# Boese0601/Dyadic-Interaction-Modeling

Measured on AMD Instinct MI355X. Metric: listener clips/sec (T=300, EMOCA-56), higher is better.
Workload: dtype bf16; 1 GPU; C3: B=256/GPU synthetic dyad clips, T=300, SLMFT.forward(mode='val'): listener VQ encode + encoder + 299-step AR decode (top-k 52 sampling) + VQ decode; global_batch=256, seq_len=300, gather=tokens+coeffs, gather_bytes_per_rank=17452032

## Files before the change

### dyadic-interaction-modeling_amd/csrc/chain.hip

```cpp
#include <algorithm>

#include "common.hpp"
#include "decode_attn_body.hpp"

namespace dimx {
namespace {

typedef __attribute__((address_space(3))) void lds_void_t;
typedef const __attribute__((address_space(1))) void glb_void_t;

constexpr int kWaves = 8;
constexpr int kThreads = kWaves * 64;
constexpr int kGroupCUs = 32;
constexpr int kGroupRows = 32;
constexpr int AUX_PLAIN = 0, AUX_SC1 = 16;
constexpr size_t kMaxDynLds = 160 * 1024 - 512;

__device__ __forceinline__ unsigned xcc_id() {
    unsigned v;
    asm volatile("s_getreg_b32 %0, hwreg(HW_REG_XCC_ID)" : "=s"(v));
    return v & 0xf;
}
__device__ __forceinline__ unsigned ld_sc1_u32(const unsigned* p) {
    return __hip_atomic_load(p, __ATOMIC_RELAXED, __HIP_MEMORY_SCOPE_AGENT);
// ... 758 lines not shown
    const int n1 = a.g1.W ? a.g1.ncb : 1, n2 = a.g2.W ? a.g2.ncb : 1;
    if (a.defer) {
        if (a.g2.W) {
            if (n1 == 1 && n2 == 1) CHD(true, 1, 1);
            else if (n1 == 2 && n2 == 1) CHD(true, 2, 1);
            else if (n1 == 1 && n2 == 2) CHD(true, 1, 2);
            else CHD(true, 2, 2);
        } else {
            if (n1 == 1) CHD(false, 1, 1);
            else CHD(false, 2, 1);
        }
    } else if (a.g1.W && a.g2.W) {
        if (n1 == 1 && n2 == 1) CH(true, true, 1, 1);
        else if (n1 == 2 && n2 == 1) CH(true, true, 2, 1);
        else if (n1 == 1 && n2 == 2) CH(true, true, 1, 2);
        else CH(true, true, 2, 2);
    } else if (a.g1.W) {
        if (n1 == 1) CH(true, false, 1, 1);
        else CH(true, false, 2, 1);
    } else if (a.g2.W) {
        if (n2 == 1) CH(false, true, 1, 1);
        else CH(false, true, 1, 2);
    } else {
        CH(false, false, 1, 1);
    }
#undef CH
#undef CHD
    DIMX_HIP(hipGetLastError());
    return DIMX_OK;
}


static size_t layer_plan(LayerChainArgs& a) {
    desc_fill(a.g_so);
    desc_fill(a.g_cq);
    desc_fill(a.g_co);
    const size_t sc_bytes = ((size_t)kAttnWaves * a.sc_stride * 4 + 1023) / 1024 * 1024;
    a.off_base = (int)sc_bytes;
    auto wbytes = [](const ChainGemmDesc& d) { return (size_t)d.nkt * d.rows_pad * 128 + 4096; };
    auto abytes = [](const ChainGemmDesc& d) { return (size_t)d.nkt * kGroupRows * 128; };
    auto rbytes = [](const ChainGemmDesc& d) { return (size_t)kWaves * d.ncb * 4096; };
    a.off_A1 = 0;
    a.off_W1 = (int)abytes(a.g_so);
    const size_t end1 = std::max(a.off_W1 + wbytes(a.g_so), rbytes(a.g_so));
    a.off_A2 = 0;
    a.off_W2 = (int)std::max(abytes(a.g_cq), rbytes(a.g_so));
    const size_t end2 = std::max(a.off_W2 + wbytes(a.g_cq), rbytes(a.g_cq));
    a.off_W3 = 0;
    a.off_A3 = (int)std::max(wbytes(a.g_co), rbytes(a.g_co));
    const size_t end3 = a.off_A3 + abytes(a.g_co);
    return sc_bytes + std::max(end1, std::max(end2, end3));
}

bool layer_chain_supported(const LayerChainArgs& a0, int cu_count) {
    LayerChainArgs a = a0;
    if (cu_count != 8 * kGroupCUs) return false;
    if (a.B < 1 || a.B > 8 * kGroupRows || a.C > 3 * kThreads || a.C % 64 != 0) return false;
    if (a.sa.H != kAttnWaves || a.ca.H != kAttnWaves || a.sa.dtype != DIMX_BF16 || a.ca.dtype != DIMX_BF16) return false;
    if (a.B * kAttnWaves * 2 <= 3072) return false;
    if (a.ca.rows_per_clip > 1) return false;
    for (ChainGemmDesc* d : {&a.g_so, &a.g_cq, &a.g_co}) {
        if (!d->W || d->N % kGroupCUs != 0 || d->K % 64 != 0 || d->ldw % 8 != 0) return false;
        desc_fill(*d);
        if (d->ncb < 1 || d->ncb > 2) return false;
    }
    if (a.g_so.N != a.C || a.g_co.N != a.C || a.g_cq.K != a.C || a.g_so.ncb != 2 || a.g_co.ncb != 2 || a.g_cq.ncb != 1) return false;
    if (a.ld_o % 8 != 0) return false;
    return layer_plan(a) <= kMaxDynLds;
}

int launch_layer_chain(const LayerChainArgs& a0, hipStream_t s) {
    LayerChainArgs a = a0;
    DIMX_REQUIRE(a.x && a.y && a.o && a.qc && a.stats && a.colsum_cq && a.counters && a.seen && a.err, DIMX_ERR_ARG,
                 "layer_chain: null operand");
    const size_t lds = layer_plan(a);
    DIMX_REQUIRE(lds <= kMaxDynLds, DIMX_ERR_ARG, "layer_chain: LDS plan %zu bytes", lds);
    if (a.sa.tab) {
        DIMX_REQUIRE(a.sa.hist && a.sa.hist_ld >= a.sa.Tmax && a.sa.Tmax >= 1 && a.sa.tab_rows >= 1 && a.sa.tab_ld % 8 == 0 &&
                         a.sa.tab_koff % 8 == 0 && a.sa.tab_voff % 8 == 0 && a.sa.tab_koff >= 0 && a.sa.tab_voff >= 0 &&
                         a.sa.tab_koff + kAttnWaves * 64 <= a.sa.tab_ld && a.sa.tab_voff + kAttnWaves * 64 <= a.sa.tab_ld &&
                         (uintptr_t)a.sa.tab % 16 == 0,
                     DIMX_ERR_ARG, "layer_chain: table form with rows of %d, K at %d, V at %d, history stride %d", a.sa.tab_ld, a.sa.tab_koff,
                     a.sa.tab_voff, a.sa.hist_ld);
        (void)hipFuncSetAttribute((const void*)xcd_layer_kernel<2, 1, 2, true>, hipFuncAttributeMaxDynamicSharedMemorySize, (int)kMaxDynLds);
        hipLaunchKernelGGL((xcd_layer_kernel<2, 1, 2, true>), dim3(8 * kGroupCUs), dim3(kLayerThreads), lds, s, a);
        DIMX_HIP(hipGetLastError());
        return DIMX_OK;
    }
    (void)hipFuncSetAttribute((const void*)xcd_layer_kernel<2, 1, 2>, hipFuncAttributeMaxDynamicSharedMemorySize, (int)kMaxDynLds);
    hipLaunchKernelGGL((xcd_layer_kernel<2, 1, 2>), dim3(8 * kGroupCUs), dim3(kLayerThreads), lds, s, a);
    DIMX_HIP(hipGetLastError());
    return DIMX_OK;
}

}
```

### dyadic-interaction-modeling_amd/csrc/common.hpp

```cpp
#pragma once
#include <hip/hip_runtime.h>
#include <stdint.h>
#include <stdio.h>
#include <string.h>
#include <string>

#include "../../include/dimx.h"

namespace dimx {

void set_error(const char* fmt, ...);
const char* get_error();

#define DIMX_HIP(expr)                                                                       \
    do {                                                                                     \
        hipError_t _e = (expr);                                                              \
        if (_e != hipSuccess) {                                                              \
            dimx::set_error("%s:%d: %s -> %s", __FILE__, __LINE__, #expr, hipGetErrorString(_e)); \
            return DIMX_ERR_HIP;                                                             \
        }                                                                                    \
    } while (0)

#define DIMX_REQUIRE(cond, code, ...)       \
    do {                                    \
// ... 222 lines not shown
    int w_tiled;
    const void* w3;
    long w3_plane;
    int x3_decode;
    int vt_pack4;
};

void gemm_args_init(GemmArgs& a);
void gemm_set_plain_out(GemmArgs& a, void* C, int ldc);
int launch_gemm(const GemmArgs& a, hipStream_t s);
bool gemm256_eligible(const GemmArgs& a);
int launch_gemm256(const GemmArgs& a, hipStream_t s);
int launch_gemm256_segs(const GemmArgs& a, const OutSeg* segs, int nseg, int seg_width, hipStream_t s);
bool gemm_use_x3(const GemmArgs& a);
bool gemm_x3_plan(const GemmArgs& a, int* bn_out, int* sp_out);
int launch_gemm_x3(const GemmArgs& a, hipStream_t s);
int launch_split_x3(const float* w, void* planes, size_t n, hipStream_t s);
int gemm_plan_splits(const GemmArgs& a);

int launch_layernorm(int out_dtype, const float* x, void* y, const float* gamma, const float* beta, int M,
                     int C, hipStream_t s);
int launch_add_slabs_layernorm(int out_dtype, float* x, const float* slabs, int nslab, long slab_stride, void* y,
                               const float* gamma, int M, int C, hipStream_t s);
int launch_instnorm(int out_dtype, const float* x, void* y, const int32_t* lens, int B, int T, int C,
                    hipStream_t s);

struct AttnArgs {
    int dtype;
    const void *q, *k, *vt;
    void* o;
    long q_sb, q_st, q_sh;
    long k_sb, k_st, k_sh;
    long v_sb, v_sh, v_sd;
    int v_rows;
    long v_st;
    long o_sb, o_st, o_sh;
    int B, H, Lq, Lk, D;
    float scale;
    int causal;
    const int32_t* lens;
    const uint8_t* kmask;
    int kmask_ld;
    unsigned long long* kwords;
    size_t kwords_cap;
    int kwords_ready;
};
int launch_pack_key_words(const uint8_t* kmask, int kmask_ld, const int32_t* lens, int B, int Lk, unsigned long long* words, size_t cap,
                          hipStream_t s);
int launch_attention(const AttnArgs& a, hipStream_t s);
int launch_attention_tr(const AttnArgs& a, hipStream_t s);
size_t mlp_fused_packed_bytes(int C, int F);
int mlp_fused_pack(const float* w1, const float* b1, const float* w2, int C, int F, uint16_t* out);
int launch_mlp_fused(float* x, const void* packed, const float* b2, const float* ln_g, const float* ln_b, int M, int C, int F, int act,
                     hipStream_t s);

struct DecodeAttnArgs {
    int dtype;
    const void* q;
    int q_ld;
    int q_f32;
    int nslab;
    long slab_stride;
    int force_nsplit;
    int rows_per_clip;
    const void* knew;
    const void* vnew;
    int kv_ld;
    void* kcache;
    void* vcache;
    int Tmax;
    void* out;
    int o_ld;
    int B, H;
    const int32_t* step;
    int n_keys;
    const uint8_t* kmask;
    int kmask_ld;
    float scale;
    const void* tab;
    int tab_ld, tab_koff, tab_voff, tab_rows;
    const int32_t* hist;
    int hist_ld;
    int win, lookahead;
};
int launch_decode_attn(const DecodeAttnArgs& a, hipStream_t s);

int launch_vq_argmin(const float* z, int N, const float* Et , const float* ee ,
                     int32_t* idx, float* best_d, float* margin, hipStream_t s);

struct ChainGemmDesc {
    const void* W;
    int N, K, ldw;
    int cols, rows_pad, ncb, nkt;
};
struct ChainArgs {
    int B;
    ChainGemmDesc g1;
    const void* A1;
    int lda1;
    float* xr;
    float* x;
    int C;
    const float* slabs;
    int nslab;
    long slab_stride;
    void* y;
    const float* gamma;
    ChainGemmDesc g2;
    float* out2;
    int ld_out2;
    unsigned* counters;
    unsigned* seen;
    const int32_t* step;
    unsigned* err;
    int defer;
    float* stats;
    const float* colsum2;
    int nbar;
    int fault;
    int offA1, offW1, offRed1, offA2, offW2, offRed2;
};
struct LayerChainArgs {
    int B, C;
    DecodeAttnArgs sa, ca;
    ChainGemmDesc g_so, g_cq, g_co;
    const void* o;
    int ld_o;
    float* x;
    void* y;
    float* stats;
    const float* colsum_cq;
    float* qc;
    int ld_qc;
    unsigned* counters;
    unsigned* seen;
    const int32_t* step;
    int epoch_add;
    unsigned* err;
    int fault;
    unsigned long long* prof;
    int sc_stride;
    int off_base, off_A1, off_W1, off_A2, off_W2, off_W3, off_A3;
};
bool layer_chain_supported(const LayerChainArgs& a, int cu_count);
int launch_layer_chain(const LayerChainArgs& a, hipStream_t s);
size_t chain_plan(ChainArgs& a);
bool chain_supported(const ChainArgs& a, int cu_count);
int launch_chain(const ChainArgs& a, hipStream_t s);

int launch_cast_pad(int out_dtype, const float* x, int ldx, const float* coladd, void* y, int ldy, int M, int K,
                    hipStream_t s, const uint8_t* zero_rows = nullptr);
int launch_gather_rows(int out_dtype, const float* table, int ld_table, int rows, const int32_t* idx, void* y,
                       int ldy, int M, int C, hipStream_t s);
constexpr int kLstmSave = 6;
size_t lstm_scratch_bytes(int B, int T, int In);
int lstm_layer_run(const float* x, int B, int T, int In, int H, const float* const* w_ih, const float* const* w_hh,
                   const float* const* b_ih, const float* const* b_hh, float* y, void* scratch, size_t scratch_bytes, int flags,
                   int cu_count, int* fault_count, hipStream_t st, float* save = nullptr);
size_t lstm_bwd_scratch_bytes(int B, int T);
int lstm_bwd_run(const float* dy, const float* save, const float* const* w_hh, int B, int T, float* dgates, void* scratch,
                 size_t scratch_bytes, int flags, int cu_count, int* fault_count, hipStream_t st);
int launch_context_concat(int out_dtype, const float* x_s, const float* patch, const float* audio, void* ctx,
                          int M, int dim, int dim_a, hipStream_t s);
int launch_finalize_idx(int32_t* idx, const int32_t* lens, int B, int T, int32_t pad_value, hipStream_t s,
                        int fqn = 1);
int launch_shift_tokens(const int32_t* z, int32_t* inp, int32_t* tgt, int B, int T, hipStream_t s);
int launch_ce_argmax(const float* logits, const int32_t* target, float* row_loss, int32_t* argmax_tok, int R,
                     int V, hipStream_t s);
// ... 12 lines not shown
    uint64_t step_host = 0;
    int32_t* tokens = nullptr;
    int tok_ld = 0, tok_col_from_step = 0, nslab = 0;
    long slab_stride = 0;
    float* logits_out = nullptr;
    int logits_out_ld = 0, row0 = 0, rows_total = 0;
    const float* emb_table = nullptr;
    int emb_C = 0;
    float* x_next = nullptr;
    int32_t* step_rw = nullptr;
    unsigned* done_ctr = nullptr;
    const float* pos_table = nullptr;
    float pos_scale = 0.f;
    int pos_rows = 0;
    const int32_t* dev_params = nullptr;
    void* y_next = nullptr;
    const float* y_gamma = nullptr;
    int y_dtype = DIMX_F32;
    const float* qkv0_table = nullptr;
    float* qkv0_out = nullptr;
    int qkv0_N = 0;
    const int32_t* prompt = nullptr;
    int prompt_ld = 0, prompt_max = 0;
    const int32_t* prompt_len = nullptr;
    int prompt_div = 1;
    int32_t* epoch_rw = nullptr;
    SampleFilter filt;
    int32_t* hist = nullptr;
    int hist_ld = 0;
};
int launch_sample(const SampleArgs& a, hipStream_t s);
struct BeamSelectArgs {
    const float* logits = nullptr;
    int nslab = 1;
    long slab_stride = 0;
    int nclip = 0, W = 0;
    const int32_t* step_dev = nullptr;
    int step_host = 0;
    int32_t* step_rw = nullptr;
    unsigned* done_ctr = nullptr;
    int32_t* epoch_rw = nullptr;
    const int32_t* dev_params = nullptr;
    const int32_t* prompt = nullptr;
    int prompt_ld = 0, prompt_max = 0;
    const int32_t* prompt_len = nullptr;
    const int32_t* lens = nullptr;
    int len_off = 0;
    const int32_t* mode = nullptr;
    const int32_t* forced_tok = nullptr;
    const double* cum_in = nullptr;
    double* cum_out = nullptr;
    int32_t* parent = nullptr;
    int32_t* tokens = nullptr;
    int32_t* backptr = nullptr;
    int tok_ld = 1;
    float* logits_out = nullptr;
    const float* emb_table = nullptr;
    int emb_C = 0;
    float* x_next = nullptr;
    const float* qkv0_table = nullptr;
    float* qkv0_out = nullptr;
    int qkv0_N = 0;
};
bool beam_width_supported(int W);
int launch_beam_select(const BeamSelectArgs& a, hipStream_t s);
struct BeamReorderArgs {
    void* buf[16] = {};
    int nbuf = 0, es = 4, nclip = 0, W = 0, H = 0, T = 0;
    const int32_t* parent = nullptr;
    const int32_t* step_dev = nullptr;
    int step_back = 0, c_host = 0;
    int32_t* tokens = nullptr;
    int32_t* backptr = nullptr;
    int tok_ld = 0;
};
int launch_beam_reorder(const BeamReorderArgs& a, hipStream_t s);
int launch_beam_init(double* cum, int32_t* parent, int R, int W, hipStream_t s);
int launch_iota_clamp(int32_t* ids, int n, int rows, hipStream_t s);
int launch_sum_slabs_rows(const float* slabs, int nslab, long slab_stride, float* table, int id0, int rows, int M, int N,
                          hipStream_t s);
int launch_gather_start_rows(const float* table, int N, int rows, const int32_t* start, int start_div, float* out, int B,
                             hipStream_t s, int start_ld = 1, int32_t* hist = nullptr, int hist_ld = 0);
int launch_kv0_image(const float* table, int ld, int rows, int col0, int W, void* image, hipStream_t s);
int launch_gen_params(int32_t* base, int groups, float temperature, uint64_t seed, int row_off, int rows_total,
                      hipStream_t s, int step0 = 0, float filter_a = 0.f, float filter_b = 0.f);
int launch_embed_step(const float* table, int C, int rows, const int32_t* start, const int32_t* tokens, int tok_ld,
                      const int32_t* step_dev, float* x, int B, int start_div, hipStream_t s,
                      const float* pos_table = nullptr, float pos_scale = 0.f, int start_ld = 1, int start_step = 0);
int launch_kv_rows_to_cache(int dtype, const void* src, void* cache, int B, int n, int H, int T, int S, hipStream_t st);
int launch_kv_vt_to_cache(const float* vt, int ld_t, float* cache, int B, int n, int H, int T, int S, hipStream_t st);
int launch_kv_rows_to_vt(const float* v_rows, int ld_rows, float* vt, int ld_t, int B, int n, int H, hipStream_t st);
int launch_prompt_rows(const int32_t* prompt, int ld, int B, int n0, int V, int S, int32_t* inp, int32_t* tokens, int tok_ld,
                       hipStream_t st);
int launch_add_pos_rows(float* x, const float* pos, int M, int n, int C, float scale, hipStream_t s);
int launch_mask_lens(const uint8_t* mask, int32_t* lens, int B, int T, hipStream_t s);
int launch_legacy_scramble(int out_dtype, const float* E, const int32_t* idx, const int32_t* lens, void* out, int B,
                           int T, int fqn, int zdim, int n_embed, hipStream_t s);
int launch_step_inc(int32_t* step_dev, hipStream_t s);
int launch_copy_rows_step(const float* src, float* dst, int B, int V, int n, const int32_t* step_dev, hipStream_t s);
int launch_mask_and(const uint8_t* a, const uint8_t* b, uint8_t* out, int n, hipStream_t s);

}
```

### dyadic-interaction-modeling_amd/csrc/decode_attn.hip

```cpp
#include "common.hpp"
#include "decode_attn_body.hpp"

namespace dimx {
namespace {

template <typename T, bool SELF, bool QF32, int NSPLIT, bool TAB = false, bool WIN = false>
__global__ __launch_bounds__(256) void decode_attn_kernel(const DecodeAttnArgs a) {
    constexpr int PPB = 4 / NSPLIT;
    __shared__ float sc[PPB][kMaxKeys];
    __shared__ float red_m[4], red_l[4];
    __shared__ float red_acc[4][64];
    decode_attn_body<T, SELF, QF32, NSPLIT, 4, false, TAB, WIN>(a, blockIdx.x, &sc[0][0], kMaxKeys, red_m, red_l, &red_acc[0][0]);
}

template <typename T, int SQ, bool QF32, bool WIN = false>
__global__ __launch_bounds__(256) void decode_attn_multi_kernel(const DecodeAttnArgs a) {
    constexpr int EPC = 16 / sizeof(T);
    constexpr int LPK = 64 / EPC;
    constexpr int KPI = 64 / LPK;
    constexpr int U = 4;
    constexpr int KB = U * KPI;
    extern __shared__ __attribute__((aligned(16))) float dyn_sc[];

    const int wave = threadIdx.x >> 6, lane = threadIdx.x & 63;
// ... 30 lines not shown
    }
    float mx[SQ];
#pragma unroll
    for (int q = 0; q < SQ; ++q) mx[q] = kNegD;
    for (int j0 = 0; j0 < n; j0 += KB) {
        if (j0 + KB < n) load_batch(kc, j0 + KB, nxt);
#pragma unroll
        for (int u = 0; u < U; ++u) {
            const int j = j0 + u * KPI + sub;
            float kv[EPC];
            cvt_chunk<T, EPC>(cur[u], kv);
            const bool dead = masked && j < n && a.kmask[(size_t)b * a.kmask_ld + j] == 0;
#pragma unroll
            for (int q = 0; q < SQ; ++q) {
                float d = 0.f;
#pragma unroll
                for (int e = 0; e < EPC; ++e) d = fmaf(qv[q][e], kv[e], d);
                d = LPK == 8 ? group8_sum(d) : row16_sum(d);
                if (j < n) {
                    const float sv = dead ? kNegD : d * scale2;
                    if (ch == 0) s[q * npad + j] = sv;
                    mx[q] = fmaxf(mx[q], sv);
                }
            }
        }
#pragma unroll
        for (int u = 0; u < U; ++u) cur[u] = nxt[u];
    }
    load_batch(vc, 0, cur);
#pragma unroll
    for (int q = 0; q < SQ; ++q) mx[q] = wave_max(mx[q]);
    __syncthreads();
    float lsum[SQ];
#pragma unroll
    for (int q = 0; q < SQ; ++q) {
        float l = 0.f;
        for (int j = lane; j < n; j += 64) {
            const float p = exp2f(s[q * npad + j] - mx[q]);
            s[q * npad + j] = p;
            l += p;
        }
        lsum[q] = wave_sum_sel<sizeof(T) == 2>(l);
    }
    __syncthreads();
    float acc[SQ][EPC];
#pragma unroll
    for (int q = 0; q < SQ; ++q)
#pragma unroll
        for (int e = 0; e < EPC; ++e) acc[q][e] = 0.f;
    for (int j0 = 0; j0 < n; j0 += KB) {
        if (j0 + KB < n) load_batch(vc, j0 + KB, nxt);
#pragma unroll
        for (int u = 0; u < U; ++u) {
            const int j = j0 + u * KPI + sub;
            float vv[EPC];
            cvt_chunk<T, EPC>(cur[u], vv);
#pragma unroll
            for (int q = 0; q < SQ; ++q) {
                const float p = j < n ? s[q * npad + j] : 0.f;
#pragma unroll
                for (int e = 0; e < EPC; ++e) acc[q][e] = fmaf(p, vv[e], acc[q][e]);
            }
        }
#pragma unroll
        for (int u = 0; u < U; ++u) cur[u] = nxt[u];
    }
#pragma unroll
    for (int q = 0; q < SQ; ++q) {
#pragma unroll
        for (int e = 0; e < EPC; ++e) {
            if (LPK <= 8) acc[q][e] += xor_lane_f32<8>(acc[q][e]);
            acc[q][e] += xor_lane_f32<16>(acc[q][e]);
            acc[q][e] += xor_lane_f32<32>(acc[q][e]);
        }
        if (active && sub == 0) {
            const float inv = lsum[q] > 0.f ? 1.0f / lsum[q] : 0.f;
#pragma unroll
            for (int e = 0; e < EPC; ++e) acc[q][e] *= inv;
            store_chunk<T, EPC>((T*)a.out + ((size_t)b * SQ + q) * a.o_ld + h * 64 + ch * EPC, acc[q]);
        }
    }
}

}

int launch_decode_attn(const DecodeAttnArgs& a, hipStream_t s) {
    DIMX_REQUIRE(a.q && a.kcache && a.vcache && a.out, DIMX_ERR_ARG, "decode_attn: null operand");
    DIMX_REQUIRE((a.knew == nullptr) == (a.vnew == nullptr), DIMX_ERR_ARG, "decode_attn: knew/vnew mismatch");
    DIMX_REQUIRE(a.knew == nullptr || a.step != nullptr, DIMX_ERR_ARG, "decode_attn: self attention needs a step counter");
    DIMX_REQUIRE(a.Tmax <= kMaxKeys && a.n_keys <= kMaxKeys, DIMX_ERR_ARG, "decode_attn: more than %d keys", kMaxKeys);
    DIMX_REQUIRE(a.knew != nullptr || a.n_keys >= 1, DIMX_ERR_ARG, "decode_attn: cross attention over %d keys", a.n_keys);
    if (a.tab) {
        const int epc = a.dtype == DIMX_BF16 ? 8 : 4;
        DIMX_REQUIRE(a.knew && a.q_f32 && a.hist && a.hist_ld >= a.Tmax && a.Tmax >= 1 && a.tab_rows >= 1, DIMX_ERR_ARG,
                     "decode_attn: the table form is self attention on f32 slabs with a token history of at least Tmax entries per row");
        DIMX_REQUIRE(a.tab_ld % epc == 0 && a.tab_koff % epc == 0 && a.tab_voff % epc == 0 && a.tab_koff >= 0 && a.tab_voff >= 0 &&
                         a.tab_koff + a.H * 64 <= a.tab_ld && a.tab_voff + a.H * 64 <= a.tab_ld && (uintptr_t)a.tab % 16 == 0,
                     DIMX_ERR_ARG, "decode_attn: table rows of %d with K at %d and V at %d", a.tab_ld, a.tab_koff, a.tab_voff);
    }
    DIMX_REQUIRE(!a.win || (a.knew == nullptr && a.step != nullptr && !a.tab), DIMX_ERR_ARG,
                 "decode_attn: the windowed form is cross attention with a step counter");
    if (a.rows_per_clip > 1) {
        DIMX_REQUIRE(a.knew == nullptr, DIMX_ERR_ARG, "decode_attn: rows_per_clip applies to cross attention only");
        const int S = a.rows_per_clip;
        const int npad = (a.n_keys + 3) & ~3;
        const size_t lds = (size_t)4 * S * npad * sizeof(float);
        DIMX_REQUIRE(lds <= 150 * 1024, DIMX_ERR_ARG, "decode_attn: %d samples x %d keys do not fit the LDS score buffer", S,
                     a.n_keys);
        dim3 grid(ceil_div(a.B * a.H, 4)), block(256);
#define DM_W(TT, SS, QQ, WW)                                                                                    \
    do {                                                                                                        \
        (void)hipFuncSetAttribute((const void*)decode_attn_multi_kernel<TT, SS, QQ, WW>,                        \
                                  hipFuncAttributeMaxDynamicSharedMemorySize, (int)lds);                        \
        hipLaunchKernelGGL((decode_attn_multi_kernel<TT, SS, QQ, WW>), grid, block, lds, s, a);                 \
    } while (0)
#define DM(TT, SS, QQ)                        \
    do {                                      \
        if (a.win) DM_W(TT, SS, QQ, true);    \
        else DM_W(TT, SS, QQ, false);         \
    } while (0)
#define DM_S(TT, QQ)                         \
    do {                                     \
        switch (S) {                         \
            case 2: DM(TT, 2, QQ); break;    \
            case 4: DM(TT, 4, QQ); break;    \
            case 5: DM(TT, 5, QQ); break;    \
            case 8: DM(TT, 8, QQ); break;    \
            case 10: DM(TT, 10, QQ); break;  \
            default:                         \
                set_error("decode_attn: rows_per_clip %d not in {2,4,5,8,10}", S); \
                return DIMX_ERR_ARG;         \
        }                                    \
    } while (0)
        if (a.dtype == DIMX_BF16) { if (a.q_f32) DM_S(bf16, true); else DM_S(bf16, false); }
        else { if (a.q_f32) DM_S(float, true); else DM_S(float, false); }
#undef DM_S
#undef DM
#undef DM_W
        DIMX_HIP(hipGetLastError());
        return DIMX_OK;
    }
    const int pairs = a.B * a.H;
    int nsplit = 1;
    if (pairs * 2 <= 3072) nsplit = 2;
    if (pairs * 4 <= 3072) nsplit = 4;
    if (a.dtype != DIMX_BF16) nsplit = a.Tmax >= 1024 ? 4 : (a.Tmax >= 512 ? 2 : 1);
    if (a.force_nsplit == 1 || a.force_nsplit == 2 || a.force_nsplit == 4) nsplit = a.force_nsplit;
    dim3 grid(ceil_div(pairs, 4 / nsplit)), block(256);
    const bool self = a.knew != nullptr;
#define DA_LAUNCH(TT, SS, QQ, NS) hipLaunchKernelGGL((decode_attn_kernel<TT, SS, QQ, NS>), grid, block, 0, s, a)
#define DA_NS(TT, SS, QQ)                          \
    do {                                           \
        if (nsplit == 4) DA_LAUNCH(TT, SS, QQ, 4); \
        else if (nsplit == 2) DA_LAUNCH(TT, SS, QQ, 2); \
        else DA_LAUNCH(TT, SS, QQ, 1);             \
    } while (0)
#define DA_TAB(TT)                                                                                  \
    do {                                                                                            \
        if (nsplit == 4) hipLaunchKernelGGL((decode_attn_kernel<TT, true, true, 4, true>), grid, block, 0, s, a);      \
        else if (nsplit == 2) hipLaunchKernelGGL((decode_attn_kernel<TT, true, true, 2, true>), grid, block, 0, s, a); \
        else hipLaunchKernelGGL((decode_attn_kernel<TT, true, true, 1, true>), grid, block, 0, s, a);                  \
    } while (0)
#define DA_WIN(TT, QQ)                                                                              \
    do {                                                                                            \
        if (nsplit == 4) hipLaunchKernelGGL((decode_attn_kernel<TT, false, QQ, 4, false, true>), grid, block, 0, s, a);      \
        else if (nsplit == 2) hipLaunchKernelGGL((decode_attn_kernel<TT, false, QQ, 2, false, true>), grid, block, 0, s, a); \
        else hipLaunchKernelGGL((decode_attn_kernel<TT, false, QQ, 1, false, true>), grid, block, 0, s, a);                  \
    } while (0)
    if (a.tab) {
        if (a.dtype == DIMX_BF16) DA_TAB(bf16); else DA_TAB(float);
    } else if (a.win) {
        if (a.dtype == DIMX_BF16) { if (a.q_f32) DA_WIN(bf16, true); else DA_WIN(bf16, false); }
        else { if (a.q_f32) DA_WIN(float, true); else DA_WIN(float, false); }
    } else if (a.dtype == DIMX_BF16) {
        if (a.q_f32) { if (self) DA_NS(bf16, true, true); else DA_NS(bf16, false, true); }
        else { if (self) DA_NS(bf16, true, false); else DA_NS(bf16, false, false); }
    } else {
        if (a.q_f32) { if (self) DA_NS(float, true, true); else DA_NS(float, false, true); }
        else { if (self) DA_NS(float, true, false); else DA_NS(float, false, false); }
    }
#undef DA_WIN
#undef DA_TAB
// ... 8 lines not shown
```

### dyadic-interaction-modeling_amd/csrc/decode_attn_body.hpp

```cpp
#pragma once
#include "common.hpp"

namespace dimx {
namespace {

typedef unsigned int u32x4_nt __attribute__((ext_vector_type(4)));
template <typename P> __device__ __forceinline__ uint4 ld_stream(const P* p) {
    const u32x4_nt v = __builtin_nontemporal_load((const u32x4_nt*)p);
    return make_uint4(v.x, v.y, v.z, v.w);
}

__device__ __forceinline__ int win_keys(int step, int lookahead, int n_keys) {
    const long long v = (long long)step + 2 + lookahead;
    return v < 1 ? 1 : (v > n_keys ? n_keys : (int)v);
}

constexpr int kMaxKeys = 2048;
constexpr float kNegD = -3.0e38f;

template <typename T, int EPC> __device__ __forceinline__ void load_chunk(const T* p, float (&v)[EPC]);
template <> __device__ __forceinline__ void load_chunk<float, 4>(const float* p, float (&v)[4]) {
    const float4 f = *(const float4*)p;
    v[0] = f.x; v[1] = f.y; v[2] = f.z; v[3] = f.w;
}
template <> __device__ __forceinline__ void load_chunk<bf16, 8>(const bf16* p, float (&v)[8]) {
    const uint4 u = *(const uint4*)p;
    const uint32_t w[4] = {u.x, u.y, u.z, u.w};
#pragma unroll
    for (int i = 0; i < 4; ++i) {
        v[2 * i] = __builtin_bit_cast(float, w[i] << 16);
        v[2 * i + 1] = __builtin_bit_cast(float, w[i] & 0xffff0000u);
    }
}
template <typename T, int EPC> __device__ __forceinline__ void store_chunk(T* p, const float (&v)[EPC]);
template <> __device__ __forceinline__ void store_chunk<float, 4>(float* p, const float (&v)[4]) {
    *(float4*)p = make_float4(v[0], v[1], v[2], v[3]);
}
template <> __device__ __forceinline__ void store_chunk<bf16, 8>(bf16* p, const float (&v)[8]) {
    *(uint4*)p = make_uint4(pack_bf16x2(v[0], v[1]), pack_bf16x2(v[2], v[3]), pack_bf16x2(v[4], v[5]),
                            pack_bf16x2(v[6], v[7]));
}

template <typename T, int EPC> __device__ __forceinline__ void cvt_chunk(const uint4& u, float (&v)[EPC]);
template <> __device__ __forceinline__ void cvt_chunk<float, 4>(const uint4& u, float (&v)[4]) {
    v[0] = __builtin_bit_cast(float, u.x); v[1] = __builtin_bit_cast(float, u.y);
    v[2] = __builtin_bit_cast(float, u.z); v[3] = __builtin_bit_cast(float, u.w);
}
template <> __device__ __forceinline__ void cvt_chunk<bf16, 8>(const uint4& u, float (&v)[8]) {
    const uint32_t w[4] = {u.x, u.y, u.z, u.w};
#pragma unroll
    for (int i = 0; i < 4; ++i) {
        v[2 * i] = __builtin_bit_cast(float, w[i] << 16);
        v[2 * i + 1] = __builtin_bit_cast(float, w[i] & 0xffff0000u);
    }
}

template <int EPC> __device__ __forceinline__ void load_f32_chunk(const float* p, float (&v)[EPC]) {
#pragma unroll
    for (int i = 0; i < EPC / 4; ++i) {
        const float4 f = *(const float4*)(p + 4 * i);
        v[4 * i] = f.x; v[4 * i + 1] = f.y; v[4 * i + 2] = f.z; v[4 * i + 3] = f.w;
    }
}
template <int EPC> __device__ __forceinline__ void load_f32_chunk_sc1(const float* p, float (&v)[EPC]) {
#pragma unroll
    for (int i = 0; i < EPC; ++i) v[i] = __hip_atomic_load(p + i, __ATOMIC_RELAXED, __HIP_MEMORY_SCOPE_AGENT);
}
template <int EPC> __device__ __forceinline__ void load_f32_slabs(const float* p, int nslab, long stride, float (&v)[EPC]) {
    load_f32_chunk<EPC>(p, v);
    for (int s = 1; s < nslab; ++s) {
        float t[EPC];
        load_f32_chunk<EPC>(p + (size_t)s * stride, t);
#pragma unroll
        for (int e = 0; e < EPC; ++e) v[e] += t[e];
    }
}

template <typename T, bool SELF, bool QF32, int NSPLIT, int NW, bool QSC1 = false, bool TAB = false, bool WIN = false>
__device__ __forceinline__ void decode_attn_body(const DecodeAttnArgs& a, int block_id, float* sc, int sc_stride, float* red_m,
                                                 float* red_l, float* red_acc) {
    constexpr int EPC = 16 / sizeof(T);
    constexpr int LPK = 64 / EPC;
    constexpr int KPI = 64 / LPK;
    constexpr int U = 4;
    constexpr int KB = U * KPI;
    constexpr int PPB = NW / NSPLIT;
    static_assert(!TAB || SELF, "the table form is a self-attention form");
    static_assert(!WIN || !SELF, "the windowed form is a cross-attention form");

    const int wave = threadIdx.x >> 6, lane = threadIdx.x & 63;
    const int pib = wave / NSPLIT, part = wave % NSPLIT;
    const int pair = block_id * PPB + pib;
    const bool active = pair < a.B * a.H;
    const int b = active ? pair / a.H : 0, h = active ? pair % a.H : 0;
    const int sub = lane / LPK, ch = lane % LPK;
    const int jfirst = part * KB, jstep = NSPLIT * KB;
    auto load_ids = [&](int j0, int (&id)[U]) {
        const int32_t* hrow = a.hist + (size_t)b * a.hist_ld;
#pragma unroll
        for (int u = 0; u < U; ++u) {
            const int j = j0 + u * KPI + sub;
            id[u] = hrow[j < a.Tmax ? j : a.Tmax - 1];
        }
    };
    int ida[U] = {}, idb[U] = {}, idc[U] = {};
    if constexpr (TAB) {
        load_ids(jfirst, ida);
        load_ids(jfirst + jstep, idb);
    }
    float qv[EPC], knv[EPC], vnv[EPC];
    if (QSC1)
        load_f32_chunk_sc1<EPC>((const float*)a.q + (size_t)b * a.q_ld + h * 64 + ch * EPC, qv);
    else if (QF32)
        load_f32_slabs<EPC>((const float*)a.q + (size_t)b * a.q_ld + h * 64 + ch * EPC, a.nslab, a.slab_stride, qv);
    else
        load_chunk<T, EPC>((const T*)a.q + (size_t)b * a.q_ld + h * 64 + ch * EPC, qv);
    if (SELF) {
        if (QF32) {
            load_f32_slabs<EPC>((const float*)a.knew + (size_t)b * a.kv_ld + h * 64 + ch * EPC, a.nslab, a.slab_stride, knv);
            load_f32_slabs<EPC>((const float*)a.vnew + (size_t)b * a.kv_ld + h * 64 + ch * EPC, a.nslab, a.slab_stride, vnv);
        } else {
            load_chunk<T, EPC>((const T*)a.knew + (size_t)b * a.kv_ld + h * 64 + ch * EPC, knv);
            load_chunk<T, EPC>((const T*)a.vnew + (size_t)b * a.kv_ld + h * 64 + ch * EPC, vnv);
        }
    }
    int n = a.n_keys;
    if (SELF) n = *a.step;
    if constexpr (WIN) n = win_keys(*a.step, a.lookahead, a.n_keys);
    const float scale2 = a.scale * 1.4426950408889634f;

    const T* kc = (const T*)a.kcache + ((size_t)(b * a.H + h) * a.Tmax) * 64 + ch * EPC;
    const T* vc = (const T*)a.vcache + ((size_t)(b * a.H + h) * a.Tmax) * 64 + ch * EPC;
    float* s = sc + (size_t)pib * sc_stride;
    const bool masked = !SELF && a.kmask != nullptr;

    auto load_batch = [&](const T* base, int j0, uint4 (&r)[U]) {
#pragma unroll
        for (int u = 0; u < U; ++u) {
            const int j = j0 + u * KPI + sub;
            r[u] = ld_stream(base + (size_t)(j < n ? j : (n > 0 ? n - 1 : 0)) * 64);
        }
    };
    const T* tk = (const T*)a.tab + a.tab_koff + h * 64 + ch * EPC;
    const T* tv = (const T*)a.tab + a.tab_voff + h * 64 + ch * EPC;
    auto load_tab = [&](const T* base, const int (&id)[U], uint4 (&r)[U]) {
#pragma unroll
        for (int u = 0; u < U; ++u) {
            const unsigned t = (unsigned)id[u] < (unsigned)a.tab_rows ? (unsigned)id[u] : (unsigned)a.tab_rows - 1u;
            r[u] = *(const uint4*)(base + (size_t)t * a.tab_ld);
        }
    };

    uint4 cur[U], nxt[U], vfirst[U];
    if (jfirst < n) {
        if constexpr (TAB) {
            load_tab(tk, ida, cur);
            load_tab(tv, ida, vfirst);
        } else {
            load_batch(kc, jfirst, cur);
            load_batch(vc, jfirst, vfirst);
        }
    }
    if (masked) {
        for (int j = part * 64 + lane; j < n; j += NSPLIT * 64) s[j] = a.kmask[(size_t)b * a.kmask_ld + j] ? 0.f : kNegD;
    }
    if (masked && NSPLIT > 1) __syncthreads();

    float mx = kNegD;
    for (int j0 = jfirst; j0 < n; j0 += jstep) {
        if constexpr (TAB) {
            if (j0 + 2 * jstep < n) load_ids(j0 + 2 * jstep, idc);
            if (j0 + jstep < n) load_tab(tk, idb, nxt);
        } else {
            if (j0 + jstep < n) load_batch(kc, j0 + jstep, nxt);
        }
#pragma unroll
        for (int u = 0; u < U; ++u) {
            const int j = j0 + u * KPI + sub;
            float kv[EPC];
            cvt_chunk<T, EPC>(cur[u], kv);
            float d = 0.f;
#pragma unroll
            for (int e = 0; e < EPC; ++e) d = fmaf(qv[e], kv[e], d);
            d = LPK == 8 ? group8_sum(d) : row16_sum(d);
            if (j < n) {
                float sv = d * scale2;
                if (masked && s[j] != 0.f) sv = kNegD;
                if (ch == 0) s[j] = sv;
                mx = fmaxf(mx, sv);
            }
        }
#pragma unroll
        for (int u = 0; u < U; ++u) cur[u] = nxt[u];
        if constexpr (TAB) {
#pragma unroll
            for (int u = 0; u < U; ++u) idb[u] = idc[u];
        }
    }
#pragma unroll
    for (int u = 0; u < U; ++u) cur[u] = vfirst[u];
    if constexpr (TAB) {
        if (jfirst + jstep < n) load_ids(jfirst + jstep, idb);
    }
    int total = n;
    if (SELF) {
        float d = 0.f;
#pragma unroll
        for (int e = 0; e < EPC; ++e) d = fmaf(qv[e], knv[e], d);
        d = LPK == 8 ? group8_sum(d) : row16_sum(d);
        const float sv = d * scale2;
        total = n + 1;
        if (part == 0) {
            if (lane == 0) s[n] = sv;
            mx = fmaxf(mx, sv);
            if (!TAB && active && sub == 0) {
                store_chunk<T, EPC>((T*)a.kcache + ((size_t)(b * a.H + h) * a.Tmax + n) * 64 + ch * EPC, knv);
                store_chunk<T, EPC>((T*)a.vcache + ((size_t)(b * a.H + h) * a.Tmax + n) * 64 + ch * EPC, vnv);
            }
        }
    }
    mx = wave_max(mx);
    if (NSPLIT > 1) {
        if (lane == 0) red_m[wave] = mx;
        __syncthreads();
#pragma unroll
        for (int p = 0; p < NSPLIT; ++p) mx = fmaxf(mx, red_m[pib * NSPLIT + p]);
    }

    float lsum = 0.f;
    for (int j = part * 64 + lane; j < total; j += NSPLIT * 64) {
        const float p = exp2f(s[j] - mx);
        s[j] = p;
        lsum += p;
    }
    lsum = wave_sum_sel<sizeof(T) == 2>(lsum);
    if (NSPLIT > 1) {
        if (lane == 0) red_l[wave] = lsum;
        __syncthreads();
        lsum = 0.f;
#pragma unroll
        for (int p = 0; p < NSPLIT; ++p) lsum += red_l[pib * NSPLIT + p];
    }

    float acc[EPC];
#pragma unroll
    for (int e = 0; e < EPC; ++e) acc[e] = 0.f;
    for (int j0 = jfirst; j0 < n; j0 += jstep) {
        if constexpr (TAB) {
            if (j0 + 2 * jstep < n) load_ids(j0 + 2 * jstep, idc);
            if (j0 + jstep < n) load_tab(tv, idb, nxt);
        } else {
            if (j0 + jstep < n) load_batch(vc, j0 + jstep, nxt);
        }
#pragma unroll
        for (int u = 0; u < U; ++u) {
            const int j = j0 + u * KPI + sub;
            float vv[EPC];
            cvt_chunk<T, EPC>(cur[u], vv);
            const float p = j < n ? s[j] : 0.f;
#pragma unroll
            for (int e = 0; e < EPC; ++e) acc[e] = fmaf(p, vv[e], acc[e]);
        }
#pragma unroll
        for (int u = 0; u < U; ++u) cur[u] = nxt[u];
        if constexpr (TAB) {
#pragma unroll
            for (int u = 0; u < U; ++u) idb[u] = idc[u];
        }
    }
    if (SELF && part == 0 && sub == 0) {
        const float p = s[n];
#pragma unroll
        for (int e = 0; e < EPC; ++e) acc[e] = fmaf(p, vnv[e], acc[e]);
    }
#pragma unroll
    for (int e = 0; e < EPC; ++e) {
        if (LPK <= 8) acc[e] += xor_lane_f32<8>(acc[e]);
        acc[e] += xor_lane_f32<16>(acc[e]);
        acc[e] += xor_lane_f32<32>(acc[e]);
    }
    if (NSPLIT > 1) {
        if (sub == 0) {
#pragma unroll
            for (int e = 0; e < EPC; ++e) red_acc[wave * 64 + ch * EPC + e] = acc[e];
        }
        __syncthreads();
        if (part == 0 && sub == 0) {
#pragma unroll
            for (int p = 1; p < NSPLIT; ++p)
#pragma unroll
                for (int e = 0; e < EPC; ++e) acc[e] += red_acc[(pib * NSPLIT + p) * 64 + ch * EPC + e];
        }
    }
// ... 11 lines not shown
```

### dyadic-interaction-modeling_amd/csrc/elementwise.hip

```cpp
#include "common.hpp"

namespace dimx {
namespace {

template <typename OutT>
__global__ void cast_pad_kernel(const float* __restrict__ x, int ldx, const float* __restrict__ coladd,
                                OutT* __restrict__ y, int ldy, int M, int K, const uint8_t* __restrict__ zero_rows) {
    const long total = (long)M * ldy;
    for (long i = (long)blockIdx.x * blockDim.x + threadIdx.x; i < total; i += (long)gridDim.x * blockDim.x) {
        const int m = (int)(i / ldy), k = (int)(i - (long)m * ldy);
        float v = 0.f;
        if (k < K && !(zero_rows && zero_rows[m])) {
            v = x[(size_t)m * ldx + k];
            if (coladd) v += coladd[k];
        }
        store_from_f32<OutT>(y + i, v);
    }
}

template <typename OutT>
__global__ void gather_rows_kernel(const float* __restrict__ table, int ld_table, int rows,
                                   const int32_t* __restrict__ idx, OutT* __restrict__ y, int ldy, int M, int C) {
    const long total = (long)M * C;
    for (long i = (long)blockIdx.x * blockDim.x + threadIdx.x; i < total; i += (long)gridDim.x * blockDim.x) {
// ... 371 lines not shown
                            *(float2*)((float*)y_next + (size_t)row * emb_C + 2 * i) = make_float2(o0, o1);
                    }
                }
            }
        } else {
            for (int i = lane; i < nv; i += 64) {
                float2 e = src[i];
                if (with_pos) {
                    const float2 q = pr[i];
                    e = make_float2(__fadd_rn(e.x, __fmul_rn(q.x, pos_scale)), __fadd_rn(e.y, __fmul_rn(q.y, pos_scale)));
                }
                dst[i] = e;
            }
        }
    }
    }
    if (step_rw) {
        __syncthreads();
        if (threadIdx.x == 0) {
            const unsigned prev = atomicAdd(done_ctr, 1u);
            if (prev == gridDim.x - 1) {
                *done_ctr = 0u;
                *step_rw = (int32_t)step + 1;
                if (epoch_rw) *epoch_rw += 1;
            }
        }
    }
}

__global__ __launch_bounds__(256) void embed_step_kernel(const float* __restrict__ table, int C,
                                                         const int32_t* __restrict__ start,
                                                         const int32_t* __restrict__ tokens, int tok_ld,
                                                         const int32_t* __restrict__ step_dev, float* __restrict__ x,
                                                         int rows, int start_div,
                                                         const float* __restrict__ pos_table, float pos_scale, int start_ld,
                                                         int start_step) {
    const int b = blockIdx.x;
    const int step = *step_dev;
    int tok = step == start_step ? start[(size_t)(b / start_div) * start_ld] : tokens[(size_t)b * tok_ld + step - 1];
    tok = tok < 0 ? 0 : (tok >= rows ? rows - 1 : tok);
    const float4* src = (const float4*)(table + (size_t)tok * C);
    float4* dst = (float4*)(x + (size_t)b * C);
    if (pos_table) {
        const float4* pr = (const float4*)(pos_table + (size_t)step * C);
        for (int i = threadIdx.x; i < C / 4; i += blockDim.x) {
            const float4 e = src[i], q = pr[i];
            dst[i] = make_float4(__fadd_rn(e.x, __fmul_rn(q.x, pos_scale)), __fadd_rn(e.y, __fmul_rn(q.y, pos_scale)),
                                 __fadd_rn(e.z, __fmul_rn(q.z, pos_scale)), __fadd_rn(e.w, __fmul_rn(q.w, pos_scale)));
        }
    } else {
        for (int i = threadIdx.x; i < C / 4; i += blockDim.x) dst[i] = src[i];
    }
}

__global__ void iota_clamp_kernel(int32_t* __restrict__ ids, int n, int rows) {
    const int i = blockIdx.x * blockDim.x + threadIdx.x;
    if (i < n) ids[i] = i < rows ? i : rows - 1;
}

__global__ __launch_bounds__(256) void sum_slabs_rows_kernel(const float* __restrict__ slabs, int nslab, long slab_stride,
                                                             float* __restrict__ table, int id0, int rows, int M, int N) {
    const int m = blockIdx.x;
    if (m >= M || id0 + m >= rows) return;
    const float4* src = (const float4*)(slabs + (size_t)m * N);
    float4* dst = (float4*)(table + (size_t)(id0 + m) * N);
    for (int i = threadIdx.x; i < N / 4; i += blockDim.x) {
        float4 v = src[i];
        for (int s = 1; s < nslab; ++s) {
            const float4 t = *(const float4*)(slabs + (size_t)s * slab_stride + (size_t)m * N + 4 * i);
            v.x = __fadd_rn(v.x, t.x); v.y = __fadd_rn(v.y, t.y); v.z = __fadd_rn(v.z, t.z); v.w = __fadd_rn(v.w, t.w);
        }
        dst[i] = v;
    }
}

__global__ __launch_bounds__(256) void gather_start_rows_kernel(const float* __restrict__ table, int N, int rows,
                                                                const int32_t* __restrict__ start, int start_div,
                                                                float* __restrict__ out, int start_ld,
                                                                int32_t* __restrict__ hist, int hist_ld) {
    const int b = blockIdx.x;
    int tok = start[(size_t)(b / start_div) * start_ld];
    tok = tok < 0 ? 0 : (tok >= rows ? rows - 1 : tok);
    if (hist && threadIdx.x == 0) hist[(size_t)b * hist_ld] = tok;
    const float4* src = (const float4*)(table + (size_t)tok * N);
    float4* dst = (float4*)(out + (size_t)b * N);
    for (int i = threadIdx.x; i < N / 4; i += blockDim.x) dst[i] = src[i];
}

__global__ __launch_bounds__(256) void kv0_image_kernel(const float* __restrict__ table, int ld, int col0, int W,
                                                        uint32_t* __restrict__ image) {
    const float2* src = (const float2*)(table + (size_t)blockIdx.x * ld + col0);
    uint32_t* dst = image + (size_t)blockIdx.x * (W / 2);
    for (int i = threadIdx.x; i < W / 2; i += blockDim.x) {
        const float2 v = src[i];
        dst[i] = pack_bf16x2(v.x, v.y);
    }
}

__global__ void add_pos_rows_kernel(float* __restrict__ x, const float* __restrict__ pos, int M, int n, int C,
                                    float scale) {
    const long total = (long)M * C;
    for (long i = (long)blockIdx.x * blockDim.x + threadIdx.x; i < total; i += (long)gridDim.x * blockDim.x) {
        const int m = (int)(i / C), c = (int)(i - (long)m * C);
        x[i] = __fadd_rn(x[i], __fmul_rn(pos[(size_t)(m % n) * C + c], scale));
    }
}

__global__ __launch_bounds__(64) void mask_lens_kernel(const uint8_t* __restrict__ mask, int32_t* __restrict__ lens,
                                                       int T) {
    const int b = blockIdx.x;
    int n = 0;
    for (int t = threadIdx.x; t < T; t += 64) n += mask[(size_t)b * T + t] ? 1 : 0;
#pragma unroll
    for (int o = 1; o < 64; o <<= 1) n += __shfl_xor(n, o);
    if (threadIdx.x == 0) lens[b] = n;
}

template <typename OutT>
__global__ void legacy_scramble_kernel(const float* __restrict__ E, const int32_t* __restrict__ idx,
                                       const int32_t* __restrict__ lens, OutT* __restrict__ out, int B, int T, int fqn,
                                       int zdim, int n_embed) {
    const long per = (long)T * fqn * zdim, total = (long)B * per;
    const int P = T * fqn;
    for (long i = (long)blockIdx.x * blockDim.x + threadIdx.x; i < total; i += (long)gridDim.x * blockDim.x) {
        const int b = (int)(i / per);
        const long f = i - (long)b * per;
        const int c = (int)(f / P), p = (int)(f - (long)c * P);
        float v = 0.f;
        if (p < lens[b] * fqn) {
            int r = idx[(size_t)b * P + p];
            r = r < 0 ? 0 : (r >= n_embed ? n_embed - 1 : r);
            v = E[(size_t)r * zdim + c];
        }
        store_from_f32<OutT>(out + i, v);
    }
}

__global__ void step_inc_kernel(int32_t* step) { *step += 1; }

__global__ void gen_params_kernel(int32_t* base, int groups, float temperature, uint64_t seed, int row_off,
                                  int rows_total, int step0, float filter_a, float filter_b) {
    const int g = threadIdx.x;
    if (g >= groups) return;
    int32_t* p = base + 16 * g;
    p[0] = step0;
    p[8] = 0;
    p[9] = 0;
    p[10] = step0;
    p[2] = __builtin_bit_cast(int32_t, temperature);
    *(uint64_t*)(p + 4) = seed;
    p[6] = row_off;
    p[7] = rows_total;
    p[11] = __builtin_bit_cast(int32_t, filter_a);
    p[12] = __builtin_bit_cast(int32_t, filter_b);
}

__global__ void copy_rows_step_kernel(const float* __restrict__ src, float* __restrict__ dst, int B, int V, int n,
                                      const int32_t* __restrict__ step_dev) {
    const int i = blockIdx.x * blockDim.x + threadIdx.x;
    if (i >= B * V) return;
    const int b = i / V, c = i - b * V;
    dst[((size_t)b * n + *step_dev) * V + c] = src[i];
}

__global__ void mask_and_kernel(const uint8_t* a, const uint8_t* b, uint8_t* out, int n) {
    const int i = blockIdx.x * blockDim.x + threadIdx.x;
// ... 58 lines not shown
}

int launch_shift_tokens(const int32_t* z, int32_t* inp, int32_t* tgt, int B, int T, hipStream_t s) {
    hipLaunchKernelGGL(shift_tokens_kernel, dim3(ceil_div(B * (T - 1), 256)), dim3(256), 0, s, z, inp, tgt, B, T);
    DIMX_HIP(hipGetLastError());
    return DIMX_OK;
}

int launch_ce_argmax(const float* logits, const int32_t* target, float* row_loss, int32_t* argmax_tok, int R, int V,
                     hipStream_t s) {
    DIMX_REQUIRE(V == 512, DIMX_ERR_ARG, "ce_argmax: vocabulary %d != 512", V);
    hipLaunchKernelGGL(ce_argmax_kernel, dim3(ceil_div(R, 4)), dim3(256), 0, s, logits, target, row_loss, argmax_tok,
                       R);
    DIMX_HIP(hipGetLastError());
    return DIMX_OK;
}

int launch_sample(const SampleArgs& a, hipStream_t s) {
    const SampleFilter& filt = a.filt;
    DIMX_REQUIRE(a.logits && a.tokens && a.R > 0, DIMX_ERR_ARG, "sample: bad arguments");
    DIMX_REQUIRE(filt.kind >= DIMX_FILTER_TOP_K && filt.kind <= DIMX_FILTER_TOP_A, DIMX_ERR_ARG, "sample: unknown filter kind %d", filt.kind);
    DIMX_REQUIRE(!filt.keep_out || !a.prompt, DIMX_ERR_ARG, "sample: keep_out is not written for prompted rows");
    DIMX_REQUIRE(!a.prompt || (a.step_dev && a.tok_col_from_step && a.prompt_max >= 1 && a.prompt_ld >= a.prompt_max && a.prompt_div >= 1),
                 DIMX_ERR_ARG, "sample: a prompt needs the device step counter, 1 <= prompt_max <= prompt_ld and rows per clip >= 1");
    DIMX_REQUIRE(!a.qkv0_table || (a.x_next && a.qkv0_out && !a.pos_table && a.emb_C / 2 <= 16 * 64 && a.qkv0_N % 4 == 0 && a.qkv0_N > 0 &&
                                   a.qkv0_N <= 12 * 256),
                 DIMX_ERR_ARG, "sample: the q/k/v table rides on the fused embedding (no positional table) and holds rows of k * 4 <= 3072");
    DIMX_REQUIRE(!a.hist || (a.step_dev && a.hist_ld >= 1), DIMX_ERR_ARG, "sample: the token history needs the device step counter");
    DIMX_REQUIRE(!a.y_next || (a.x_next && a.y_gamma && a.emb_C % 128 == 0 && a.emb_C <= 2048), DIMX_ERR_ARG,
                 "sample: the fused pre-norm needs the fused embedding and a width of k * 128 <= 2048");
    const int wpb = a.R <= 1024 ? 1 : 4;
    auto kern = filt.kind == DIMX_FILTER_TOP_P   ? sample_kernel<DIMX_FILTER_TOP_P>
                : filt.kind == DIMX_FILTER_MIN_P ? sample_kernel<DIMX_FILTER_MIN_P>
                : filt.kind == DIMX_FILTER_TOP_A ? sample_kernel<DIMX_FILTER_TOP_A>
                                                 : sample_kernel<DIMX_FILTER_TOP_K>;
    hipLaunchKernelGGL(kern, dim3(ceil_div(a.R, wpb)), dim3(64 * wpb), 0, s, a.logits, a.ld_logits, a.R, a.top_k,
                       a.temperature, a.noise, a.seed, a.step_dev, a.step_host, a.tokens, a.tok_ld, a.tok_col_from_step,
                       a.nslab < 1 ? 1 : a.nslab, a.slab_stride, a.logits_out, a.logits_out_ld, a.row0, a.rows_total, a.emb_table,
                       a.emb_C, a.x_next, a.step_rw, a.done_ctr, a.pos_table, a.pos_scale, a.pos_rows, a.dev_params, a.y_next,
                       a.y_gamma, a.y_dtype == DIMX_BF16 ? 1 : 0, a.qkv0_table, a.qkv0_out, a.qkv0_N, a.prompt, a.prompt_ld,
                       a.prompt_max, a.prompt_len, a.prompt_div < 1 ? 1 : a.prompt_div, a.epoch_rw, filt.a, filt.b, filt.keep_out,
                       a.hist, a.hist_ld);
    DIMX_HIP(hipGetLastError());
    return DIMX_OK;
}

int launch_gen_params(int32_t* base, int groups, float temperature, uint64_t seed, int row_off, int rows_total,
                      hipStream_t s, int step0, float filter_a, float filter_b) {
    DIMX_REQUIRE(step0 >= 0, DIMX_ERR_ARG, "gen_params: negative first step");
    hipLaunchKernelGGL(gen_params_kernel, dim3(1), dim3(64), 0, s, base, groups, temperature, seed, row_off, rows_total, step0,
                       filter_a, filter_b);
    DIMX_HIP(hipGetLastError());
    return DIMX_OK;
}

int launch_embed_step(const float* table, int C, int rows, const int32_t* start, const int32_t* tokens, int tok_ld,
                      const int32_t* step_dev, float* x, int B, int start_div, hipStream_t s, const float* pos_table,
                      float pos_scale, int start_ld, int start_step) {
    DIMX_REQUIRE(C % 4 == 0 && start_ld >= 1 && start_step >= 0, DIMX_ERR_ARG, "embed_step: C %% 4, start stride or step");
    hipLaunchKernelGGL(embed_step_kernel, dim3(B), dim3(256), 0, s, table, C, start, tokens, tok_ld, step_dev, x,
                       rows, start_div < 1 ? 1 : start_div, pos_table, pos_scale, start_ld, start_step);
    DIMX_HIP(hipGetLastError());
    return DIMX_OK;
}

int launch_iota_clamp(int32_t* ids, int n, int rows, hipStream_t s) {
    DIMX_REQUIRE(ids && n > 0 && rows > 0, DIMX_ERR_ARG, "iota_clamp: bad arguments");
    hipLaunchKernelGGL(iota_clamp_kernel, dim3(ceil_div(n, 256)), dim3(256), 0, s, ids, n, rows);
    DIMX_HIP(hipGetLastError());
    return DIMX_OK;
}

int launch_sum_slabs_rows(const float* slabs, int nslab, long slab_stride, float* table, int id0, int rows, int M, int N,
                          hipStream_t s) {
    DIMX_REQUIRE(slabs && table && nslab >= 1 && M > 0 && N > 0 && N % 4 == 0 && slab_stride % 4 == 0 && id0 >= 0, DIMX_ERR_ARG,
                 "sum_slabs_rows: bad arguments");
    hipLaunchKernelGGL(sum_slabs_rows_kernel, dim3(M), dim3(256), 0, s, slabs, nslab, slab_stride, table, id0, rows, M, N);
    DIMX_HIP(hipGetLastError());
    return DIMX_OK;
}

int launch_gather_start_rows(const float* table, int N, int rows, const int32_t* start, int start_div, float* out, int B,
                             hipStream_t s, int start_ld, int32_t* hist, int hist_ld) {
    DIMX_REQUIRE(table && start && out && B > 0 && N > 0 && N % 4 == 0 && rows > 0 && start_ld >= 1 && (!hist || hist_ld >= 1), DIMX_ERR_ARG,
                 "gather_start_rows: bad arguments");
    hipLaunchKernelGGL(gather_start_rows_kernel, dim3(B), dim3(256), 0, s, table, N, rows, start, start_div < 1 ? 1 : start_div, out,
                       start_ld, hist, hist_ld);
    DIMX_HIP(hipGetLastError());
    return DIMX_OK;
}

int launch_kv0_image(const float* table, int ld, int rows, int col0, int W, void* image, hipStream_t s) {
    DIMX_REQUIRE(table && image && rows > 0 && W > 0 && W % 2 == 0 && col0 >= 0 && col0 % 2 == 0 && ld % 2 == 0 && col0 + W <= ld, DIMX_ERR_ARG,
                 "kv0_image: bad arguments");
    hipLaunchKernelGGL(kv0_image_kernel, dim3(rows), dim3(256), 0, s, table, ld, col0, W, (uint32_t*)image);
    DIMX_HIP(hipGetLastError());
    return DIMX_OK;
}

int launch_add_pos_rows(float* x, const float* pos, int M, int n, int C, float scale, hipStream_t s) {
    DIMX_REQUIRE(x && pos && M > 0 && n > 0, DIMX_ERR_ARG, "add_pos_rows: bad arguments");
    const long total = (long)M * C;
    const int blocks = (int)(total / 256 + 1 < 4096 ? total / 256 + 1 : 4096);
    hipLaunchKernelGGL(add_pos_rows_kernel, dim3(blocks), dim3(256), 0, s, x, pos, M, n, C, scale);
    DIMX_HIP(hipGetLastError());
    return DIMX_OK;
}

int launch_mask_lens(const uint8_t* mask, int32_t* lens, int B, int T, hipStream_t s) {
    DIMX_REQUIRE(mask && lens && B > 0 && T > 0, DIMX_ERR_ARG, "mask_lens: bad arguments");
    hipLaunchKernelGGL(mask_lens_kernel, dim3(B), dim3(64), 0, s, mask, lens, T);
    DIMX_HIP(hipGetLastError());
    return DIMX_OK;
}

int launch_legacy_scramble(int out_dtype, const float* E, const int32_t* idx, const int32_t* lens, void* out, int B,
                           int T, int fqn, int zdim, int n_embed, hipStream_t s) {
    DIMX_REQUIRE(E && idx && lens && out && B > 0 && T > 0, DIMX_ERR_ARG, "legacy_scramble: bad arguments");
    const long total = (long)B * T * fqn * zdim;
    const int blocks = (int)(total / 256 + 1 < 8192 ? total / 256 + 1 : 8192);
    if (out_dtype == DIMX_BF16)
        hipLaunchKernelGGL((legacy_scramble_kernel<bf16>), dim3(blocks), dim3(256), 0, s, E, idx, lens, (bf16*)out, B,
                           T, fqn, zdim, n_embed);
    else
        hipLaunchKernelGGL((legacy_scramble_kernel<float>), dim3(blocks), dim3(256), 0, s, E, idx, lens, (float*)out,
                           B, T, fqn, zdim, n_embed);
    DIMX_HIP(hipGetLastError());
    return DIMX_OK;
}

int launch_step_inc(int32_t* step_dev, hipStream_t s) {
    hipLaunchKernelGGL(step_inc_kernel, dim3(1), dim3(1), 0, s, step_dev);
    DIMX_HIP(hipGetLastError());
    return DIMX_OK;
}

int launch_copy_rows_step(const float* src, float* dst, int B, int V, int n, const int32_t* step_dev, hipStream_t s) {
    hipLaunchKernelGGL(copy_rows_step_kernel, dim3(ceil_div(B * V, 256)), dim3(256), 0, s, src, dst, B, V, n, step_dev);
    DIMX_HIP(hipGetLastError());
    return DIMX_OK;
}

int launch_mask_and(const uint8_t* a, const uint8_t* b, uint8_t* out, int n, hipStream_t s) {
    hipLaunchKernelGGL(mask_and_kernel, dim3(ceil_div(n, 256)), dim3(256), 0, s, a, b, out, n);
    DIMX_HIP(hipGetLastError());
    return DIMX_OK;
}

}
```

### dyadic-interaction-modeling_amd/csrc/generate.hip

```cpp
#include <stdlib.h>

#include "stages.hpp"

namespace dimx {

static void chain_desc(ChainGemmDesc& d, const Linear& L) { d.W = L.w; d.N = L.N; d.K = L.K; d.ldw = L.Kp; }

static bool gen_use_chain(dimx_handle h, int B, int S) {
    if (!h->use_chain || h->at != DIMX_BF16 || S != 1 || h->gen_groups > 1 || !h->chain_err_dev) return false;
    const DecGeom& dg = h->decg;
    ChainArgs c;
    memset(&c, 0, sizeof(c));
    c.B = B;
    c.C = dg.dim;
    const XAttn& sa = h->dec.self_[0];
    const XAttn& ca = h->dec.cross[0];
    chain_desc(c.g1, sa.out);
    c.lda1 = dg.heads * dg.dim_head;
    chain_desc(c.g2, ca.qkv);
    if (!chain_supported(c, h->cu_count)) return false;
    chain_desc(c.g2, h->dec.logits);
    c.g1.W = nullptr;
    return chain_supported(c, h->cu_count) && 3 * dg.depth + 1 <= kChainSites;
}

static bool gen_multi_tr(dimx_handle h, int S) {
    return S > 1 && h->multi_tr && h->at == DIMX_BF16 && h->decg.dim_head == 64;
}

static int slab_gemm_rows(dimx_handle h, int B, hipStream_t st, const void* A, int lda, const Linear& L, float* out, long stride,
                          int* nsl) {
    GemmArgs g;
    gemm_lin(h, A, lda, L, B, g);
    g.x3_decode = 1;
    g.out_dtype = DIMX_F32;
    g.out_slabs = 1;
    static const bool f32_split = getenv("DIMX_F32_NO_SPLIT") == nullptr;
    if (f32_split) g.allow_splitk = 1;
    g.slab_stride = stride;
    gemm_set_plain_out(g, out, L.N);
    *nsl = gemm_plan_splits(g);
    g.force_splitk = *nsl;
    return launch_gemm(g, st);
}

static bool qkv0_table_supported(dimx_handle h) {
    const DecGeom& dg = h->decg;
    const int N = 3 * dg.heads * dg.dim_head;
    return h->use_qkv0_table && !dg.abs_pos && h->dec.self_[0].qkv.N == N && N % 4 == 0 && N <= 12 * 256 && dg.dim % 4 == 0 &&
           dg.dim / 2 <= 16 * 64;
}

static int qkv0_table_alloc(dimx_handle h) {
    const int V = h->decg.num_tokens, N = h->dec.self_[0].qkv.N;
    if (!h->qkv0_table) {
        DIMX_HIP(hipMalloc((void**)&h->qkv0_table, (size_t)V * N * sizeof(float)));
        h->qkv0_epoch = 0;
        h->graph_valid = false;
    }
    if (h->use_kv0_table && h->at == DIMX_BF16 && !h->kv0_image) {
        DIMX_HIP(hipMalloc(&h->kv0_image, (size_t)V * 2 * (N / 3) * sizeof(bf16)));
        h->qkv0_epoch = 0;
        h->graph_valid = false;
    }
    return DIMX_OK;
}

static int qkv0_table_build(dimx_handle h, const GenScratch& s, int M, hipStream_t st, int step0 = 0) {
    const DecGeom& dg = h->decg;
    const int DD = dg.dim, V = dg.num_tokens, N = h->dec.self_[0].qkv.N;
    if (h->qkv0_M == M && h->qkv0_at == h->at && h->qkv0_epoch == h->dec_epoch) return DIMX_OK;
    h->qkv0_epoch = 0;
    const int rounds = (V + M - 1) / M;
    int32_t* ids = (int32_t*)s.logits;
    DIMX_TRY(launch_iota_clamp(ids, rounds * M, V, st));
    for (int r = 0; r < rounds; ++r) {
        int ns = 0;
        DIMX_TRY(launch_embed_step(h->dec.tok_emb, DD, V, ids + (size_t)r * M, nullptr, 0, s.step, s.x, M, 1, st, nullptr, 0.f, 1, step0));
        DIMX_TRY(launch_add_slabs_layernorm(h->at, s.x, s.xr, 0, s.st_xr, s.y, h->dec.self_[0].ln_g, M, DD, st));
        DIMX_TRY(slab_gemm_rows(h, M, st, s.y, DD, h->dec.self_[0].qkv, s.qkv, s.st_qkv, &ns));
        DIMX_TRY(launch_sum_slabs_rows(s.qkv, ns, s.st_qkv, h->qkv0_table, r * M, V, M, N, st));
    }
    if (h->kv0_image) DIMX_TRY(launch_kv0_image(h->qkv0_table, N, V, N / 3, 2 * (N / 3), h->kv0_image, st));
    h->qkv0_M = M;
    h->qkv0_at = h->at;
    h->qkv0_epoch = h->dec_epoch;
    ++h->qkv0_builds;
    return DIMX_OK;
}

struct GenRequest {
    GenPrompt pr;
    const uint8_t* ctx_mask;
    int B, T, S;
    float temperature;
    int top_k;
    const float* noise;
    uint64_t seed;
    int32_t* tokens;
    float* logits_out;
    void* ws;
    size_t ws_bytes;
    hipStream_t st;
    const BeamCall* beam;
};

struct GenCall {
    const GenRequest& req;
    const CtxPersist& cp;
    const GenScratch& s;
    int R;
    int top_k;
};

struct StepCtx {
    dimx_handle h;
    const GenCall* gc;
    const StepRoute* r;
    hipStream_t st;
    int row0, B, grp;
    int clip0, nclip;
    int T, S, DD, heads, D, inner, V, n, Tp;
    int n_keys;
    size_t es;
    float scale, pos_scale;
    const float* pos;
    GenScratch s;
    const void *ck[8], *cv[8];
    const int32_t *start, *forced, *forced_len;
    const uint8_t* ctx_mask;
    int32_t* tokens;
    float* logits_out;
};

static StepCtx step_ctx(dimx_handle h, const GenCall& gc, const StepRoute& r, int row0, int B, int grp, hipStream_t st) {
    const GenRequest& q = gc.req;
    const GenScratch& s0 = gc.s;
    const GenPrompt& pr = q.pr;
    const DecGeom& dg = h->decg;
    StepCtx c;
    c.h = h; c.gc = &gc; c.r = &r; c.st = st;
    c.row0 = row0; c.B = B; c.grp = grp;
    c.T = q.T; c.S = q.S;
    c.clip0 = row0 / c.S; c.nclip = B / c.S;
    c.DD = dg.dim; c.heads = dg.heads; c.D = dg.dim_head; c.inner = c.heads * c.D;
    c.V = dg.num_tokens; c.n = gen_steps(h, c.T); c.Tp = tpad(c.T); c.n_keys = c.T;
    c.es = es_of(h); c.scale = 1.0f / sqrtf((float)c.D);
    c.pos = dg.abs_pos ? h->dec.pos_emb : nullptr; c.pos_scale = 1.0f / sqrtf((float)c.DD);
    const int T = c.T, DD = c.DD, heads = c.heads, inner = c.inner;
    const size_t es = c.es;
    auto boff = [&](void* p, size_t per_row_bytes) { return (void*)((unsigned char*)p + (size_t)row0 * per_row_bytes); };
    c.s = s0;
    for (int l = 0; l < dg.depth; ++l) {
        c.s.sk[l] = boff(s0.sk[l], (size_t)heads * T * 64 * es);
        c.s.sv[l] = boff(s0.sv[l], (size_t)heads * T * 64 * es);
        c.ck[l] = (unsigned char*)gc.cp.ck[l] + (size_t)c.clip0 * heads * c.Tp * 64 * es;
        c.cv[l] = (unsigned char*)gc.cp.cv[l] + (size_t)c.clip0 * heads * c.Tp * 64 * es;
    }
    c.s.x = s0.x + (size_t)row0 * DD;
    c.s.y = boff(s0.y, DD * es);
    c.s.qkv = s0.qkv + (size_t)row0 * 3 * inner;
    c.s.qc = s0.qc + (size_t)row0 * inner;
    c.s.xr = s0.xr + (size_t)row0 * DD;
    c.s.o = boff(s0.o, inner * es);
    c.s.f = boff(s0.f, (size_t)DD * dg.ff_mult * es);
    c.s.logits = s0.logits + (size_t)row0 * c.V;
    c.s.step = s0.step + 16 * grp;
    c.s.hist = s0.hist + (size_t)row0 * T;
    c.s.qcb = boff(s0.qcb, inner * es);
    c.s.kw = s0.kw + (size_t)c.clip0 * ((T + 63) / 64);
    c.s.kw_cap = s0.kw_cap - (size_t)c.clip0 * ((T + 63) / 64);
    c.start = pr.tok + (size_t)c.clip0 * pr.ld + pr.step0;
    c.forced = pr.Pmax > 1 ? pr.tok + (size_t)c.clip0 * pr.ld : nullptr;
    c.forced_len = pr.len ? pr.len + c.clip0 : nullptr;
    c.ctx_mask = q.ctx_mask + (size_t)c.clip0 * T;
    c.tokens = q.tokens + (size_t)row0 * c.n;
    c.logits_out = q.logits_out ? q.logits_out + (size_t)row0 * c.n * c.V : nullptr;
    return c;
}

static int gen_start(const StepCtx& c) {
    dimx_handle h = c.h;
    const GenScratch& s = c.s;
    const GenPrompt& pr = c.gc->req.pr;
    DIMX_TRY(launch_embed_step(h->dec.tok_emb, c.DD, c.V, c.start, c.tokens, c.n, s.step, s.x, c.B, c.S, c.st, c.pos, c.pos_scale, pr.ld, pr.step0));
    if (c.r->qkv0)
        return launch_gather_start_rows(c.r->qkv0, 3 * c.inner, c.V, c.start, c.S, s.qkv, c.B, c.st, pr.ld, c.r->kv0 ? s.hist : nullptr, c.T);
    return launch_add_slabs_layernorm(h->at, s.x, s.xr, 0, s.st_xr, s.y, h->dec.self_[0].ln_g, c.B, c.DD, c.st);
}

static int slab_gemm(const StepCtx& c, const void* A, int lda, const Linear& L, float* out, long stride, int* nsl) {
    return slab_gemm_rows(c.h, c.B, c.st, A, lda, L, out, stride, nsl);
}

static int chain_site(const StepCtx& c, int site, const void* A1, int lda1, const Linear* W1, int nslab, const float* gamma,
                      const Linear* W2, float* out2, int ld_out2, const float* colsum2 = nullptr) {
    dimx_handle h = c.h;
    const GenScratch& s = c.s;
    ChainArgs a;
    memset(&a, 0, sizeof(a));
    a.B = c.B; a.C = c.DD;
    if (c.r->defer && W1) { a.defer = 1; a.stats = h->chain_stats_dev; a.colsum2 = colsum2; }
    if (W1) {
        chain_desc(a.g1, *W1);
        a.A1 = A1; a.lda1 = lda1; a.xr = s.xr;
    }
    a.x = s.x; a.y = s.y; a.gamma = gamma;
    a.slabs = nslab ? s.xr : nullptr; a.nslab = nslab; a.slab_stride = s.st_xr;
    if (W2) {
        chain_desc(a.g2, *W2);
        a.out2 = out2; a.ld_out2 = ld_out2;
    }
    a.counters = s.chain_ctr + (size_t)site * kChainSiteWords;
    a.seen = a.counters + 8 * 16; a.err = h->chain_err_dev; a.fault = c.r->fault_inject ? 1 : 0;
    a.step = s.step + 9;
    return launch_chain(a, c.st);
}

static DecodeAttnArgs self_args(const StepCtx& c, int l, int ns) {
    const GenScratch& s = c.s;
    const int inner = c.inner;
    DecodeAttnArgs sa;
    memset(&sa, 0, sizeof(sa));
    sa.dtype = c.h->at;
    sa.q = s.qkv; sa.q_ld = 3 * inner; sa.q_f32 = 1; sa.nslab = ns; sa.slab_stride = s.st_qkv;
    sa.knew = s.qkv + inner; sa.vnew = s.qkv + 2 * inner; sa.kv_ld = 3 * inner;
    sa.kcache = s.sk[l]; sa.vcache = s.sv[l]; sa.Tmax = c.T;
    sa.out = s.o; sa.o_ld = inner; sa.B = c.B; sa.H = c.heads; sa.step = s.step; sa.scale = c.scale;
    if (l == 0 && c.r->kv0) {
        sa.tab = c.r->kv0; sa.tab_rows = c.V;
        if (c.h->at == DIMX_BF16) { sa.tab_ld = 2 * inner; sa.tab_koff = 0; sa.tab_voff = inner; }
        else { sa.tab_ld = 3 * inner; sa.tab_koff = inner; sa.tab_voff = 2 * inner; }
        sa.hist = s.hist; sa.hist_ld = c.T;
    }
    return sa;
}

static DecodeAttnArgs cross_args(const StepCtx& c, int l) {
    const GenScratch& s = c.s;
    DecodeAttnArgs ca;
    memset(&ca, 0, sizeof(ca));
    ca.dtype = c.h->at;
    ca.q = s.qc; ca.q_ld = c.inner; ca.q_f32 = 1; ca.nslab = 1; ca.slab_stride = s.st_qc;
    ca.kcache = (void*)c.ck[l]; ca.vcache = (void*)c.cv[l]; ca.Tmax = c.Tp;
    ca.out = s.o; ca.o_ld = c.inner; ca.B = c.S > 1 ? c.nclip : c.B; ca.rows_per_clip = c.S; ca.H = c.heads;
    ca.n_keys = c.n_keys; ca.kmask = c.ctx_mask; ca.kmask_ld = c.T; ca.scale = c.scale;
    if (c.r->win) { ca.win = 1; ca.lookahead = c.r->lookahead; ca.step = s.step; }
    return ca;
}

static bool layer_args(const StepCtx& c, int l, const DecodeAttnArgs& sa, const DecodeAttnArgs& ca, LayerChainArgs& lc) {
    dimx_handle h = c.h;
    const GenScratch& s = c.s;
    const Linear& so = h->dec.self_[l].out;
    const Linear& cq = h->dec.cross[l].q_ln;
    const Linear& co = h->dec.cross[l].out;
    if (!so.w || !cq.w || !co.w || !h->dec.cross[l].q_ln_colsum) return false;
    lc.B = c.B; lc.C = c.DD; lc.sa = sa; lc.ca = ca;
    chain_desc(lc.g_so, so);
    chain_desc(lc.g_cq, cq);
    chain_desc(lc.g_co, co);
    lc.o = s.o; lc.ld_o = c.inner; lc.x = s.x; lc.y = s.y;
    lc.stats = h->chain_stats_dev; lc.colsum_cq = h->dec.cross[l].q_ln_colsum;
    lc.qc = s.qc; lc.ld_qc = c.inner;
    lc.counters = s.chain_ctr + (size_t)(3 * h->decg.depth + 1 + l) * kChainSiteWords;
    lc.seen = lc.counters + 8 * 16; lc.step = s.step + 9; lc.err = h->chain_err_dev; lc.fault = c.r->fault_inject ? 1 : 0;
    lc.sc_stride = (c.T + 15) / 16 * 16;
    lc.prof = h->layer_prof_dev ? h->layer_prof_dev + (size_t)l * 256 * 16 : nullptr;
    return true;
}

static int cross_attention_multi(const StepCtx& c, int l, const DecodeAttnArgs& ca) {
    dimx_handle h = c.h;
    const GenScratch& s = c.s;
    const int heads = c.heads, D = c.D, inner = c.inner, S = c.S, T = c.T, Tp = c.Tp;
    GemmArgs g;
    gemm_lin(h, s.y, c.DD, h->dec.cross[l].qkv, c.B, g);
    g.out_dtype = h->at;
    gemm_set_plain_out(g, s.qcb, inner);
    DIMX_TRY(launch_gemm(g, c.st));
    AttnArgs ta;
    memset(&ta, 0, sizeof(ta));
    ta.dtype = h->at;
    ta.q = s.qcb;
    ta.q_sb = (long)S * inner; ta.q_st = inner; ta.q_sh = D;
    ta.k = ca.kcache; ta.k_sb = (long)heads * Tp * D; ta.k_sh = (long)Tp * D; ta.k_st = D;
    ta.vt = ca.vcache; ta.v_rows = 1; ta.v_sb = (long)heads * Tp * D; ta.v_sh = (long)Tp * D; ta.v_st = D;
    ta.o = s.o; ta.o_sb = (long)S * inner; ta.o_st = inner; ta.o_sh = D;
    ta.B = c.nclip; ta.H = heads; ta.Lq = S; ta.Lk = T; ta.D = D;
    ta.scale = c.scale;
    ta.kmask = c.ctx_mask; ta.kmask_ld = T;
    ta.kwords = s.kw; ta.kwords_cap = s.kw_cap;
    ta.kwords_ready = 1;
    return launch_attention_tr(ta, c.st);
}

static int attention_half(const StepCtx& c, int l, int* pending) {
    dimx_handle h = c.h;
    const GenScratch& s = c.s;
    const StepRoute& r = *c.r;
    const int B = c.B, DD = c.DD, inner = c.inner;
    int ns = 0;
    if (l > 0) DIMX_TRY(launch_add_slabs_layernorm(h->at, s.x, s.xr, *pending, s.st_xr, s.y, h->dec.self_[l].ln_g, B, DD, c.st));
    if (l == 0 && r.qkv0)
        ns = 1;
    else
        DIMX_TRY(slab_gemm(c, s.y, DD, h->dec.self_[l].qkv, s.qkv, s.st_qkv, &ns));
    const DecodeAttnArgs sa = self_args(c, l, ns);
    DecodeAttnArgs ca = cross_args(c, l);
    if (r.layer_kernel[l]) {
        LayerChainArgs lc;
        memset(&lc, 0, sizeof(lc));
        DIMX_REQUIRE(layer_args(c, l, sa, ca, lc), DIMX_ERR_STATE, "generate: layer %d lost its layer-kernel weights after the route was resolved", l);
        DIMX_TRY(launch_layer_chain(lc, c.st));
    } else if (r.chain) {
        DIMX_TRY(launch_decode_attn(sa, c.st));
// ... 16 lines not shown
            ca.nslab = ns;
            DIMX_TRY(launch_decode_attn(ca, c.st));
        }
        DIMX_TRY(slab_gemm(c, s.o, inner, h->dec.cross[l].out, s.xr, s.st_xr, pending));
        DIMX_TRY(launch_add_slabs_layernorm(h->at, s.x, s.xr, *pending, s.st_xr, s.y, h->dec.ff[l].ln_g, B, DD, c.st));
    }
    return DIMX_OK;
}

static int feed_forward(const StepCtx& c, int l, int* pending) {
    dimx_handle h = c.h;
    const GenScratch& s = c.s;
    const bool defer = c.r->defer;
    const int F = c.DD * h->decg.ff_mult;
    GemmArgs g;
    gemm_lin(h, s.y, c.DD, defer ? h->dec.ff[l].f1_ln : h->dec.ff[l].f1, c.B, g);
    g.x3_decode = 1;
    if (defer) {
        g.ln_stats = h->chain_stats_dev;
        g.ln_err = h->chain_err_dev;
        g.ln_colsum = h->dec.ff[l].f1_ln_colsum;
        g.ln_C = c.DD;
    }
    g.out_dtype = h->at;
    g.act = ACT_GELU_ERF;
    gemm_set_plain_out(g, s.f, F);
    DIMX_TRY(launch_gemm(g, c.st));
    return slab_gemm(c, s.f, F, h->dec.ff[l].f2, s.xr, s.st_xr, pending);
}

static int logits(const StepCtx& c, int pending, int* nlg) {
    dimx_handle h = c.h;
    const GenScratch& s = c.s;
    if (c.r->logits_chain) {
        *nlg = 1;
        return chain_site(c, 3 * h->decg.depth, nullptr, 0, nullptr, pending, h->dec.final_g, &h->dec.logits, s.logits, c.V);
    }
    DIMX_TRY(launch_add_slabs_layernorm(h->at, s.x, s.xr, pending, s.st_xr, s.y, h->dec.final_g, c.B, c.DD, c.st));
    return slab_gemm(c, s.y, c.DD, h->dec.logits, s.logits, s.st_lg, nlg);
}

static int finish_beam(const StepCtx& c, int nlg) {
    dimx_handle h = c.h;
    const GenScratch& s = c.s;
    const GenPrompt& pr = c.gc->req.pr;
    const BeamCall& bm = *c.r->beam;
    const int row0 = c.row0, n = c.n, depth = h->decg.depth;
    BeamSelectArgs bs;
    bs.logits = s.logits; bs.nslab = nlg; bs.slab_stride = s.st_lg; bs.nclip = c.nclip; bs.W = c.S;
    bs.step_dev = s.step; bs.step_rw = s.step; bs.done_ctr = (unsigned*)(s.step + 8); bs.epoch_rw = s.step + 9; bs.dev_params = s.step + 2;
    bs.prompt = c.forced; bs.prompt_ld = pr.ld; bs.prompt_max = pr.Pmax; bs.prompt_len = c.forced_len;
    bs.lens = bm.lens ? bm.lens + c.clip0 : nullptr; bs.len_off = c.T - n;
    bs.cum_in = bm.cum + row0; bs.cum_out = bm.cum + row0; bs.parent = bm.parent + row0;
    bs.tokens = c.tokens; bs.backptr = bm.backptr ? bm.backptr + (size_t)row0 * n : nullptr; bs.tok_ld = n; bs.logits_out = c.logits_out;
    bs.emb_table = h->dec.tok_emb; bs.emb_C = c.DD; bs.x_next = s.x;
    bs.qkv0_table = c.r->qkv0; bs.qkv0_out = s.qkv; bs.qkv0_N = 3 * c.inner;
    DIMX_TRY(launch_beam_select(bs, c.st));
    if (!c.r->qkv0) DIMX_TRY(launch_add_slabs_layernorm(h->at, s.x, s.xr, 0, s.st_xr, s.y, h->dec.self_[0].ln_g, c.B, c.DD, c.st));
    BeamReorderArgs br;
    for (int l = 0; l < depth; ++l) {
        br.buf[2 * l] = s.sk[l];
        br.buf[2 * l + 1] = s.sv[l];
    }
    br.nbuf = 2 * depth; br.es = (int)c.es; br.nclip = c.nclip; br.W = c.S; br.H = c.heads; br.T = c.T;
    br.parent = bs.parent; br.step_dev = s.step; br.step_back = 1;
    br.tokens = c.tokens; br.backptr = bs.backptr; br.tok_ld = n;
    return launch_beam_reorder(br, c.st);
}

static int finish_sample(const StepCtx& c, int nlg) {
    dimx_handle h = c.h;
    const GenScratch& s = c.s;
    const GenRequest& q = c.gc->req;
    const GenPrompt& pr = q.pr;
    const float* qkv0 = c.r->qkv0;
    SampleArgs sm;
    sm.logits = s.logits; sm.ld_logits = c.V; sm.R = c.B; sm.nslab = nlg; sm.slab_stride = s.st_lg; sm.row0 = c.row0; sm.rows_total = c.gc->R;
    sm.top_k = c.gc->top_k; sm.noise = q.noise; sm.filt.kind = h->filter_kind;
    sm.temperature = q.temperature; sm.seed = q.seed;
    sm.step_dev = s.step; sm.step_rw = s.step; sm.dev_params = s.step + 2; sm.done_ctr = (unsigned*)(s.step + 8); sm.epoch_rw = s.step + 9;
    sm.tokens = c.tokens; sm.tok_ld = c.n; sm.tok_col_from_step = 1; sm.logits_out = c.logits_out; sm.logits_out_ld = c.n;
    sm.emb_table = h->dec.tok_emb; sm.emb_C = c.DD; sm.x_next = s.x; sm.pos_table = c.pos; sm.pos_scale = c.pos_scale; sm.pos_rows = c.n;
    sm.y_next = qkv0 ? nullptr : s.y; sm.y_gamma = qkv0 ? nullptr : h->dec.self_[0].ln_g; sm.y_dtype = h->at;
    sm.qkv0_table = qkv0; sm.qkv0_out = s.qkv; sm.qkv0_N = 3 * c.inner;
    if (c.r->kv0) { sm.hist = s.hist; sm.hist_ld = c.T; }
    sm.prompt = c.forced; sm.prompt_ld = pr.ld; sm.prompt_max = pr.Pmax; sm.prompt_len = c.forced_len; sm.prompt_div = c.S;
    return launch_sample(sm, c.st);
}

static int gen_step(const StepCtx& c) {
    int pending = 0;
    for (int l = 0; l < c.h->decg.depth; ++l) {
        DIMX_TRY(attention_half(c, l, &pending));
        DIMX_TRY(feed_forward(c, l, &pending));
    }
    int nlg = 0;
    DIMX_TRY(logits(c, pending, &nlg));
    return c.r->beam ? finish_beam(c, nlg) : finish_sample(c, nlg);
}

static int resolve_route(dimx_handle h, const GenCall& gc, int G, int rows, StepRoute& r) {
    const GenRequest& q = gc.req;
    const DecGeom& dg = h->decg;
    r = StepRoute{};
    r.G = G;
    r.S = q.S;
    r.beam = q.beam;
    r.fault_inject = h->chain_fault_inject > 0;
    r.chain = gen_use_chain(h, rows, q.S);
    r.defer = r.chain && h->defer_ln && h->chain_stats_dev && h->dec.cross[0].q_ln.w && h->dec.ff[0].f1_ln.w;
    r.logits_chain = r.chain && !h->dec.logits.bias;
    r.multi_tr = gen_multi_tr(h, q.S);
    r.win = h->xwin_on != 0;
    r.lookahead = r.win ? h->xwin_lookahead : 0;
    if (G == 1 && qkv0_table_supported(h)) {
        DIMX_TRY(qkv0_table_alloc(h));
        r.qkv0 = h->qkv0_table;
    }
    if (r.qkv0 && h->use_kv0_table && !q.beam && q.pr.step0 == 0 && q.pr.Pmax <= 1 && dg.dim_head == 64 && dg.num_tokens <= 512)
        r.kv0 = h->at == DIMX_BF16 ? h->kv0_image : (const void*)h->qkv0_table;
    if (h->use_layer_chain && r.chain && r.defer && q.S == 1 && 4 * dg.depth + 1 <= kChainSites && !r.win) {
        const StepCtx c = step_ctx(h, gc, r, 0, rows, 0, q.st);
        for (int l = 0; l < dg.depth; ++l) {
            LayerChainArgs lc;
            memset(&lc, 0, sizeof(lc));
            r.layer_kernel[l] = layer_args(c, l, self_args(c, l, 1), cross_args(c, l), lc) && layer_chain_supported(lc, h->cu_count);
        }
    }
    return DIMX_OK;
}

static GraphKey graph_key(dimx_handle h, const GenCall& gc, const StepRoute& r) {
    const GenRequest& q = gc.req;
    GraphKey k{};
    k.ws = q.ws; k.B = q.B; k.T = q.T; k.top_k = gc.top_k;
    k.noise = q.noise; k.start = q.pr.tok; k.mask = q.ctx_mask; k.tokens = q.tokens; k.logits_out = q.logits_out;
    k.G = r.G; k.S = r.S;
    k.chain = r.chain; k.defer = r.defer; k.logits_chain = r.logits_chain; k.multi_tr = r.multi_tr; k.fault_inject = r.fault_inject;
    for (int l = 0; l < 8; ++l) k.layer_kernel |= r.layer_kernel[l] ? 1u << l : 0u;
    k.qkv0 = r.qkv0; k.kv0 = r.kv0;
    k.prompt_len = q.pr.len; k.ld_prompt = q.pr.ld; k.Pmax = q.pr.Pmax;
    k.filter_kind = h->filter_kind;
    k.beam = q.beam ? *q.beam : BeamCall{};
    k.xwin_on = r.win ? 1 : 0; k.xwin_lookahead = r.lookahead;
    return k;
}

static int gen_prefill(dimx_handle h, const CtxPersist& cp, const GenScratch& gs, const PrefillScratch& s, const GenPrompt& pr,
                       const uint8_t* ctx_mask, int B, int T, int S, int32_t* tokens, hipStream_t st, const int* win = nullptr,
                       int n_keys = 0) {
    const DecGeom& dg = h->decg;
    const int n0 = pr.step0, M = B * n0, DD = dg.dim, heads = dg.heads, D = dg.dim_head;
    const int np = tpad(n0), Tp = tpad(T), V = dg.num_tokens;
    DIMX_TRY(launch_prompt_rows(pr.tok, pr.ld, B, n0, V, S, s.inp, tokens, gen_steps(h, T), st));
    DIMX_TRY(launch_gather_rows(DIMX_F32, h->dec.tok_emb, DD, V, s.inp, s.h, DD, M, DD, st));
    const bool rowv = qkv_row_v(h->at, D);
    for (int l = 0; l < dg.depth; ++l) {
        AttnArgs a;
        DIMX_TRY(self_attn_qkv(h, s, h->dec.self_[l].ln_g, nullptr, h->dec.self_[l].qkv, B, n0, DD, heads, D, a, st));
        DIMX_TRY(launch_kv_rows_to_cache(h->at, s.k, gs.sk[l], B, n0, heads, T, S, st));
        if (rowv)
            DIMX_TRY(launch_kv_rows_to_cache(h->at, s.vt, gs.sv[l], B, n0, heads, T, S, st));
        else
            DIMX_TRY(launch_kv_vt_to_cache((const float*)s.vt, np, (float*)gs.sv[l], B, n0, heads, T, S, st));
        if (l == dg.depth - 1) break;
        a.scale = 1.0f / sqrtf((float)D); a.causal = 1;
        DIMX_TRY(attn_out(h, s, a, h->dec.self_[l].out, DD, st));
        if (win) {
            const XAttn& x = h->dec.cross[l];
            float* qf = win_q_rows(s, B, n0, heads * D, es_of(h));
            DIMX_REQUIRE(qf, DIMX_ERR_WORKSPACE, "generate: no room for the windowed prefill's f32 queries");
            DIMX_TRY(launch_layernorm(h->at, s.h, s.y, x.ln_g, nullptr, M, DD, st));
            DIMX_TRY(linear(h, s.y, DD, x.qkv, M, DIMX_F32, qf, heads * D, st));
            WinAttnArgs w;
            w.dtype = h->at;
            w.q = qf; w.ld = heads * D;
            w.kcache = cp.ck[l]; w.vcache = cp.cv[l]; w.Tp = Tp;
            w.out = s.o; w.o_ld = heads * D;
            w.B = B; w.H = heads; w.Lq = n0; w.t0 = 0; w.n_keys = n_keys; w.lookahead = *win;
            w.kmask = ctx_mask; w.kmask_ld = T;
            w.scale = 1.0f / sqrtf((float)D);
            DIMX_TRY(launch_win_attn(w, st));
            DIMX_TRY(residual_linear(h, s.o, heads * D, x.out, M, s.h, DD, st));
            DIMX_TRY(ff_sublayer(h, s, h->dec.ff[l].ln_g, nullptr, h->dec.ff[l].f1, h->dec.ff[l].f2, nullptr, ACT_GELU_ERF, M, DD, st));
            continue;
        }
        set_attn_packed(a, h->at, s.q, cp.ck[l], rowv ? cp.cv[l] : s.cvt, s.o, B, heads, n0, T, D, Tp, rowv);
        a.k_sb = (long)heads * Tp * D; a.k_sh = (long)Tp * D; a.k_st = D;
        if (rowv) { a.v_sb = a.k_sb; a.v_sh = a.k_sh; a.v_st = D; }
        DIMX_TRY(cross_attn_sublayer(h, s, h->dec.cross[l], a, ctx_mask, DD, st, rowv ? nullptr : (const float*)cp.cv[l]));
        DIMX_TRY(ff_sublayer(h, s, h->dec.ff[l].ln_g, nullptr, h->dec.ff[l].f1, h->dec.ff[l].f2, nullptr, ACT_GELU_ERF, M, DD, st));
    }
    return DIMX_OK;
}

static int chain_state_ensure(dimx_handle h) {
    if (!(h->use_chain && h->at == DIMX_BF16 && !h->chain_err_dev)) return DIMX_OK;
    DIMX_HIP(hipMalloc((void**)&h->chain_err_dev, 64));
    DIMX_HIP(hipMemset(h->chain_err_dev, 0, 64));
    DIMX_HIP(hipMalloc((void**)&h->chain_stats_dev, 8 * 32 * 32 * 2 * sizeof(float)));
    DIMX_HIP(hipMemset(h->chain_stats_dev, 0, 8 * 32 * 32 * 2 * sizeof(float)));
    DIMX_HIP(hipHostMalloc((void**)&h->chain_err_host, 64, hipHostMallocDefault));
    *h->chain_err_host = 0;
    DIMX_HIP(hipEventCreateWithFlags(&h->chain_err_ev, hipEventDisableTiming));
    return DIMX_OK;
}

static int gen_groups_fork(dimx_handle h, int G, hipStream_t st, hipStream_t* gs) {
    if (G == 1) {
        gs[0] = st;
        return DIMX_OK;
    }
    if (!h->ev_fork) DIMX_HIP(hipEventCreateWithFlags(&h->ev_fork, hipEventDisableTiming));
    DIMX_HIP(hipEventRecord(h->ev_fork, st));
    for (int g = 0; g < G; ++g) {
        if (!h->grp_stream[g]) DIMX_HIP(hipStreamCreateWithFlags(&h->grp_stream[g], hipStreamNonBlocking));
        if (!h->ev_join[g]) DIMX_HIP(hipEventCreateWithFlags(&h->ev_join[g], hipEventDisableTiming));
        gs[g] = h->grp_stream[g];
        DIMX_HIP(hipStreamWaitEvent(gs[g], h->ev_fork, 0));
    }
    return DIMX_OK;
}

// ... 305 lines not shown
    const int S = n_samples < 1 ? 1 : n_samples;
    const bool win_prefill = h->xwin_on && (flags & 2) && !(flags & 1);
    const int p0 = ((flags & 1) || (h->xwin_on && !win_prefill)) ? 1 : P0;
    DIMX_REQUIRE(!(flags & 4) || p0 >= 2, DIMX_ERR_ARG, "generate_prompted: flags bit 2 (the prefill stage alone) without a prefill (P0=%d, flags 0x%x)",
                 P0, flags);
    DIMX_REQUIRE(p0 == 1 || h->decg.dim_head == 64, DIMX_ERR_ARG, "generate_prompted: the prefill needs 64-wide heads");
    DIMX_REQUIRE(B >= 1 && T <= h->d.max_seq_len, DIMX_ERR_ARG, "B=%d T=%d out of range (T <= %d)", B, T, h->d.max_seq_len);
    const size_t need = workspace_bytes_prompt(h, B, T, S, p0);
    DIMX_REQUIRE(ws_bytes >= need, DIMX_ERR_WORKSPACE, "generate_prompted: workspace %zu < required %zu (dimx_workspace_bytes_prompt)",
                 ws_bytes, need);
    const GenRequest q{{prompt, ld_prompt, Pmax, prompt_len, p0 - 1, win_prefill && p0 >= 2}, ctx_mask, B, T, S, temperature, top_k, exp_noise, seed,
                       tokens, logits_out, ws, ws_bytes, (hipStream_t)stream, nullptr};
    if (flags & 4) {
        StepRoute route;
        return generate_impl(h, q, false, true, &route);
    }
    return generate_checked(h, q);
}

int dimx_generate_beam(dimx_handle h, const int32_t* prompt, int ld_prompt, const int32_t* prompt_len, int Pmax, int P0,
                       const uint8_t* ctx_mask, const int32_t* lens, int B, int T, int beam_width, int32_t* tokens, double* scores,
                       int32_t* backptr, float* logits_out, void* beam_state, size_t beam_state_bytes, int flags, void* ws, size_t ws_bytes,
                       void* stream) {
    DIMX_REQUIRE(h, DIMX_ERR_ARG, "null handle");
    DIMX_NO_SESSION(h, "generate_beam");
    DIMX_REQUIRE(h->variant == 0, DIMX_ERR_ARG, "generate_beam: beam search is implemented for variant 0 (SLMFT) only; this handle is variant %d",
                 h->variant);
    DIMX_REQUIRE(!h->xwin_on, DIMX_ERR_ARG, "generate_beam: not available while the cross-attention window is on (dimx_set_cross_lookahead)");
    DIMX_REQUIRE(beam_width_supported(beam_width), DIMX_ERR_ARG, "generate_beam: beam_width %d not in {1,2,4,5,8,10}", beam_width);
    DIMX_REQUIRE(prompt && scores && T >= 2 && Pmax >= 1 && Pmax <= T - 1 && ld_prompt >= Pmax, DIMX_ERR_ARG,
                 "generate_beam: need scores, 1 <= Pmax <= T - 1 and ld_prompt >= Pmax (Pmax=%d T=%d ld_prompt=%d)", Pmax, T, ld_prompt);
    DIMX_REQUIRE(P0 >= 1 && P0 <= Pmax, DIMX_ERR_ARG, "generate_beam: need 1 <= P0 <= Pmax (P0=%d Pmax=%d)", P0, Pmax);
    DIMX_REQUIRE((flags & ~1) == 0, DIMX_ERR_ARG, "generate_beam: unknown flags 0x%x", flags);
    DIMX_REQUIRE(B >= 1 && T <= h->d.max_seq_len, DIMX_ERR_ARG, "B=%d T=%d out of range (T <= %d)", B, T, h->d.max_seq_len);
    const size_t R = (size_t)B * beam_width;
    DIMX_REQUIRE(beam_state && ((uintptr_t)beam_state % 8) == 0 && beam_state_bytes >= DIMX_BEAM_STATE_BYTES(B, beam_width), DIMX_ERR_ARG,
                 "generate_beam: the beam state needs %zu bytes, 8-byte aligned (DIMX_BEAM_STATE_BYTES); got %zu", (size_t)DIMX_BEAM_STATE_BYTES(B, beam_width),
                 beam_state_bytes);
    const int p0 = (flags & 1) ? 1 : P0;
    DIMX_REQUIRE(p0 == 1 || h->decg.dim_head == 64, DIMX_ERR_ARG, "generate_beam: the prefill needs 64-wide heads");
    const size_t need = workspace_bytes_prompt(h, B, T, beam_width, p0);
    DIMX_REQUIRE(ws_bytes >= need, DIMX_ERR_WORKSPACE, "generate_beam: workspace %zu < required %zu (dimx_workspace_bytes_prompt)", ws_bytes, need);
    BeamCall bm;
    bm.cum = (double*)beam_state;
    bm.parent = (int32_t*)((double*)beam_state + R);
    bm.backptr = backptr;
    bm.lens = lens;
    const GenRequest q{{prompt, ld_prompt, Pmax, prompt_len, p0 - 1}, ctx_mask, B, T, beam_width, 0.f, 0, nullptr, 0,
                       tokens, logits_out, ws, ws_bytes, (hipStream_t)stream, &bm};
    DIMX_TRY(generate_checked(h, q));
    DIMX_HIP(hipMemcpyAsync(scores, bm.cum, R * sizeof(double), hipMemcpyDeviceToDevice, (hipStream_t)stream));
    return DIMX_OK;
}

int dimx_set_sampler_filter(dimx_handle h, int kind, float a, float b) {
    DIMX_REQUIRE(h, DIMX_ERR_ARG, "null handle");
    DIMX_TRY(check_sampler_filter(kind, a, b));
    h->filter_kind = kind;
    h->filter_a = kind == DIMX_FILTER_TOP_K ? 0.f : a;
    h->filter_b = kind == DIMX_FILTER_TOP_A ? b : 0.f;
    return DIMX_OK;
}

int dimx_set_cross_lookahead(dimx_handle h, int on, int lookahead) {
    DIMX_REQUIRE(h, DIMX_ERR_ARG, "null handle");
    DIMX_NO_SESSION(h, "set_cross_lookahead");
    DIMX_REQUIRE(h->variant == 0, DIMX_ERR_ARG, "set_cross_lookahead: online generation is implemented for variant 0 (SLMFT) only; this handle is variant %d",
                 h->variant);
    h->xwin_on = on ? 1 : 0;
    h->xwin_lookahead = on ? lookahead : 0;
    return DIMX_OK;
}

int dimx_cross_lookahead(dimx_handle h, int* on, int* lookahead) {
    DIMX_REQUIRE(h, DIMX_ERR_ARG, "null handle");
    if (on) *on = h->xwin_on;
    if (lookahead) *lookahead = h->xwin_lookahead;
    return DIMX_OK;
}

int dimx_chain_faults(dimx_handle h) { return h ? h->chain_faults : 0; }
int dimx_qkv0_table_builds(dimx_handle h) { return h ? h->qkv0_builds : 0; }
int dimx_kv0_table_generations(dimx_handle h) { return h ? h->kv0_generations : 0; }

int dimx_debug_chain_fault(dimx_handle h, int n_calls) {
    DIMX_REQUIRE(h && n_calls >= 0, DIMX_ERR_ARG, "debug_chain_fault: bad argument");
    h->chain_fault_inject = n_calls;
    h->graph_valid = false;
    return DIMX_OK;
}

}
```

### dyadic-interaction-modeling_amd/csrc/model.hip

```cpp
#include <stdarg.h>
#include <stdlib.h>
#include <set>

#include "stages.hpp"

namespace dimx {

static thread_local char g_err[1024] = "";
void set_error(const char* fmt, ...) {
    va_list ap;
    va_start(ap, fmt);
    vsnprintf(g_err, sizeof(g_err), fmt, ap);
    va_end(ap);
}
const char* get_error() { return g_err; }

static std::string vq_prefix(int which) { return which == 0 ? "speaker_vq." : "listener_vq."; }

struct KeySpec {
    std::string name;
    std::vector<int64_t> shape;
};

static void vq_keys(const dimx_dims& d, int which, std::vector<KeySpec>& out) {
// ... 762 lines not shown

}

using namespace dimx;

extern "C" {

int dimx_version(void) { return 100; }
const char* dimx_last_error(void) { return get_error(); }

void dimx_legacy_dims(dimx_dims* d) {
    if (!d) return;
    dimx_default_dims(d);
    d->variant = 1;
    d->dim_in = 1024; d->dim = 512; d->dim_a = 0; d->enc_depth = 6; d->dec_depth = 6; d->heads = 8;
    d->max_seq_len = 1024;
    d->spk_in_dim = 824; d->spk_hidden = 768; d->spk_heads = 8; d->spk_inter = 1536; d->spk_face_quan_num = 8;
}

void dimx_default_dims(dimx_dims* d) {
    if (!d) return;
    memset(d, 0, sizeof(*d));
    d->vq_in_dim = 56; d->vq_hidden = 384; d->vq_layers = 6; d->vq_heads = 8; d->vq_inter = 1536;
    d->vq_n_embed = 512; d->vq_zdim = 128;
    d->dim_in = 56; d->dim = 384; d->dim_a = 768; d->enc_depth = 4; d->dec_depth = 4; d->heads = 12;
    d->dim_head = 64; d->num_tokens = 512; d->max_seq_len = 2048; d->ff_mult = 4;
}

int dimx_create(dimx_handle* h, int device_id, const dimx_dims* dims, int numeric_mode) {
    DIMX_REQUIRE(h, DIMX_ERR_ARG, "dimx_create: null handle pointer");
    DIMX_REQUIRE(numeric_mode == DIMX_MODE_PARITY_F32 || numeric_mode == DIMX_MODE_PERF_BF16, DIMX_ERR_ARG,
                 "dimx_create: numeric_mode %d", numeric_mode);
    dimx_dims d;
    dimx_default_dims(&d);
    if (dims) d = *dims;
    DIMX_REQUIRE(d.vq_hidden == 384 && d.vq_heads == 8 && d.vq_zdim == 128 && d.vq_n_embed == 512 && d.vq_in_dim == 56,
                 DIMX_ERR_ARG, "dimx_create: only the DIM-Listener VQ geometry (56/384/8/128/512) is built");
    if (d.variant == 0 || d.variant == 2) {
        DIMX_REQUIRE(d.dim == 384 && d.dim_a == 768 && d.dim_head == 64 && d.heads == 12 && d.num_tokens == 512 &&
                         d.vq_layers <= 8 && d.enc_depth <= 8 && d.dec_depth <= 8 && d.max_seq_len <= 2048,
                     DIMX_ERR_ARG, "dimx_create: only the SLMFT geometry (384+768, 12x64, 512 tokens) is built");
    } else {
        DIMX_REQUIRE(d.variant == 1 && d.dim == 512 && d.dim_a == 0 && d.dim_head == 64 && d.heads == 8 &&
                         d.num_tokens == 512 && d.enc_depth <= 8 && d.dec_depth <= 8 && d.max_seq_len <= 2048 &&
                         d.spk_hidden == 768 && d.spk_heads == 8 && d.spk_in_dim == 824 && d.spk_face_quan_num == 8,
                     DIMX_ERR_ARG, "dimx_create: only the legacy ListenerGenerator geometry (824/768 VQ, 512, 8x64) is built");
    }
    DIMX_REQUIRE(d.mesh_dim == 0 || (d.variant == 2 && d.mesh_dim > 0), DIMX_ERR_ARG,
                 "dimx_create: the mesh head (mesh_dim %d) belongs to a handle of variant 2", d.mesh_dim);
    int ndev = 0;
    DIMX_HIP(hipGetDeviceCount(&ndev));
    DIMX_REQUIRE(device_id >= 0 && device_id < ndev, DIMX_ERR_ARG, "dimx_create: device %d of %d", device_id, ndev);
    DIMX_HIP(hipSetDevice(device_id));
    dimx_ctx* c = new dimx_ctx();
    c->device = device_id;
    c->d = d;
    c->mode = numeric_mode;
    c->at = numeric_mode == DIMX_MODE_PERF_BF16 ? DIMX_BF16 : DIMX_F32;
    c->variant = d.variant;
    const VQGeom lvq = {d.vq_in_dim, 64, d.vq_hidden, d.vq_heads, d.vq_inter, d.vq_layers, d.vq_zdim, 1, d.vq_zdim,
                        d.vq_n_embed, true};
    c->vqg[0] = c->vqg[1] = lvq;
    if (d.variant == 1) {
        c->vqg[0] = {d.spk_in_dim, (d.spk_in_dim + 63) / 64 * 64, d.spk_hidden, d.spk_heads, d.spk_inter, d.vq_layers,
                     d.spk_face_quan_num * d.vq_zdim, d.spk_face_quan_num, d.vq_zdim, d.vq_n_embed, false};
        const int din = d.spk_face_quan_num * d.vq_zdim;
        c->encg[0] = c->encg[1] = {din, din, d.dim, d.heads, d.dim_head, d.enc_depth, d.ff_mult, 0};
        c->decg = {d.dim, d.heads, d.dim_head, d.dec_depth, d.ff_mult, 1, d.num_tokens, d.dim};
    } else {
        const int causal = d.variant == 2 ? 0 : 1, abs_pos = d.variant == 2 ? 1 : 0;
        c->encg[0] = {d.dim_in, 64, d.dim, d.heads, d.dim_head, d.enc_depth, d.ff_mult, causal};
        c->encg[1] = {d.dim, d.dim, d.dim, d.heads, d.dim_head, d.enc_depth, d.ff_mult, causal};
        c->decg = {d.dim + d.dim_a, d.heads, d.dim_head, d.dec_depth, d.ff_mult, abs_pos, d.num_tokens, d.dim + d.dim_a};
    }
    for (const auto& k : all_keys(d)) c->required.push_back(k.name);
    const char* ng = getenv("DIMX_NO_GRAPH");
    c->use_graph = (ng && ng[0] == '1') ? 0 : 1;
    const char* nc = getenv("DIMX_NO_CHAIN");
    c->use_chain = (nc && nc[0] == '1') ? 0 : 1;
    c->use_layer_chain = getenv("DIMX_NO_LAYER_CHAIN") ? 0 : 1;
    c->multi_tr = getenv("DIMX_NO_MULTI_TR") ? 0 : 1;
    c->use_qkv0_table = getenv("DIMX_NO_QKV0_TABLE") ? 0 : 1;
    c->use_kv0_table = getenv("DIMX_NO_KV0_TABLE") ? 0 : 1;
    if (getenv("DIMX_LAYER_PROF")) {
        void* p = nullptr;
        if (hipMalloc(&p, (size_t)8 * 256 * 16 * 8) == hipSuccess) {
            (void)hipMemset(p, 0, (size_t)8 * 256 * 16 * 8);
            c->layer_prof_dev = (unsigned long long*)p;
        }
    }
    if (const char* pg = getenv("DIMX_PREFILL_GROUPS")) {
        const int v = atoi(pg);
        if (v >= 1 && v <= dimx_ctx::kPreGroups) c->prefill_groups = v;
    }
    {
        int cus = 0;
        if (hipDeviceGetAttribute(&cus, hipDeviceAttributeMultiprocessorCount, device_id) == hipSuccess) c->cu_count = cus;
    }
    const char* gg = getenv("DIMX_GEN_GROUPS");
    if (gg && atoi(gg) >= 1 && atoi(gg) <= dimx_ctx::kMaxGroups) c->gen_groups = atoi(gg);
    *h = c;
    return DIMX_OK;
}

int dimx_destroy(dimx_handle h) {
    if (!h) return DIMX_OK;
    (void)hipSetDevice(h->device);
    for (int g = 0; g < dimx_ctx::kMaxGroups; ++g) {
        if (h->graph_multi[g]) (void)hipGraphExecDestroy(h->graph_multi[g]);
        if (h->graph_exec[g]) (void)hipGraphExecDestroy(h->graph_exec[g]);
        if (h->grp_stream[g]) (void)hipStreamDestroy(h->grp_stream[g]);
        if (h->ev_join[g]) (void)hipEventDestroy(h->ev_join[g]);
    }
    if (h->ev_fork) (void)hipEventDestroy(h->ev_fork);
    for (int g = 0; g < dimx_ctx::kPreGroups - 1; ++g) {
        if (h->pre_stream[g]) (void)hipStreamDestroy(h->pre_stream[g]);
        if (h->pre_join[g]) (void)hipEventDestroy(h->pre_join[g]);
    }
    if (h->pre_fork) (void)hipEventDestroy(h->pre_fork);
    if (h->cap_stream) (void)hipStreamDestroy(h->cap_stream);
    if (h->chain_err_ev) (void)hipEventDestroy(h->chain_err_ev);
    if (h->chain_err_dev) (void)hipFree(h->chain_err_dev);
    if (h->chain_stats_dev) (void)hipFree(h->chain_stats_dev);
    if (h->layer_prof_dev) (void)hipFree(h->layer_prof_dev);
    if (h->qkv0_table) (void)hipFree(h->qkv0_table);
    if (h->kv0_image) (void)hipFree(h->kv0_image);
    if (h->chain_err_host) (void)hipHostFree(h->chain_err_host);
    free_packed(h);
    stream_forget(h);
    train_forget(h);
    delete h;
    return DIMX_OK;
}

int dimx_numeric_mode(dimx_handle h) { return h ? h->mode : DIMX_ERR_ARG; }

int dimx_set_shard(dimx_handle h, int row_offset, int rows_total) {
    DIMX_REQUIRE(h, DIMX_ERR_ARG, "set_shard: null handle");
    DIMX_REQUIRE(row_offset >= 0 && (rows_total == 0 || rows_total > row_offset), DIMX_ERR_ARG,
                 "set_shard: row_offset %d, rows_total %d", row_offset, rows_total);
    h->shard_row_off = row_offset;
    h->shard_rows_total = rows_total;
    return DIMX_OK;
}

int dimx_begin_checkpoint(dimx_handle h) {
    DIMX_REQUIRE(h, DIMX_ERR_ARG, "dimx_begin_checkpoint: null handle");
    std::set<std::string> spec;
    for (const auto& k : all_keys(h->d)) spec.insert(k.name);
    bool dirty = false;
    for (auto it = h->host.begin(); it != h->host.end();) {
        if (!spec.count(it->first)) {
            it = h->host.erase(it);
            dirty = true;
        } else {
            ++it;
        }
    }
    if (dirty) {
        (void)hipSetDevice(h->device);
        (void)hipDeviceSynchronize();
        free_packed(h);
        h->graph_valid = false;
        h->ctx_ready = false;
    }
    return DIMX_OK;
}

int dimx_load_weights(dimx_handle h, const dimx_weight_desc* descs, int n) {
    DIMX_REQUIRE(h && descs && n >= 0, DIMX_ERR_ARG, "dimx_load_weights: null argument");
    static thread_local std::map<std::string, std::vector<int64_t>> spec;
    spec.clear();
    for (const auto& k : all_keys(h->d)) spec[k.name] = k.shape;
    bool dirty = false;
    for (int i = 0; i < n; ++i) {
        const dimx_weight_desc& w = descs[i];
        DIMX_REQUIRE(w.name && w.data && w.ndim >= 1 && w.ndim <= 4, DIMX_ERR_ARG, "dimx_load_weights: bad desc %d", i);
        const std::string name(w.name);
        auto it = spec.find(name);
        if (it == spec.end()) {
            std::vector<int64_t> oshape;
            const int opt = optional_key(spec, name, &oshape);
            if (opt != OPT_NONE) {
                DIMX_REQUIRE(w.ndim == 1 && w.shape[0] == oshape[0], DIMX_ERR_WEIGHT, "%s: expected %lld values", w.name, (long long)oshape[0]);
                if (opt == OPT_NORM_BIAS) {
                    for (int64_t k = 0; k < w.shape[0]; ++k)
                        DIMX_REQUIRE(w.data[k] == 0.f, DIMX_ERR_WEIGHT,
                                     "%s: a non-zero LayerNorm bias -- this x-transformers variant is not the one the path implements", w.name);
                    continue;
                }
                HostTensor& t = h->host[name];
                t.shape.assign(w.shape, w.shape + 1);
                t.data.assign(w.data, w.data + w.shape[0]);
                dirty = true;
                continue;
            }
            DIMX_REQUIRE(ignorable_key(name), DIMX_ERR_WEIGHT, "unknown weight key %s", w.name);
            if (name == "speaker_embed.weight" && w.ndim == 2 && w.shape[1] == h->d.dim && w.shape[0] >= 1 && w.shape[0] <= (1 << 20))
                h->spk_embed_rows = (int)w.shape[0];
            continue;
        }
        DIMX_REQUIRE((int)it->second.size() == w.ndim, DIMX_ERR_WEIGHT, "%s: rank %d, expected %d", w.name, w.ndim,
                     (int)it->second.size());
        size_t cnt = 1;
        for (int k = 0; k < w.ndim; ++k) {
            DIMX_REQUIRE(it->second[k] == w.shape[k], DIMX_ERR_WEIGHT, "%s: dim %d is %lld, expected %lld", w.name, k,
                         (long long)w.shape[k], (long long)it->second[k]);
            cnt *= (size_t)w.shape[k];
        }
// ... 808 lines not shown
```

### dyadic-interaction-modeling_amd/csrc/model.hpp

```cpp
#pragma once
#include <map>
#include <string>
#include <vector>

#include "common.hpp"

namespace dimx {

struct Linear {
    void* w = nullptr;
    const float* bias = nullptr;
    int N = 0, K = 0, Kp = 0;
    void* w3 = nullptr;
};

struct VQBlock {
    const float *ln1_g, *ln1_b, *ln2_g, *ln2_b;
    Linear qkv, out, l1, l2;
    const void* mlp = nullptr;
};

struct VQNet {
    Linear vm, conv, le, post;
    VQBlock enc[8];
// ... 12 lines not shown
    Linear kv;
    Linear out;
    Linear q_ln;
    const float* q_ln_colsum = nullptr;
};
struct XFF {
    const float* ln_g;
    Linear f1, f2;
    Linear f1_ln;
    const float* f1_ln_colsum = nullptr;
    const void* mlp = nullptr;
};
struct XEnc {
    Linear proj_in;
    const float* pos_emb = nullptr;
    XAttn attn[8];
    XFF ff[8];
    const float* final_g = nullptr;
};
struct XDec {
    const float* tok_emb = nullptr;
    const float* pos_emb = nullptr;
    XAttn self_[8], cross[8];
    XFF ff[8];
    const float* final_g = nullptr;
    Linear logits;
    Linear cross_kv_all;
};

struct MeshHead {
    const float *w_ih[2][2], *w_hh[2][2], *b_ih[2][2], *b_hh[2][2];
    Linear l1, l2;
};

struct VQGeom {
    int in_dim, in_pad, hidden, heads, inter, layers, out_dim, fqn, zdim, n_embed;
    bool has_decoder;
};
struct EncGeom {
    int dim_in, in_pad, dim, heads, dim_head, depth, ff_mult, causal;
};
struct DecGeom {
    int dim, heads, dim_head, depth, ff_mult, abs_pos, num_tokens, ctx_dim;
};

struct HostTensor {
    std::vector<float> data;
    std::vector<int64_t> shape;
};

struct Arena {
    unsigned char* base;
    size_t off;
    size_t cap;
    bool overflow;
    Arena(void* b, size_t c) : base((unsigned char*)b), off(0), cap(c), overflow(false) {}
    void* take(size_t bytes) {
        off = align_up(off, 256);
        void* p = base ? base + off : nullptr;
        off += bytes;
        if (base && off > cap) overflow = true;
        return p;
    }
};

struct BeamCall {
    double* cum = nullptr;
    int32_t* parent = nullptr;
    int32_t* backptr = nullptr;
    const int32_t* lens = nullptr;
    bool operator==(const BeamCall& o) const { return cum == o.cum && parent == o.parent && backptr == o.backptr && lens == o.lens; }
};

struct StepRoute {
    bool chain = false;
    bool defer = false;
    bool layer_kernel[8] = {};
    bool logits_chain = false;
    bool multi_tr = false;
    bool win = false;
    int lookahead = 0;
    const float* qkv0 = nullptr;
    const void* kv0 = nullptr;
    const BeamCall* beam = nullptr;
    bool fault_inject = false;
    int G = 1, S = 1;
};

struct GraphKey {
    void* ws;
    int B, T, top_k;
    const void *noise, *start, *mask, *tokens, *logits_out;
    int G, S;
    bool chain, defer, logits_chain, multi_tr, fault_inject;
    unsigned layer_kernel;
    const void *qkv0, *kv0;
    const void* prompt_len;
    int ld_prompt, Pmax;
    int filter_kind;
    BeamCall beam;
    int xwin_on, xwin_lookahead;
    bool operator==(const GraphKey& o) const {
        return ws == o.ws && B == o.B && T == o.T && top_k == o.top_k && noise == o.noise && start == o.start && mask == o.mask &&
               tokens == o.tokens && logits_out == o.logits_out && G == o.G && S == o.S && chain == o.chain && defer == o.defer &&
               logits_chain == o.logits_chain && multi_tr == o.multi_tr && fault_inject == o.fault_inject &&
               layer_kernel == o.layer_kernel && qkv0 == o.qkv0 && kv0 == o.kv0 && prompt_len == o.prompt_len &&
               ld_prompt == o.ld_prompt && Pmax == o.Pmax && filter_kind == o.filter_kind && beam == o.beam && xwin_on == o.xwin_on &&
               xwin_lookahead == o.xwin_lookahead;
    }
};

}

namespace dimx {
int vq_pe_buffers(dimx_ctx* c, int which, const float** pe_enc, const float** pe_dec);
void train_forget(dimx_ctx* h);
void stream_forget(dimx_ctx* h);
}

struct dimx_ctx {
    int device = 0;
    dimx_dims d;
    int variant = 0;
    dimx::VQGeom vqg[2];
    dimx::EncGeom encg[2];
    dimx::DecGeom decg;
    int mode = 0;
    int at = DIMX_F32;
    std::map<std::string, dimx::HostTensor> host;
    std::vector<std::string> required;
    int packed_mask = 0;
    std::vector<void*> dev_allocs;
    dimx::VQNet vq[2];
    dimx::XEnc enc_s, enc_joint, enc_l;
    dimx::XDec dec;
    const float *patch_s = nullptr, *patch_dec_s = nullptr, *norm_s_g = nullptr, *norm_s_b = nullptr;
    const float *patch_l = nullptr, *patch_dec_l = nullptr, *norm_l_g = nullptr, *norm_l_b = nullptr;
    const float *norm_j_g = nullptr, *norm_j_b = nullptr;
    bool ctx_ready = false;
    int ctx_B = 0, ctx_T = 0, ctx_for_generate = 0;
    void* ctx_ws = nullptr;
    static constexpr int kMaxGroups = 8;
    hipGraphExec_t graph_exec[kMaxGroups] = {};
    hipGraphExec_t graph_multi[kMaxGroups] = {};
    int graph_unroll = 16;
    static constexpr int kPreGroups = 4;
    int prefill_groups = 0;
    hipStream_t pre_stream[kPreGroups - 1] = {};
    hipEvent_t pre_fork = nullptr, pre_join[kPreGroups - 1] = {};
    hipStream_t grp_stream[kMaxGroups] = {};
    hipEvent_t ev_fork = nullptr, ev_join[kMaxGroups] = {};
    int gen_groups = 1;
    hipStream_t cap_stream = nullptr;
    dimx::GraphKey graph_key{};
    bool graph_valid = false;
    int use_graph = 1;
    int use_chain = 1;
    int cu_count = 0;
    float* chain_stats_dev = nullptr;
    int defer_ln = 1;
    unsigned long long* layer_prof_dev = nullptr;
    int multi_tr = 1;
    int use_layer_chain = 1;
    unsigned* chain_err_dev = nullptr;
    unsigned* chain_err_host = nullptr;
    hipEvent_t chain_err_ev = nullptr;
    int chain_faults = 0;
    int chain_fault_inject = 0;
    int use_qkv0_table = 1;
    float* qkv0_table = nullptr;
    int qkv0_M = 0, qkv0_at = -1;
    uint64_t qkv0_epoch = 0;
    uint64_t dec_epoch = 1;
    int qkv0_builds = 0;
    int use_kv0_table = 1;
    void* kv0_image = nullptr;
    int kv0_generations = 0;
    int shard_row_off = 0, shard_rows_total = 0;
    int filter_kind = 0;
    float filter_a = 0.f, filter_b = 0.f;
    int xwin_on = 0, xwin_lookahead = 0;
    int twin_on = 0, twin_lookahead = 0;
    void* stream_sess = nullptr;
    dimx::MeshHead mesh;
    int lstm_faults = 0;
    int spk_embed_rows = 0;
};
```

### dyadic-interaction-modeling_amd/engine.py

```python
import ctypes

import numpy as np
import torch

from . import lib as L
from . import sampling


class Engine:
    def __init__(self, device=None, mode=L.MODE_PARITY_F32, variant="slmft", mesh_dim=0):
        if not torch.cuda.is_available():
            raise L.DimxError("dimx needs a ROCm GPU (torch.cuda.is_available() is False); "
                              "there is no CPU fallback")
        self.device = torch.device(device if device is not None else "cuda:0")
        if self.device.index is None:
            self.device = torch.device("cuda", torch.cuda.current_device())
        self.lib = L.load()
        self.mode = mode
        assert variant in ("slmft", "legacy", "slm", "speaker")
        self.variant = variant
        if variant == "speaker":
            assert mesh_dim > 0, "the speaker variant needs mesh_dim"
            self.dims = L.speaker_dims(mesh_dim)
        else:
# ... 258 lines not shown
                           return_logits, n_samples, return_scores=False):
        B, Pmax = prompt.shape
        R = B * n_samples
        prompt = prompt.to(torch.int32).contiguous()
        prompt_len = prompt_len.to(torch.int32).contiguous() if prompt_len is not None else None
        window = False
        if isinstance(prefill, str) or isinstance(prefill, tuple):
            kind, prefill = (prefill, None) if isinstance(prefill, str) else prefill
            if kind != "window":
                raise ValueError("prefill=%r: an integer P0, 'window' or ('window', P0)" % (kind,))
            window = True
        P0 = int(prefill) if prefill is not None else (Pmax if prompt_len is None else 1)
        if noise is not None:
            noise = noise.to(torch.float32).contiguous()
            assert tuple(noise.shape) == (self.n_gen(T), R, self.dims.num_tokens)
        self._chk(prompt, prompt_len, mask_u8, noise)
        n = self.n_gen(T)
        tokens = torch.empty(R, n, dtype=torch.int32, device=self.device)
        lg = torch.empty(R, n, self.dims.num_tokens, dtype=torch.float32, device=self.device) if (return_logits or return_scores) else None
        ws, wsb = self.workspace(B, T, n_samples)
        L.check(self.lib.dimx_generate_prompted(self.h, L.ptr(prompt), int(prompt.stride(0)), L.ptr(prompt_len), int(Pmax), P0,
                                                L.ptr(mask_u8), B, T, int(n_samples), float(temperature), int(top_k), L.ptr(noise),
                                                int(seed) & 0xFFFFFFFFFFFFFFFF, L.ptr(tokens), L.ptr(lg),
                                                (1 if no_prefill else 0) | (2 if window else 0), ws, wsb, self._s()), "dimx_generate_prompted")
        plen = None
        if return_scores:
            no_prefill = no_prefill or (self.cross_lookahead() is not None and not window)
            plen = prompt_len.clamp(1 if no_prefill else P0, Pmax) if prompt_len is not None \
                else torch.full((B,), Pmax, dtype=torch.int32, device=self.device)
        return self._generated(tokens, lg, mask_u8, T, n_samples, plen, return_logits, return_scores)

    def generate_beam(self, start, mask_u8, T, beam_width, prompt=None, prompt_len=None, prefill=None, return_logits=False,
                      return_backptr=False):
        W = int(beam_width)
        if prompt is None:
            prompt, prompt_len, prefill = start.reshape(-1, 1), None, 1
        B, Pmax = prompt.shape
        R = B * W
        prompt = prompt.to(torch.int32).contiguous()
        prompt_len = prompt_len.to(torch.int32).contiguous() if prompt_len is not None else None
        P0 = int(prefill) if prefill is not None else (Pmax if prompt_len is None else 1)
        lens = mask_u8.sum(1, dtype=torch.int32)
        self._chk(prompt, prompt_len, mask_u8)
        n = self.n_gen(T)
        tokens = torch.empty(R, n, dtype=torch.int32, device=self.device)
        scores = torch.empty(R, dtype=torch.float64, device=self.device)
        lg = torch.empty(R, n, self.dims.num_tokens, dtype=torch.float32, device=self.device) if return_logits else None
        bp = torch.empty(R, n, dtype=torch.int32, device=self.device) if return_backptr else None
        state = torch.empty(2 * R, dtype=torch.float64, device=self.device)
        ws, wsb = self.workspace(B, T, W)
        L.check(self.lib.dimx_generate_beam(self.h, L.ptr(prompt), int(prompt.stride(0)), L.ptr(prompt_len), int(Pmax), P0,
                                            L.ptr(mask_u8), L.ptr(lens), B, T, W, L.ptr(tokens), L.ptr(scores), L.ptr(bp), L.ptr(lg),
                                            L.ptr(state), state.numel() * 8, 0, ws, wsb, self._s()), "dimx_generate_beam")
        return (tokens, scores) + ((lg,) if return_logits else ()) + ((bp,) if return_backptr else ())

    def mesh_head(self, motion, template=None, safe=False, out=None):
        B, Lq, _ = motion.shape
        V = self.dims.mesh_dim
        motion = motion.to(torch.float32).contiguous()
        template = template.to(torch.float32).contiguous() if template is not None else None
        if template is not None:
            assert tuple(template.shape) == (B, V), "template must be [B, mesh_dim]"
        if out is None:
            out = torch.empty(B, Lq, V, dtype=torch.float32, device=self.device)
        assert tuple(out.shape) == (B, Lq, V) and out.dtype == torch.float32
        self._chk(motion, template, out)
        ws, wsb = self.workspace(B, Lq)
        L.check(self.lib.dimx_mesh_head(self.h, L.ptr(motion), L.ptr(template), B, Lq, L.ptr(out), 1 if safe else 0, ws, wsb,
                                        self._s()), "dimx_mesh_head")
        return out

    def lstm_faults(self):
        return int(self.lib.dimx_lstm_faults(self.h))

    def chain_faults(self):
        return int(self.lib.dimx_chain_faults(self.h))

    def qkv0_table_builds(self):
        return int(self.lib.dimx_qkv0_table_builds(self.h))

    def kv0_table_generations(self):
        return int(self.lib.dimx_kv0_table_generations(self.h))

    def debug_chain_fault(self, n_calls=1):
        L.check(self.lib.dimx_debug_chain_fault(self.h, int(n_calls)), "dimx_debug_chain_fault")


class StreamSession:

    def __init__(self, eng, B, Tmax, start, lookahead=0, temperature=1.0, top_k=52, noise=None, seed=0, prompt=None, v_speaker=None,
                 v_audio=None):
        self.eng, self.B, self.Tmax, self.lookahead = eng, int(B), int(Tmax), int(lookahead)
        self._open = False
        lib, dev = eng.lib, eng.device
        need = lib.dimx_stream_workspace_bytes(eng.h, self.B, self.Tmax)
        if need == 0:
            raise L.DimxError("dimx_stream_workspace_bytes(%d,%d) = 0: sessions need the SLMFT variant and 2 <= Tmax <= 2048" % (B, Tmax))
        self._ws = torch.empty(need + 256, dtype=torch.uint8, device=dev)
        self._V = eng.dims.num_tokens
        self._tok = torch.zeros(self.B, self.Tmax - 1, dtype=torch.int32, device=dev)
        self._lg = None
        self.begin(start, temperature, top_k, noise, seed, prompt, v_speaker, v_audio)

    def _ws_ptr(self):
        base = self._ws.data_ptr()
        aligned = (base + 255) // 256 * 256
        return ctypes.c_void_p(aligned), self._ws.numel() - (aligned - base)

    def begin(self, start=None, temperature=1.0, top_k=52, noise=None, seed=0, prompt=None, v_speaker=None, v_audio=None):
        if self._open:
            raise L.DimxError("StreamSession.begin: the session is open (end() or close() first)")
        if noise is not None:
            noise = noise.to(torch.float32).contiguous()
            assert tuple(noise.shape) == (self.Tmax - 1, self.B, self._V)
        if prompt is not None:
            return self._begin_prompted(prompt, v_speaker, v_audio, temperature, top_k, noise, seed)
        start = start.to(torch.int32).contiguous()
        self.eng._chk(start, noise)
        assert tuple(start.shape) == (self.B,)
        self._noise = noise
        self._last = (0, 0)
        ws, wsb = self._ws_ptr()
        L.check(self.eng.lib.dimx_stream_begin(self.eng.h, L.ptr(start), self.B, self.Tmax, self.lookahead, float(temperature), int(top_k),
                                               L.ptr(self._noise), int(seed) & 0xFFFFFFFFFFFFFFFF, ws, wsb, self.eng._s()),
                "dimx_stream_begin")
        self._open = True
        self.frames = 0
        self.steps = 0

    def _begin_prompted(self, prompt, v_speaker, v_audio, temperature, top_k, noise, seed):
        from . import stream as _stream
        prompt = prompt.to(torch.int32).contiguous()
        v_speaker = v_speaker.to(torch.float32).contiguous()
        v_audio = v_audio.to(torch.float32).contiguous()
        self.eng._chk(prompt, v_speaker, v_audio, noise)
        B, P = prompt.shape
        F = v_speaker.shape[1]
        assert B == self.B and v_speaker.shape[0] == B and tuple(v_audio.shape[:2]) == (B, F)
        if not _stream.prompt_fits(P, self.lookahead, F, self.Tmax):
            raise ValueError("a session cannot start from P=%d codes and F=%d frames: need 1 <= P and P + max(lookahead, 0) = %d <= F <= Tmax = %d"
                             % (P, F, P + max(self.lookahead, 0), self.Tmax))
        need = self.eng.lib.dimx_stream_workspace_bytes_prompt(self.eng.h, self.B, self.Tmax)
        if self._ws.numel() < need + 256:
            self._ws = None
            self._ws = torch.empty(need + 256, dtype=torch.uint8, device=self.eng.device)
        self._noise = noise
        ws, wsb = self._ws_ptr()
        L.check(self.eng.lib.dimx_stream_begin_prompted(self.eng.h, L.ptr(prompt), P, P, L.ptr(v_speaker), L.ptr(v_audio), F, self.B, self.Tmax,
                                                        self.lookahead, float(temperature), int(top_k), L.ptr(self._noise),
                                                        int(seed) & 0xFFFFFFFFFFFFFFFF, ws, wsb, self.eng._s()), "dimx_stream_begin_prompted")
        self._open = True
        self.frames = F
        self.steps = P - 1
        self._last = (P - 1, P - 1)
        self._tok[:, :P - 1] = prompt[:, 1:]
        if self._lg is not None:
            self._lg[:, :P - 1] = 0

    def _logits(self):
        if self._lg is None:
            self._lg = torch.zeros(self.B, self.Tmax - 1, self._V, dtype=torch.float32, device=self.eng.device)
        return self._lg

    def _took(self, n_new, return_logits, extra=()):
        lo, hi = self.steps, self.steps + n_new
        self.steps = hi
# ... 983 lines not shown
```

### dyadic-interaction-modeling_amd/lib.py

```python
import ctypes
import os
from ctypes import (POINTER, c_char_p, c_float, c_int, c_int32, c_int64, c_size_t, c_uint64,
                    c_void_p)

import torch

HERE = os.path.dirname(os.path.abspath(__file__))
LIB_PATH = os.environ.get("DIMX_LIB", os.path.join(HERE, "libdimx_hip.so"))

MODE_PARITY_F32 = 0
MODE_PERF_BF16 = 1
F32, BF16 = 0, 1
ACT_NONE, ACT_LEAKY, ACT_GELU_TANH, ACT_GELU_ERF = 0, 1, 2, 3


class DimxError(RuntimeError):
    pass


class Dims(ctypes.Structure):
    _fields_ = [(n, c_int) for n in (
        "vq_in_dim", "vq_hidden", "vq_layers", "vq_heads", "vq_inter", "vq_n_embed", "vq_zdim",
        "dim_in", "dim", "dim_a", "enc_depth", "dec_depth", "heads", "dim_head", "num_tokens",
        "max_seq_len", "ff_mult", "variant", "spk_in_dim", "spk_hidden", "spk_heads", "spk_inter",
# ... 32 lines not shown
    "dimx_cross_lookahead": (c_int, [c_void_p, POINTER(c_int), POINTER(c_int)]),
    "dimx_stream_workspace_bytes": (c_size_t, [c_void_p, c_int, c_int]),
    "dimx_stream_begin": (c_int, [c_void_p, c_void_p, c_int, c_int, c_int, c_float, c_int, c_void_p, c_uint64, c_void_p, c_size_t,
                                  c_void_p]),
    "dimx_stream_workspace_bytes_prompt": (c_size_t, [c_void_p, c_int, c_int]),
    "dimx_stream_begin_prompted": (c_int, [c_void_p, c_void_p, c_int, c_int, c_void_p, c_void_p, c_int, c_int, c_int, c_int, c_float, c_int,
                                           c_void_p, c_uint64, c_void_p, c_size_t, c_void_p]),
    "dimx_stream_push": (c_int, [c_void_p, c_void_p, c_void_p, c_int, c_void_p, c_int, c_void_p, c_void_p, POINTER(c_int), c_void_p]),
    "dimx_stream_end": (c_int, [c_void_p, c_void_p, c_int, c_void_p, POINTER(c_int), c_void_p]),
    "dimx_stream_abort": (c_int, [c_void_p]),
    "dimx_stream_state": (c_int, [c_void_p, POINTER(c_int), POINTER(c_int), POINTER(c_int)]),
    "dimx_stream_set_events": (c_int, [c_void_p, c_void_p, c_void_p, c_void_p, c_void_p]),
    "dimx_encode_ctx": (c_int, [c_void_p, c_void_p, c_void_p, c_void_p, c_int, c_int, c_int, c_void_p,
                                c_void_p, c_size_t, c_void_p]),
    "dimx_legacy_speaker_features": (c_int, [c_void_p, c_void_p, c_void_p, c_int, c_int, c_void_p, c_void_p,
                                             c_void_p, c_size_t, c_void_p]),
    "dimx_slm_encode": (c_int, [c_void_p, c_void_p, c_void_p, c_void_p, c_void_p, c_void_p, c_int, c_int, c_void_p,
                                c_void_p, c_void_p, c_void_p, c_size_t, c_void_p]),
    "dimx_set_context": (c_int, [c_void_p, c_void_p, c_int, c_int, c_void_p, c_int, c_int, c_int, c_void_p, c_size_t,
                                 c_void_p]),
    "dimx_decode_tf": (c_int, [c_void_p, c_void_p, c_void_p, c_void_p, c_int, c_int, c_void_p, c_void_p,
                               c_void_p, c_void_p, c_size_t, c_void_p]),
    "dimx_decode_tf_win": (c_int, [c_void_p, c_void_p, c_void_p, c_int, c_int, c_int, c_void_p, c_void_p, c_void_p, c_void_p,
                                   c_size_t, c_void_p]),
    "dimx_generate": (c_int, [c_void_p, c_void_p, c_void_p, c_int, c_int, c_int, c_float, c_int, c_void_p, c_uint64,
                              c_void_p, c_void_p, c_void_p, c_size_t, c_void_p]),
    "dimx_workspace_bytes_prompt": (c_size_t, [c_void_p, c_int, c_int, c_int, c_int]),
    "dimx_generate_prompted": (c_int, [c_void_p, c_void_p, c_int, c_void_p, c_int, c_int, c_void_p, c_int, c_int, c_int, c_float,
                                       c_int, c_void_p, c_uint64, c_void_p, c_void_p, c_int, c_void_p, c_size_t, c_void_p]),
    "dimx_generate_beam": (c_int, [c_void_p, c_void_p, c_int, c_void_p, c_int, c_int, c_void_p, c_void_p, c_int, c_int, c_int, c_void_p,
                                   c_void_p, c_void_p, c_void_p, c_void_p, c_size_t, c_int, c_void_p, c_size_t, c_void_p]),
    "dimx_train_num_params": (c_int, [c_void_p]),
    "dimx_train_total": (c_int64, [c_void_p]),
    "dimx_train_param_info": (c_int, [c_void_p, c_int, POINTER(c_char_p), POINTER(c_int64), POINTER(c_int64)]),
    "dimx_train_workspace_bytes": (c_size_t, [c_void_p, c_int, c_int]),
    "dimx_train_forward_backward": (c_int, [c_void_p, c_void_p, c_void_p, c_void_p, c_void_p, c_void_p, c_void_p, c_void_p, c_int,
                                            c_int, c_void_p, c_void_p, c_void_p, c_size_t, c_void_p]),
    "dimx_train_graph_stats": (c_int, [c_void_p, c_void_p]),
    "dimx_set_train_lookahead": (c_int, [c_void_p, c_int, c_int]),
    "dimx_train_lookahead": (c_int, [c_void_p, POINTER(c_int), POINTER(c_int)]),
    "dimx_train_legacy_workspace_bytes": (c_size_t, [c_void_p, c_int, c_int]),
    "dimx_train_legacy_forward_backward": (c_int, [c_void_p, c_void_p, c_void_p, c_void_p, c_void_p, c_void_p, c_void_p, c_void_p, c_void_p,
                                                   c_void_p, c_int, c_int, c_void_p, c_void_p, c_void_p, c_void_p, c_size_t, c_void_p]),
    "dimx_train_slm_workspace_bytes": (c_size_t, [c_void_p, c_int, c_int]),
    "dimx_train_slm_forward_backward": (c_int, [c_void_p] + [c_void_p] * 14 + [c_int, c_int, c_void_p, c_void_p, c_size_t, c_void_p]),
    "dimx_train_vq_num_params": (c_int, [c_void_p, c_int]),
    "dimx_train_vq_total": (c_int64, [c_void_p, c_int]),
    "dimx_train_vq_param_info": (c_int, [c_void_p, c_int, c_int, POINTER(c_char_p), POINTER(c_int64), POINTER(c_int64)]),
    "dimx_train_vq_workspace_bytes": (c_size_t, [c_void_p, c_int, c_int]),
    "dimx_train_vq_forward_backward": (c_int, [c_void_p, c_int, c_void_p, c_void_p, c_void_p, c_int, c_int, c_float, c_float, c_float,
                                               c_uint64, c_int64, c_void_p, c_void_p, c_void_p, c_void_p, c_size_t, c_void_p]),
    "dimx_train_conv_num_params": (c_int, [c_void_p]),
    "dimx_train_conv_total": (c_int64, [c_void_p]),
    "dimx_train_conv_param_info": (c_int, [c_void_p, c_int, POINTER(c_char_p), POINTER(c_int64), POINTER(c_int64)]),
    "dimx_train_conv_workspace_bytes": (c_size_t, [c_void_p, c_int, c_int]),
    "dimx_train_conv_forward_backward": (c_int, [c_void_p, c_void_p, c_void_p, c_void_p, c_void_p, c_void_p, c_void_p, c_int, c_int, c_int,
                                                 c_int, c_void_p, c_void_p, c_void_p, c_size_t, c_void_p]),
    "dimx_train_spk_num_params": (c_int, [c_void_p]),
    "dimx_train_spk_total": (c_int64, [c_void_p]),
    "dimx_train_spk_param_info": (c_int, [c_void_p, c_int, POINTER(c_char_p), POINTER(c_int64), POINTER(c_int64)]),
    "dimx_train_spk_workspace_bytes": (c_size_t, [c_void_p, c_int, c_int]),
    "dimx_train_spk_forward_backward": (c_int, [c_void_p] + [c_void_p] * 9 + [c_int, c_int, c_void_p, c_void_p, c_void_p, c_void_p, c_void_p,
                                                c_size_t, c_void_p]),
    "dimx_op_lstm_layer_bwd": (c_int, [c_int, c_void_p, c_int, c_int, c_int, c_int, POINTER(c_void_p), POINTER(c_void_p),
                                       POINTER(c_void_p), POINTER(c_void_p), c_void_p, c_void_p, POINTER(c_void_p), POINTER(c_void_p),
                                       POINTER(c_void_p), c_int, POINTER(c_int), c_void_p]),
    "dimx_train_adamw": (c_int, [c_void_p, c_void_p, c_void_p, c_void_p, c_int64, c_float, c_float, c_float, c_float, c_float,
                                 c_int, c_float, c_void_p, c_void_p]),
    "dimx_op_train_attention": (c_int, [c_int, c_void_p, c_void_p, c_void_p, c_void_p, c_void_p, c_void_p, c_int, c_int, c_int,
                                        c_int, c_int, c_float, c_void_p, c_void_p, c_void_p, c_void_p, c_void_p, c_void_p,
                                        c_void_p]),
    "dimx_op_train_attention_win": (c_int, [c_int, c_void_p, c_void_p, c_void_p, c_void_p, c_void_p, c_void_p, c_int, c_int, c_int,
                                            c_int, c_int, c_float, c_int, c_int, c_void_p, c_void_p, c_void_p, c_void_p, c_void_p,
                                            c_void_p, c_void_p]),
    "dimx_op_train_layernorm_bwd": (c_int, [c_void_p, c_void_p, c_void_p, c_void_p, c_int, c_int, c_int, c_void_p, c_void_p, c_void_p,
                                            c_size_t, c_void_p]),
    "dimx_op_train_colsum": (c_int, [c_void_p, c_int, c_int, c_void_p, c_void_p, c_size_t, c_void_p]),
    "dimx_op_train_prep": (c_int, [c_int, c_int, c_void_p, c_int, c_void_p, c_int, c_void_p, c_void_p, c_int, c_int, c_void_p, c_size_t,
                                   c_void_p, c_size_t, c_void_p, c_size_t, POINTER(c_int), c_void_p]),
    "dimx_op_train_cross_entropy": (c_int, [c_void_p, c_void_p, c_int, c_void_p, c_void_p, c_void_p, c_void_p]),
    "dimx_chain_faults": (c_int, [c_void_p]),
    "dimx_qkv0_table_builds": (c_int, [c_void_p]),
    "dimx_kv0_table_generations": (c_int, [c_void_p]),
    "dimx_lstm_faults": (c_int, [c_void_p]),
    "dimx_mesh_head": (c_int, [c_void_p, c_void_p, c_void_p, c_int, c_int, c_void_p, c_int, c_void_p, c_size_t, c_void_p]),
    "dimx_op_lstm_layer": (c_int, [c_int, c_void_p, c_int, c_int, c_int, c_int, POINTER(c_void_p), POINTER(c_void_p),
                                   POINTER(c_void_p), POINTER(c_void_p), c_void_p, c_int, POINTER(c_int), c_void_p]),
    "dimx_debug_chain_fault": (c_int, [c_void_p, c_int]),
    "dimx_op_gemm_slabs": (c_int, [c_int, c_int, c_int, c_int, c_int]),
    "dimx_op_split_x3": (c_int, [c_void_p, c_void_p, ctypes.c_long, c_void_p]),
    "dimx_op_gemm_x3": (c_int, [c_void_p, c_int, c_void_p, c_void_p, c_int, c_int, c_int, c_int, c_void_p, c_int, c_void_p, c_int, c_int,
                                c_void_p]),
    "dimx_op_gemm": (c_int, [c_int, c_int, c_void_p, c_int, c_void_p, c_int, c_void_p, c_int, c_int, c_int,
                             c_int, c_void_p, c_int, c_void_p, c_int, c_int, c_void_p, c_int, c_void_p]),
    "dimx_op_gemm_headmajor": (c_int, [c_int, c_void_p, c_int, c_void_p, c_int, c_void_p, c_int, c_int, c_int, c_int, c_int,
                                       c_int, c_void_p]),
    "dimx_op_layernorm": (c_int, [c_int, c_void_p, c_void_p, c_void_p, c_void_p, c_int, c_int, c_void_p]),
    "dimx_op_instnorm": (c_int, [c_int, c_void_p, c_void_p, c_void_p, c_int, c_int, c_int, c_void_p]),
    "dimx_op_attention": (c_int, [c_int, c_void_p, c_void_p, c_void_p, c_void_p, c_int, c_int, c_int, c_int,
                                  c_int, c_int, c_int, c_int, c_int, c_float, c_int, c_void_p, c_void_p,
                                  c_void_p]),
    "dimx_op_attention_rowv": (c_int, [c_void_p, c_void_p, c_void_p, c_void_p, c_int, c_int, c_int, c_int, c_int, c_int, c_int,
                                       c_int, c_int, c_float, c_int, c_void_p, c_void_p, c_void_p]),
    "dimx_op_decode_attn": (c_int, [c_int, c_void_p, c_void_p, c_void_p, c_void_p, c_int, c_int, c_int, c_int,
                                    c_float, c_void_p, c_int, c_int, c_void_p]),
    "dimx_op_append_attn": (c_int, [c_int, c_void_p, c_int, c_void_p, c_void_p, c_void_p, c_int, c_int, c_int, c_int, c_int, c_float,
                                    c_void_p]),
    "dimx_op_cross_attn_win": (c_int, [c_int, c_void_p, c_int, c_void_p, c_void_p, c_int, c_void_p, c_int, c_int, c_int, c_int, c_int, c_int,
                                       c_int, c_void_p, c_int, c_float, c_void_p]),
    "dimx_op_decode_attn_self": (c_int, [c_int, c_void_p, c_int, c_void_p, c_void_p, c_void_p, c_int, c_int, c_int,
                                         c_void_p, c_float, c_int, c_void_p]),
    "dimx_op_decode_attn_ex": (c_int, [c_int, c_void_p, c_int, c_int, c_int, ctypes.c_long, c_int, c_void_p, c_void_p, c_void_p,
                                       c_int, c_int, c_int, c_int, c_void_p, c_int, c_void_p, c_int, c_int, c_float, c_int,
                                       c_void_p]),
    "dimx_op_decode_attn_win": (c_int, [c_int, c_void_p, c_int, c_int, c_int, ctypes.c_long, c_void_p, c_void_p, c_void_p,
                                        c_int, c_int, c_int, c_int, c_void_p, c_int, c_void_p, c_int, c_int, c_float, c_int,
                                        c_int, c_void_p]),
    "dimx_op_decode_attn_tab": (c_int, [c_int, c_void_p, c_int, c_int, c_int, ctypes.c_long, c_void_p, c_void_p, c_void_p, c_int, c_int,
                                        c_int, c_int, c_void_p, c_float, c_int, c_void_p, c_int, c_int, c_int, c_int, c_void_p, c_int,
                                        c_void_p]),
    "dimx_op_mlp_fused": (c_int, [c_void_p, c_void_p, c_void_p, c_void_p, c_void_p, c_void_p, c_void_p, c_int, c_int, c_int, c_int, c_void_p]),
    "dimx_mlp_fused_packed_bytes": (c_size_t, [c_int, c_int]),
    "dimx_mlp_fused_pack": (c_int, [c_void_p, c_void_p, c_void_p, c_int, c_int, c_void_p, c_size_t]),
    "dimx_op_mlp_fused_packed": (c_int, [c_void_p, c_void_p, c_void_p, c_void_p, c_void_p, c_int, c_int, c_int, c_int, c_void_p]),
    "dimx_op_add_slabs_layernorm": (c_int, [c_int, c_void_p, c_void_p, c_int, ctypes.c_long, c_void_p, c_void_p, c_int,
                                            c_int, c_void_p]),
    "dimx_op_chain": (c_int, [c_void_p, c_int, c_void_p, c_void_p, c_void_p, c_int, c_void_p, c_void_p, c_void_p, c_int,
                              c_void_p, c_int, c_int, c_void_p, c_void_p]),
    "dimx_op_chain_ln": (c_int, [c_void_p, c_int, c_void_p, c_void_p, c_void_p, c_void_p, c_void_p, c_void_p, c_int,
                                 c_void_p, c_int, c_int, c_void_p, c_void_p]),
    "dimx_op_layer_chain": (c_int, [c_void_p, c_int, ctypes.c_long, c_void_p, c_void_p, c_int, c_void_p, c_void_p, c_int, c_int, c_void_p,
                                    c_void_p, c_void_p, c_void_p, c_void_p, c_void_p, c_void_p, c_void_p, c_void_p, c_void_p, c_int,
                                    c_void_p, c_int, c_float, c_void_p, c_void_p, c_void_p]),
    "dimx_op_layer_chain_tab": (c_int, [c_void_p, c_int, ctypes.c_long, c_void_p, c_void_p, c_int, c_void_p, c_void_p, c_int, c_int, c_void_p,
                                        c_void_p, c_void_p, c_void_p, c_void_p, c_void_p, c_void_p, c_void_p, c_void_p, c_void_p, c_int,
                                        c_void_p, c_int, c_float, c_void_p, c_void_p, c_void_p, c_int, c_int, c_int, c_int, c_void_p,
                                        c_int, c_void_p]),
    "dimx_op_gemm_ln": (c_int, [c_int, c_void_p, c_void_p, c_void_p, c_int, c_int, c_int, c_void_p, c_int, c_void_p,
                                c_void_p, c_void_p]),
    "dimx_op_fd_select_ws_bytes": (c_size_t, [c_int, c_int, c_int]),
    "dimx_op_fd_select": (c_int, [c_void_p, ctypes.c_long, ctypes.c_long, c_void_p, ctypes.c_long, ctypes.c_long, ctypes.c_long, c_void_p,
                                  c_int, c_int, c_int, c_int, c_int, c_int, c_void_p, c_void_p, c_void_p, c_void_p, c_void_p, c_size_t,
                                  c_void_p]),
    "dimx_op_mesh_metrics_ws_bytes": (c_size_t, [c_int, c_int, c_int, c_int]),
    "dimx_op_mesh_metrics": (c_int, [c_void_p, ctypes.c_long, ctypes.c_long, c_void_p, ctypes.c_long, ctypes.c_long, c_void_p, ctypes.c_long,
                                     POINTER(c_int32), c_int, c_int, c_int, c_void_p, c_int, c_void_p, c_int, c_void_p, c_void_p, c_void_p,
                                     c_void_p, c_size_t, c_void_p]),
    "dimx_op_listener_metrics_ws_bytes": (c_size_t, [c_int, c_int, c_int]),
    "dimx_op_listener_metrics": (c_int, [c_void_p, ctypes.c_long, ctypes.c_long, c_void_p, ctypes.c_long, ctypes.c_long, c_void_p, ctypes.c_long,
                                         ctypes.c_long, c_void_p, c_int, c_int, c_int, c_int, POINTER(c_int32), c_int, c_void_p, c_void_p,
                                         c_void_p, c_size_t, c_void_p]),
    "dimx_op_kmeans_fit_ws_bytes": (c_size_t, [c_int, c_int, c_int]),
    "dimx_op_kmeans_fit": (c_int, [c_void_p, ctypes.c_long, c_int, c_int, c_int, c_int, c_int, c_int, c_void_p, c_int, ctypes.c_double,
                                   c_int, c_void_p, c_void_p, c_void_p, c_void_p, c_void_p, c_size_t, c_void_p]),
    "dimx_op_sid_assign": (c_int, [c_void_p, ctypes.c_long, c_int, c_int, c_int, c_int, c_void_p, c_int, c_void_p, c_void_p, c_void_p,
                                   c_void_p]),
    "dimx_op_seq_logprob": (c_int, [c_void_p, ctypes.c_long, ctypes.c_long, c_void_p, ctypes.c_long, c_void_p, c_void_p, c_int, c_int,
                                    c_int, c_void_p, c_void_p, c_void_p, c_void_p]),
    "dimx_op_score_select": (c_int, [c_void_p, c_void_p, ctypes.c_long, ctypes.c_long, ctypes.c_long, c_void_p, c_void_p, ctypes.c_long,
                                     c_int, c_int, c_int, c_int, c_int, c_void_p, c_void_p, c_void_p, c_void_p, c_void_p]),
    "dimx_op_consensus_select_ws_bytes": (c_size_t, [c_int, c_int, c_int, c_int]),
    "dimx_op_consensus_select": (c_int, [c_void_p, ctypes.c_long, ctypes.c_long, ctypes.c_long, c_void_p, c_int, c_int, c_int, c_int, c_int,
                                         c_int, c_int, c_void_p, c_void_p, c_void_p, c_void_p, c_void_p, c_void_p, ctypes.c_long, c_int,
                                         c_void_p, c_void_p, c_size_t, c_void_p]),
    "dimx_op_pool_desc": (c_int, [c_void_p, ctypes.c_long, ctypes.c_long, c_void_p, c_int, c_int, c_int, c_int, c_void_p, c_void_p,
                                  c_void_p]),
# ... 94 lines not shown
```

### include/dimx.h

```cpp
#ifndef DIMX_H
#define DIMX_H

#include <stddef.h>
#include <stdint.h>

#ifdef __cplusplus
extern "C" {
#endif

typedef struct dimx_ctx* dimx_handle;

typedef enum {
    DIMX_OK = 0,
    DIMX_ERR_ARG = -1,
    DIMX_ERR_HIP = -2,
    DIMX_ERR_WEIGHT = -3,
    DIMX_ERR_STATE = -4,
    DIMX_ERR_WORKSPACE = -5
} dimx_status;

#define DIMX_MODE_PARITY_F32 0
#define DIMX_MODE_PERF_BF16 1

#define DIMX_F32 0
// ... 33 lines not shown
int dimx_vq_encode(dimx_handle h, int which, const float* x, const int32_t* lens, int B, int T,
                   int pe_mode, int batch_row_offset, int32_t pad_value, int32_t* idx, float* z_out,
                   void* ws, size_t ws_bytes, void* stream);

int dimx_vq_argmin(dimx_handle h, int which, const float* z, int N, int32_t* idx, float* best_d,
                   float* margin, void* stream);

int dimx_vq_decode(dimx_handle h, int which, const int32_t* idx, int B, int L, int batch_row_offset,
                   int rows_per_clip, float* out, void* ws, size_t ws_bytes, void* stream);

int dimx_vq_decode_latent(dimx_handle h, int which, const float* z, int B, int L, int batch_row_offset,
                          float* out, void* ws, size_t ws_bytes, void* stream);

int dimx_encode_speaker(dimx_handle h, const float* v_speaker, const uint8_t* mask, int B, int T,
                        float* x_s_out, void* ws, size_t ws_bytes, void* stream);

int dimx_set_shard(dimx_handle h, int row_offset, int rows_total);

int dimx_encode_ctx(dimx_handle h, const float* v_speaker, const float* v_audio, const uint8_t* mask,
                    int B, int T, int for_generate, float* x_s_out, void* ws, size_t ws_bytes,
                    void* stream);

int dimx_slm_encode(dimx_handle h, const float* v_speaker, const float* v_listener, const uint8_t* mask,
                    const uint8_t* mask_speaker, const uint8_t* mask_listener, int B, int T, float* x_s,
                    float* x_l, float* x_joint, void* ws, size_t ws_bytes, void* stream);

int dimx_set_context(dimx_handle h, const float* x, int ldx_rows, int which_patch, const float* v_audio, int B,
                     int T, int for_generate, void* ws, size_t ws_bytes, void* stream);

int dimx_legacy_speaker_features(dimx_handle h, const float* v_speaker, const uint8_t* mask, int B, int T,
                                 float* x_speaker_out, int32_t* idx_out, void* ws, size_t ws_bytes,
                                 void* stream);

int dimx_decode_tf(dimx_handle h, const int32_t* z_l, const uint8_t* ctx_mask, const uint8_t* kv_mask,
                   int B, int T, float* logits, float* row_loss, int32_t* argmax_tok, void* ws,
                   size_t ws_bytes, void* stream);

int dimx_decode_tf_win(dimx_handle h, const int32_t* z_l, const uint8_t* ctx_mask, int B, int T, int lookahead, float* logits,
                       float* row_loss, int32_t* argmax_tok, void* ws, size_t ws_bytes, void* stream);

int dimx_generate(dimx_handle h, const int32_t* start, const uint8_t* ctx_mask, int B, int T, int n_samples,
                  float temperature, int top_k, const float* exp_noise, uint64_t seed, int32_t* tokens,
                  float* logits_out, void* ws, size_t ws_bytes, void* stream);

size_t dimx_workspace_bytes_prompt(dimx_handle h, int B, int T, int n_samples, int P0);
int dimx_generate_prompted(dimx_handle h, const int32_t* prompt, int ld_prompt, const int32_t* prompt_len, int Pmax, int P0,
                           const uint8_t* ctx_mask, int B, int T, int n_samples, float temperature, int top_k,
                           const float* exp_noise, uint64_t seed, int32_t* tokens, float* logits_out, int flags, void* ws,
                           size_t ws_bytes, void* stream);

#define DIMX_BEAM_STATE_BYTES(B, W) ((size_t)16 * (size_t)(B) * (size_t)(W))
int dimx_generate_beam(dimx_handle h, const int32_t* prompt, int ld_prompt, const int32_t* prompt_len, int Pmax, int P0,
                       const uint8_t* ctx_mask, const int32_t* lens, int B, int T, int beam_width, int32_t* tokens, double* scores,
                       int32_t* backptr, float* logits_out, void* beam_state, size_t beam_state_bytes, int flags, void* ws, size_t ws_bytes,
                       void* stream);

int dimx_chain_faults(dimx_handle h);

typedef enum {
    DIMX_FILTER_TOP_K = 0,
    DIMX_FILTER_TOP_P = 1,
    DIMX_FILTER_MIN_P = 2,
    DIMX_FILTER_TOP_A = 3
} dimx_filter_kind;
int dimx_set_sampler_filter(dimx_handle h, int kind, float a, float b);

int dimx_set_cross_lookahead(dimx_handle h, int on, int lookahead);
int dimx_cross_lookahead(dimx_handle h, int* on, int* lookahead);
size_t dimx_stream_workspace_bytes(dimx_handle h, int B, int Tmax);
int dimx_stream_begin(dimx_handle h, const int32_t* start, int B, int Tmax, int lookahead, float temperature, int top_k, const float* noise,
                      uint64_t seed, void* ws, size_t ws_bytes, void* stream);
size_t dimx_stream_workspace_bytes_prompt(dimx_handle h, int B, int Tmax);
int dimx_stream_begin_prompted(dimx_handle h, const int32_t* prompt, int ld_prompt, int P, const float* v_speaker, const float* v_audio, int F,
                               int B, int Tmax, int lookahead, float temperature, int top_k, const float* noise, uint64_t seed, void* ws,
                               size_t ws_bytes, void* stream);
int dimx_stream_push(dimx_handle h, const float* v_speaker, const float* v_audio, int c, int32_t* tokens_out, int ld_tok, float* logits_out,
                     float* x_s_out, int* n_new, void* stream);
int dimx_stream_end(dimx_handle h, int32_t* tokens_out, int ld_tok, float* logits_out, int* n_new, void* stream);
int dimx_stream_abort(dimx_handle h);
int dimx_stream_state(dimx_handle h, int* frames, int* steps, int* open);
int dimx_stream_set_events(dimx_handle h, void* ev_start, void* ev_encoded, void* ev_appended, void* ev_stepped);
int dimx_qkv0_table_builds(dimx_handle h);
int dimx_kv0_table_generations(dimx_handle h);
int dimx_debug_chain_fault(dimx_handle h, int n_calls);

int dimx_mesh_head(dimx_handle h, const float* motion, const float* templ, int B, int L, float* mesh_out, int flags, void* ws,
                   size_t ws_bytes, void* stream);
int dimx_lstm_faults(dimx_handle h);

int dimx_train_num_params(dimx_handle h);
int64_t dimx_train_total(dimx_handle h);
int dimx_train_param_info(dimx_handle h, int i, const char** name, int64_t* offset, int64_t* numel);
size_t dimx_train_workspace_bytes(dimx_handle h, int B, int T);
int dimx_train_forward_backward(dimx_handle h, const float* params, float* grads, const float* v_speaker, const float* v_audio,
                                const uint8_t* mask, const int32_t* z_l, const uint8_t* kv_mask, int B, int T, float* loss_out,
                                float* logits_out, void* ws, size_t ws_bytes, void* stream);
int dimx_train_graph_stats(dimx_handle h, int64_t* out3);
int dimx_set_train_lookahead(dimx_handle h, int on, int lookahead);
int dimx_train_lookahead(dimx_handle h, int* on, int* lookahead);
size_t dimx_train_legacy_workspace_bytes(dimx_handle h, int B, int T);
int dimx_train_legacy_forward_backward(dimx_handle h, const float* params, float* grads, const float* x_speaker, const int32_t* z_l,
                                       const float* v_listener, const uint8_t* mask, const int32_t* listener_ids, const float* codebook,
                                       const float* pe, int B, int T, float* loss_out, float* pred_out, float* logits_out, void* ws,
                                       size_t ws_bytes, void* stream);
size_t dimx_train_slm_workspace_bytes(dimx_handle h, int B, int T);
int dimx_train_slm_forward_backward(dimx_handle h, const float* params, float* grads, const float* v_speaker, const float* v_listener,
                                    const float* v_audio, const uint8_t* mask, const uint8_t* mask_speaker, const uint8_t* mask_listener,
                                    const int32_t* z_s, const int32_t* z_l, const float* codebook_s, const float* codebook_l,
                                    const float* pe_s, const float* pe_l, int B, int T, float* loss_out, void* ws, size_t ws_bytes,
                                    void* stream);
int dimx_train_vq_num_params(dimx_handle h, int which);
int64_t dimx_train_vq_total(dimx_handle h, int which);
int dimx_train_vq_param_info(dimx_handle h, int which, int i, const char** name, int64_t* offset, int64_t* numel);
size_t dimx_train_vq_workspace_bytes(dimx_handle h, int B, int T);
int dimx_train_vq_forward_backward(dimx_handle h, int which, const float* params, float* grads, const float* x, int B, int T, float beta,
                                   float quant_loss_weight, float dropout_p, uint64_t dropout_seed, int64_t step, float* loss_out,
                                   float* pred_out, int32_t* idx_out, void* ws, size_t ws_bytes, void* stream);
int dimx_train_conv_num_params(dimx_handle h);
int64_t dimx_train_conv_total(dimx_handle h);
int dimx_train_conv_param_info(dimx_handle h, int i, const char** name, int64_t* offset, int64_t* numel);
size_t dimx_train_conv_workspace_bytes(dimx_handle h, int B, int T);
int dimx_train_conv_forward_backward(dimx_handle h, const float* params, float* grads, const float* motion, const float* templ,
                                     const float* target, const float* vert_w, int n_mouth, int B, int T, int flags, float* loss_out,
                                     float* mesh_out, void* ws, size_t ws_bytes, void* stream);
int dimx_train_spk_num_params(dimx_handle h);
int64_t dimx_train_spk_total(dimx_handle h);
int dimx_train_spk_param_info(dimx_handle h, int i, const char** name, int64_t* offset, int64_t* numel);
size_t dimx_train_spk_workspace_bytes(dimx_handle h, int B, int T);
int dimx_train_spk_forward_backward(dimx_handle h, const float* params, float* grads, const float* v_emoca, const float* v_audio,
                                    const uint8_t* mask, const int32_t* z, const int32_t* speaker_ids, const float* codebook_s,
                                    const float* pe_s, int B, int T, float* loss_out, float* logits_out, int32_t* idx_out, float* pred_out,
                                    void* ws, size_t ws_bytes, void* stream);
int dimx_op_lstm_layer_bwd(int dtype, const float* x, int B, int T, int In, int H, const float* const* w_ih, const float* const* w_hh,
                           const float* const* b_ih, const float* const* b_hh, const float* dy, float* dx, float* const* dw_ih,
                           float* const* dw_hh, float* const* db, int flags, int* faults_out, void* stream);
int dimx_train_adamw(float* params, const float* grads, float* exp_avg, float* exp_avg_sq, int64_t n, float lr, float beta1,
                     float beta2, float eps, float weight_decay, int step, float max_norm, float* scratch, void* stream);
int dimx_op_train_attention(int mfma, const float* q, const float* k, const float* v, const float* d_o, const uint8_t* kmask,
                            const uint8_t* kmask2, int B, int H, int Lq, int Lk, int causal, float scale, float* o, float* lse,
                            float* delta, float* dq, float* dk, float* dv, void* stream);
int dimx_op_train_attention_win(int mfma, const float* q, const float* k, const float* v, const float* d_o, const uint8_t* kmask,
                                const uint8_t* kmask2, int B, int H, int Lq, int Lk, int causal, float scale, int win, int lookahead,
                                float* o, float* lse, float* delta, float* dq, float* dk, float* dv, void* stream);
int dimx_op_train_layernorm_bwd(const float* x, const float* gamma, const float* dy, float* dx, int accumulate, int M, int C, float* dgamma,
                                float* dbeta, float* scratch, size_t scratch_floats, void* stream);
int dimx_op_train_colsum(const float* dy, int M, int C, float* out, float* scratch, size_t scratch_floats, void* stream);
int dimx_op_train_prep(int dtype, int mode, const float* src, int lds, const float* src2, int lds2, const float* gamma, const float* beta,
                       int rows, int cols, void* o, size_t o_elems, void* t, size_t t_elems, float* colpart, size_t colpart_floats,
                       int* dims3, void* stream);
int dimx_op_train_cross_entropy(const float* logits, const int32_t* targets, int R, float* row_loss, float* dlogits, float* loss_out2,
                                void* stream);


int dimx_op_gemm(int in_dtype, int out_dtype, const void* A, int lda, const void* W, int ldw, void* C,
                 int ldc, int M, int N, int K, const float* bias, int act, const float* residual,
                 int ldr, int conv_T, const int32_t* conv_lens, int flags, void* stream);
int dimx_op_split_x3(const float* w, void* planes, long n, void* stream);
int dimx_op_gemm_x3(const float* A, int lda, const void* planes, float* C, int ldc, int M, int N, int K, const float* bias, int act,
                    const float* residual, int ldr, int flags, void* stream);
int dimx_op_gemm_slabs(int in_dtype, int M, int N, int K, int flags);
int dimx_op_gemm_headmajor(int dtype, const void* A, int lda, const void* W, int ldw, void* out, int M, int N, int K,
                           int rowT, int Tp, int nlayers, void* stream);
int dimx_op_lstm_layer(int dtype, const float* x, int B, int T, int In, int H, const float* const* w_ih, const float* const* w_hh,
                       const float* const* b_ih, const float* const* b_hh, float* y, int flags, int* faults_out, void* stream);
int dimx_op_layernorm(int out_dtype, const float* x, void* y, const float* gamma, const float* beta,
                      int M, int C, void* stream);
// ... 104 lines not shown
```

Before: 1728 clips/s.

## Precompute first-layer self-attention score table over token pairs

Layer 0's self-attention query and key depend only on the token id, so a per-head table of scaled q·k scores for every pair of vocabulary tokens (plus the self-score) is built once per weight epoch. The decode attention kernel then reads scores from that table via a row load and a cross-lane permute instead of loading K rows and computing dot products. It also skips gathering the qkv row into the workspace and reads V straight from the table. This adds H*V*512 floats of memory and a table-build kernel, and applies only when the vocabulary is at most 512 and the kv0 table path is active.

```diff
diff --git a/dyadic-interaction-modeling_amd/csrc/chain.hip b/dyadic-interaction-modeling_amd/csrc/chain.hip
--- a/dyadic-interaction-modeling_amd/csrc/chain.hip
+++ b/dyadic-interaction-modeling_amd/csrc/chain.hip
@@ -864,6 +864,7 @@
                          (uintptr_t)a.sa.tab % 16 == 0,
                      DIMX_ERR_ARG, "layer_chain: table form with rows of %d, K at %d, V at %d, history stride %d", a.sa.tab_ld, a.sa.tab_koff,
                      a.sa.tab_voff, a.sa.hist_ld);
+        DIMX_REQUIRE(!a.sa.s0 || decode_attn_s0_args_ok(a.sa), DIMX_ERR_ARG, "layer_chain: score-table form without its tables");
         (void)hipFuncSetAttribute((const void*)xcd_layer_kernel<2, 1, 2, true>, hipFuncAttributeMaxDynamicSharedMemorySize, (int)kMaxDynLds);
         hipLaunchKernelGGL((xcd_layer_kernel<2, 1, 2, true>), dim3(8 * kGroupCUs), dim3(kLayerThreads), lds, s, a);
         DIMX_HIP(hipGetLastError());
diff --git a/dyadic-interaction-modeling_amd/csrc/common.hpp b/dyadic-interaction-modeling_amd/csrc/common.hpp
--- a/dyadic-interaction-modeling_amd/csrc/common.hpp
+++ b/dyadic-interaction-modeling_amd/csrc/common.hpp
@@ -328,8 +328,14 @@
     const int32_t* hist;
     int hist_ld;
     int win, lookahead;
-};
+    const float* s0;
+    const float* s0new;
+    const float* qkv0_v;
+    int qkv0_ld;
+};
+constexpr int kS0Ld = 512;
 int launch_decode_attn(const DecodeAttnArgs& a, hipStream_t s);
+bool decode_attn_s0_args_ok(const DecodeAttnArgs& a);
 
 int launch_vq_argmin(const float* z, int N, const float* Et , const float* ee ,
                      int32_t* idx, float* best_d, float* margin, hipStream_t s);
@@ -508,6 +514,8 @@
 int launch_gather_start_rows(const float* table, int N, int rows, const int32_t* start, int start_div, float* out, int B,
                              hipStream_t s, int start_ld = 1, int32_t* hist = nullptr, int hist_ld = 0);
 int launch_kv0_image(const float* table, int ld, int rows, int col0, int W, void* image, hipStream_t s);
+int launch_s0_table(int dtype, const float* table, int ld, int rows, int H, const void* ktab, int k_ld, int k_off, float scale,
+                    float* s0, float* s0new, hipStream_t s);
 int launch_gen_params(int32_t* base, int groups, float temperature, uint64_t seed, int row_off, int rows_total,
                       hipStream_t s, int step0 = 0, float filter_a = 0.f, float filter_b = 0.f);
 int launch_embed_step(const float* table, int C, int rows, const int32_t* start, const int32_t* tokens, int tok_ld,
diff --git a/dyadic-interaction-modeling_amd/csrc/decode_attn.hip b/dyadic-interaction-modeling_amd/csrc/decode_attn.hip
--- a/dyadic-interaction-modeling_amd/csrc/decode_attn.hip
+++ b/dyadic-interaction-modeling_amd/csrc/decode_attn.hip
@@ -136,6 +136,55 @@
     }
 }
 
+template <typename T>
+__global__ __launch_bounds__(256) void s0_table_kernel(const float* __restrict__ table, int ld, int rows, int H,
+                                                       const T* __restrict__ ktab, int k_ld, int k_off, float scale,
+                                                       float* __restrict__ s0, float* __restrict__ s0new) {
+    constexpr int EPC = 16 / sizeof(T);
+    constexpr int LPK = 64 / EPC;
+    constexpr int KPI = 64 / LPK;
+    const int a = blockIdx.x, h = blockIdx.y;
+    const int wave = threadIdx.x >> 6, lane = threadIdx.x & 63;
+    const int sub = lane / LPK, ch = lane % LPK;
+    const float scale2 = attn_scale2(scale);
+    float qv[EPC], knv[EPC];
+    load_f32_chunk<EPC>(table + (size_t)a * ld + h * 64 + ch * EPC, qv);
+    load_f32_chunk<EPC>(table + (size_t)a * ld + H * 64 + h * 64 + ch * EPC, knv);
+    float* row = s0 + ((size_t)h * rows + a) * kS0Ld;
+    for (int b0 = wave * KPI; b0 < kS0Ld; b0 += 4 * KPI) {
+        const int b = b0 + sub;
+        const uint4 u = *(const uint4*)(ktab + (size_t)(b < rows ? b : rows - 1) * k_ld + k_off + h * 64 + ch * EPC);
+        float kv[EPC];
+        cvt_chunk<T, EPC>(u, kv);
+        const float sv = key_score<EPC>(qv, kv, scale2);
+        if (ch == 0) row[b] = b < rows ? sv : 0.f;
+    }
+    if (wave == 0) {
+        const float sv = key_score<EPC>(qv, knv, scale2);
+        if (lane == 0) s0new[(size_t)h * rows + a] = sv;
+    }
+}
+
+}
+
+int launch_s0_table(int dtype, const float* table, int ld, int rows, int H, const void* ktab, int k_ld, int k_off, float scale,
+                    float* s0, float* s0new, hipStream_t s) {
+    const int epc = dtype == DIMX_BF16 ? 8 : 4;
+    DIMX_REQUIRE(table && ktab && s0 && s0new && rows >= 1 && rows <= kS0Ld && H >= 1 && ld % 4 == 0 && ld >= 2 * H * 64 &&
+                     k_ld % epc == 0 && k_off % epc == 0 && k_off >= 0 && k_off + H * 64 <= k_ld && (uintptr_t)ktab % 16 == 0 &&
+                     (uintptr_t)table % 16 == 0,
+                 DIMX_ERR_ARG, "s0_table: %d rows of %d, %d heads, K rows of %d at %d", rows, ld, H, k_ld, k_off);
+    if (dtype == DIMX_BF16)
+        hipLaunchKernelGGL(s0_table_kernel<bf16>, dim3(rows, H), dim3(256), 0, s, table, ld, rows, H, (const bf16*)ktab, k_ld, k_off, scale, s0, s0new);
+    else
+        hipLaunchKernelGGL(s0_table_kernel<float>, dim3(rows, H), dim3(256), 0, s, table, ld, rows, H, (const float*)ktab, k_ld, k_off, scale, s0, s0new);
+    DIMX_HIP(hipGetLastError());
+    return DIMX_OK;
+}
+
+bool decode_attn_s0_args_ok(const DecodeAttnArgs& a) {
+    return a.tab && a.s0new && a.qkv0_v && a.tab_rows <= kS0Ld && a.qkv0_ld % 4 == 0 && a.qkv0_ld >= a.H * 64 &&
+           (uintptr_t)a.s0 % 16 == 0 && (uintptr_t)a.qkv0_v % 16 == 0;
 }
 
 int launch_decode_attn(const DecodeAttnArgs& a, hipStream_t s) {
@@ -152,6 +201,8 @@
                          a.tab_koff + a.H * 64 <= a.tab_ld && a.tab_voff + a.H * 64 <= a.tab_ld && (uintptr_t)a.tab % 16 == 0,
                      DIMX_ERR_ARG, "decode_attn: table rows of %d with K at %d and V at %d", a.tab_ld, a.tab_koff, a.tab_voff);
     }
+    DIMX_REQUIRE(!a.s0 || decode_attn_s0_args_ok(a), DIMX_ERR_ARG, "decode_attn: the score-table form needs the table form, at most %d ids, "
+                 "s0new and the q/k/v table's V columns", kS0Ld);
     DIMX_REQUIRE(!a.win || (a.knew == nullptr && a.step != nullptr && !a.tab), DIMX_ERR_ARG,
                  "decode_attn: the windowed form is cross attention with a step counter");
     if (a.rows_per_clip > 1) {
diff --git a/dyadic-interaction-modeling_amd/csrc/decode_attn_body.hpp b/dyadic-interaction-modeling_amd/csrc/decode_attn_body.hpp
--- a/dyadic-interaction-modeling_amd/csrc/decode_attn_body.hpp
+++ b/dyadic-interaction-modeling_amd/csrc/decode_attn_body.hpp
@@ -74,6 +74,16 @@
 #pragma unroll
         for (int e = 0; e < EPC; ++e) v[e] += t[e];
     }
+}
+
+__device__ __forceinline__ float attn_scale2(float scale) { return scale * 1.4426950408889634f; }
+
+template <int EPC> __device__ __forceinline__ float key_score(const float (&qv)[EPC], const float (&kv)[EPC], float scale2) {
+    float d = 0.f;
+#pragma unroll
+    for (int e = 0; e < EPC; ++e) d = fmaf(qv[e], kv[e], d);
+    d = 64 / EPC == 8 ? group8_sum(d) : row16_sum(d);
+    return d * scale2;
 }
 
 template <typename T, bool SELF, bool QF32, int NSPLIT, int NW, bool QSC1 = false, bool TAB = false, bool WIN = false>
@@ -104,18 +114,28 @@
         }
     };
     int ida[U] = {}, idb[U] = {}, idc[U] = {};
+    bool s0f = false;
+    int kid = 0;
     if constexpr (TAB) {
+        s0f = a.s0 != nullptr;
         load_ids(jfirst, ida);
         load_ids(jfirst + jstep, idb);
+        if (s0f) {
+            const int j = part * 64 + lane;
+            kid = a.hist[(size_t)b * a.hist_ld + (j < a.Tmax ? j : a.Tmax - 1)];
+        }
     }
     float qv[EPC], knv[EPC], vnv[EPC];
-    if (QSC1)
+    if (s0f) {
+#pragma unroll
+        for (int e = 0; e < EPC; ++e) qv[e] = knv[e] = vnv[e] = 0.f;
+    } else if (QSC1)
         load_f32_chunk_sc1<EPC>((const float*)a.q + (size_t)b * a.q_ld + h * 64 + ch * EPC, qv);
     else if (QF32)
         load_f32_slabs<EPC>((const float*)a.q + (size_t)b * a.q_ld + h * 64 + ch * EPC, a.nslab, a.slab_stride, qv);
     else
         load_chunk<T, EPC>((const T*)a.q + (size_t)b * a.q_ld + h * 64 + ch * EPC, qv);
-    if (SELF) {
+    if (SELF && !s0f) {
         if (QF32) {
             load_f32_slabs<EPC>((const float*)a.knew + (size_t)b * a.kv_ld + h * 64 + ch * EPC, a.nslab, a.slab_stride, knv);
             load_f32_slabs<EPC>((const float*)a.vnew + (size_t)b * a.kv_ld + h * 64 + ch * EPC, a.nslab, a.slab_stride, vnv);
@@ -127,7 +147,7 @@
     int n = a.n_keys;
     if (SELF) n = *a.step;
     if constexpr (WIN) n = win_keys(*a.step, a.lookahead, a.n_keys);
-    const float scale2 = a.scale * 1.4426950408889634f;
+    const float scale2 = attn_scale2(a.scale);
 
     const T* kc = (const T*)a.kcache + ((size_t)(b * a.H + h) * a.Tmax) * 64 + ch * EPC;
     const T* vc = (const T*)a.vcache + ((size_t)(b * a.H + h) * a.Tmax) * 64 + ch * EPC;
@@ -151,10 +171,24 @@
         }
     };
 
+    float4 srow0 = make_float4(0.f, 0.f, 0.f, 0.f), srow1 = srow0;
+    float snew = 0.f;
+    if constexpr (TAB) {
+        if (s0f) {
+            const int tn = a.hist[(size_t)b * a.hist_ld + (n < a.Tmax ? n : a.Tmax - 1)];
+            const unsigned t = (unsigned)tn < (unsigned)a.tab_rows ? (unsigned)tn : (unsigned)a.tab_rows - 1u;
+            const float* rp = a.s0 + ((size_t)h * a.tab_rows + t) * kS0Ld + 4 * lane;
+            srow0 = *(const float4*)rp;
+            srow1 = *(const float4*)(rp + 256);
+            snew = a.s0new[(size_t)h * a.tab_rows + t];
+            load_f32_chunk<EPC>(a.qkv0_v + (size_t)t * a.qkv0_ld + h * 64 + ch * EPC, vnv);
+        }
+    }
+
     uint4 cur[U], nxt[U], vfirst[U];
     if (jfirst < n) {
         if constexpr (TAB) {
-            load_tab(tk, ida, cur);
+            if (!s0f) load_tab(tk, ida, cur);
             load_tab(tv, ida, vfirst);
         } else {
             load_batch(kc, jfirst, cur);
@@ -167,7 +201,28 @@
     if (masked && NSPLIT > 1) __syncthreads();
 
     float mx = kNegD;
-    for (int j0 = jfirst; j0 < n; j0 += jstep) {
+    if constexpr (TAB) {
+        for (int j0 = part * 64; s0f && j0 < n; j0 += NSPLIT * 64) {
+            const int j = j0 + lane, jn = j + NSPLIT * 64;
+            int kidn = 0;
+            if (j0 + NSPLIT * 64 < n) kidn = a.hist[(size_t)b * a.hist_ld + (jn < a.Tmax ? jn : a.Tmax - 1)];
+            const unsigned t = (unsigned)kid < (unsigned)a.tab_rows ? (unsigned)kid : (unsigned)a.tab_rows - 1u;
+            const int src = (int)((t & 255u) >> 2) << 2, sel = (int)(((t >> 8) << 2) | (t & 3u));
+            const float r[8] = {srow0.x, srow0.y, srow0.z, srow0.w, srow1.x, srow1.y, srow1.z, srow1.w};
+            float sv = 0.f;
+#pragma unroll
+            for (int i = 0; i < 8; ++i) {
+                const float p = __builtin_bit_cast(float, __builtin_amdgcn_ds_bpermute(src, __builtin_bit_cast(int, r[i])));
+                sv = sel == i ? p : sv;
+            }
+            if (j < n) {
+                s[j] = sv;
+                mx = fmaxf(mx, sv);
+            }
+            kid = kidn;
+        }
+    }
+    for (int j0 = jfirst; !s0f && j0 < n; j0 += jstep) {
         if constexpr (TAB) {
             if (j0 + 2 * jstep < n) load_ids(j0 + 2 * jstep, idc);
             if (j0 + jstep < n) load_tab(tk, idb, nxt);
@@ -179,12 +234,9 @@
             const int j = j0 + u * KPI + sub;
             float kv[EPC];
             cvt_chunk<T, EPC>(cur[u], kv);
-            float d = 0.f;
-#pragma unroll
-            for (int e = 0; e < EPC; ++e) d = fmaf(qv[e], kv[e], d);
-            d = LPK == 8 ? group8_sum(d) : row16_sum(d);
+            const float ks = key_score<EPC>(qv, kv, scale2);
             if (j < n) {
-                float sv = d * scale2;
+                float sv = ks;
                 if (masked && s[j] != 0.f) sv = kNegD;
                 if (ch == 0) s[j] = sv;
                 mx = fmaxf(mx, sv);
@@ -200,15 +252,11 @@
 #pragma unroll
     for (int u = 0; u < U; ++u) cur[u] = vfirst[u];
     if constexpr (TAB) {
-        if (jfirst + jstep < n) load_ids(jfirst + jstep, idb);
+        if (!s0f && jfirst + jstep < n) load_ids(jfirst + jstep, idb);
     }
     int total = n;
     if (SELF) {
-        float d = 0.f;
-#pragma unroll
-        for (int e = 0; e < EPC; ++e) d = fmaf(qv[e], knv[e], d);
-        d = LPK == 8 ? group8_sum(d) : row16_sum(d);
-        const float sv = d * scale2;
+        const float sv = s0f ? snew : key_score<EPC>(qv, knv, scale2);
         total = n + 1;
         if (part == 0) {
             if (lane == 0) s[n] = sv;
diff --git a/dyadic-interaction-modeling_amd/csrc/elementwise.hip b/dyadic-interaction-modeling_amd/csrc/elementwise.hip
--- a/dyadic-interaction-modeling_amd/csrc/elementwise.hip
+++ b/dyadic-interaction-modeling_amd/csrc/elementwise.hip
@@ -477,6 +477,7 @@
     int tok = start[(size_t)(b / start_div) * start_ld];
     tok = tok < 0 ? 0 : (tok >= rows ? rows - 1 : tok);
     if (hist && threadIdx.x == 0) hist[(size_t)b * hist_ld] = tok;
+    if (!out) return;
     const float4* src = (const float4*)(table + (size_t)tok * N);
     float4* dst = (float4*)(out + (size_t)b * N);
     for (int i = threadIdx.x; i < N / 4; i += blockDim.x) dst[i] = src[i];
@@ -701,7 +702,7 @@
 
 int launch_gather_start_rows(const float* table, int N, int rows, const int32_t* start, int start_div, float* out, int B,
                              hipStream_t s, int start_ld, int32_t* hist, int hist_ld) {
-    DIMX_REQUIRE(table && start && out && B > 0 && N > 0 && N % 4 == 0 && rows > 0 && start_ld >= 1 && (!hist || hist_ld >= 1), DIMX_ERR_ARG,
+    DIMX_REQUIRE(table && start && (out || hist) && B > 0 && N > 0 && N % 4 == 0 && rows > 0 && start_ld >= 1 && (!hist || hist_ld >= 1), DIMX_ERR_ARG,
                  "gather_start_rows: bad arguments");
     hipLaunchKernelGGL(gather_start_rows_kernel, dim3(B), dim3(256), 0, s, table, N, rows, start, start_div < 1 ? 1 : start_div, out,
                        start_ld, hist, hist_ld);
diff --git a/dyadic-interaction-modeling_amd/csrc/generate.hip b/dyadic-interaction-modeling_amd/csrc/generate.hip
--- a/dyadic-interaction-modeling_amd/csrc/generate.hip
+++ b/dyadic-interaction-modeling_amd/csrc/generate.hip
@@ -51,6 +51,11 @@
            dg.dim / 2 <= 16 * 64;
 }
 
+static bool s0_table_supported(dimx_handle h) {
+    const DecGeom& dg = h->decg;
+    return h->use_s0_table && h->use_kv0_table && dg.dim_head == 64 && dg.num_tokens <= kS0Ld;
+}
+
 static int qkv0_table_alloc(dimx_handle h) {
     const int V = h->decg.num_tokens, N = h->dec.self_[0].qkv.N;
     if (!h->qkv0_table) {
@@ -60,6 +65,13 @@
     }
     if (h->use_kv0_table && h->at == DIMX_BF16 && !h->kv0_image) {
         DIMX_HIP(hipMalloc(&h->kv0_image, (size_t)V * 2 * (N / 3) * sizeof(bf16)));
+        h->qkv0_epoch = 0;
+        h->graph_valid = false;
+    }
+    if (s0_table_supported(h) && !h->s0_table) {
+        const int H = h->decg.heads;
+        DIMX_HIP(hipMalloc((void**)&h->s0_table, (size_t)H * V * kS0Ld * sizeof(float)));
+        DIMX_HIP(hipMalloc((void**)&h->s0new_table, (size_t)H * V * sizeof(float)));
         h->qkv0_epoch = 0;
         h->graph_valid = false;
     }
@@ -82,6 +94,15 @@
         DIMX_TRY(launch_sum_slabs_rows(s.qkv, ns, s.st_qkv, h->qkv0_table, r * M, V, M, N, st));
     }
     if (h->kv0_image) DIMX_TRY(launch_kv0_image(h->qkv0_table, N, V, N / 3, 2 * (N / 3), h->kv0_image, st));
+    if (h->s0_table) {
+        const int inner = N / 3;
+        const float scale = 1.0f / sqrtf((float)dg.dim_head);
+        if (h->at == DIMX_BF16)
+            DIMX_TRY(launch_s0_table(h->at, h->qkv0_table, N, V, dg.heads, h->kv0_image, 2 * inner, 0, scale, h->s0_table, h->s0new_table, st));
+        else
+            DIMX_TRY(launch_s0_table(h->at, h->qkv0_table, N, V, dg.heads, h->qkv0_table, N, inner, scale, h->s0_table, h->s0new_table, st));
+        ++h->s0_builds;
+    }
     h->qkv0_M = M;
     h->qkv0_at = h->at;
     h->qkv0_epoch = h->dec_epoch;
@@ -185,7 +206,8 @@
     const GenPrompt& pr = c.gc->req.pr;
     DIMX_TRY(launch_embed_step(h->dec.tok_emb, c.DD, c.V, c.start, c.tokens, c.n, s.step, s.x, c.B, c.S, c.st, c.pos, c.pos_scale, pr.ld, pr.step0));
     if (c.r->qkv0)
-        return launch_gather_start_rows(c.r->qkv0, 3 * c.inner, c.V, c.start, c.S, s.qkv, c.B, c.st, pr.ld, c.r->kv0 ? s.hist : nullptr, c.T);
+        return launch_gather_start_rows(c.r->qkv0, 3 * c.inner, c.V, c.start, c.S, c.r->s0 ? nullptr : s.qkv, c.B, c.st, pr.ld,
+                                        c.r->kv0 ? s.hist : nullptr, c.T);
     return launch_add_slabs_layernorm(h->at, s.x, s.xr, 0, s.st_xr, s.y, h->dec.self_[0].ln_g, c.B, c.DD, c.st);
 }
 
@@ -232,6 +254,10 @@
         if (c.h->at == DIMX_BF16) { sa.tab_ld = 2 * inner; sa.tab_koff = 0; sa.tab_voff = inner; }
         else { sa.tab_ld = 3 * inner; sa.tab_koff = inner; sa.tab_voff = 2 * inner; }
         sa.hist = s.hist; sa.hist_ld = c.T;
+        if (c.r->s0) {
+            sa.s0 = c.r->s0; sa.s0new = c.r->s0new;
+            sa.qkv0_v = c.r->qkv0 + 2 * inner; sa.qkv0_ld = 3 * inner;
+        }
     }
     return sa;
 }
@@ -414,7 +440,7 @@
     sm.tokens = c.tokens; sm.tok_ld = c.n; sm.tok_col_from_step = 1; sm.logits_out = c.logits_out; sm.logits_out_ld = c.n;
     sm.emb_table = h->dec.tok_emb; sm.emb_C = c.DD; sm.x_next = s.x; sm.pos_table = c.pos; sm.pos_scale = c.pos_scale; sm.pos_rows = c.n;
     sm.y_next = qkv0 ? nullptr : s.y; sm.y_gamma = qkv0 ? nullptr : h->dec.self_[0].ln_g; sm.y_dtype = h->at;
-    sm.qkv0_table = qkv0; sm.qkv0_out = s.qkv; sm.qkv0_N = 3 * c.inner;
+    sm.qkv0_table = c.r->s0 ? nullptr : qkv0; sm.qkv0_out = s.qkv; sm.qkv0_N = 3 * c.inner;
     if (c.r->kv0) { sm.hist = s.hist; sm.hist_ld = c.T; }
     sm.prompt = c.forced; sm.prompt_ld = pr.ld; sm.prompt_max = pr.Pmax; sm.prompt_len = c.forced_len; sm.prompt_div = c.S;
     return launch_sample(sm, c.st);
@@ -451,6 +477,10 @@
     }
     if (r.qkv0 && h->use_kv0_table && !q.beam && q.pr.step0 == 0 && q.pr.Pmax <= 1 && dg.dim_head == 64 && dg.num_tokens <= 512)
         r.kv0 = h->at == DIMX_BF16 ? h->kv0_image : (const void*)h->qkv0_table;
+    if (r.kv0 && h->s0_table) {
+        r.s0 = h->s0_table;
+        r.s0new = h->s0new_table;
+    }
     if (h->use_layer_chain && r.chain && r.defer && q.S == 1 && 4 * dg.depth + 1 <= kChainSites && !r.win) {
         const StepCtx c = step_ctx(h, gc, r, 0, rows, 0, q.st);
         for (int l = 0; l < dg.depth; ++l) {
@@ -470,7 +500,7 @@
     k.G = r.G; k.S = r.S;
     k.chain = r.chain; k.defer = r.defer; k.logits_chain = r.logits_chain; k.multi_tr = r.multi_tr; k.fault_inject = r.fault_inject;
     for (int l = 0; l < 8; ++l) k.layer_kernel |= r.layer_kernel[l] ? 1u << l : 0u;
-    k.qkv0 = r.qkv0; k.kv0 = r.kv0;
+    k.qkv0 = r.qkv0; k.kv0 = r.kv0; k.s0 = r.s0;
     k.prompt_len = q.pr.len; k.ld_prompt = q.pr.ld; k.Pmax = q.pr.Pmax;
     k.filter_kind = h->filter_kind;
     k.beam = q.beam ? *q.beam : BeamCall{};
@@ -942,6 +972,20 @@
 int dimx_chain_faults(dimx_handle h) { return h ? h->chain_faults : 0; }
 int dimx_qkv0_table_builds(dimx_handle h) { return h ? h->qkv0_builds : 0; }
 int dimx_kv0_table_generations(dimx_handle h) { return h ? h->kv0_generations : 0; }
+int dimx_s0_table_builds(dimx_handle h) { return h ? h->s0_builds : 0; }
+
+int dimx_debug_table_read(dimx_handle h, int which, void* dst, size_t bytes) {
+    DIMX_REQUIRE(h && dst && which >= 0 && which <= 3, DIMX_ERR_ARG, "debug_table_read: bad argument");
+    const DecGeom& dg = h->decg;
+    const size_t V = dg.num_tokens, H = dg.heads, N = h->dec.self_[0].qkv.N;
+    const void* src[4] = {h->qkv0_table, h->kv0_image, h->s0_table, h->s0new_table};
+    const size_t size[4] = {V * N * sizeof(float), V * 2 * (N / 3) * sizeof(bf16), H * V * kS0Ld * sizeof(float), H * V * sizeof(float)};
+    DIMX_REQUIRE(src[which] && h->qkv0_epoch == h->dec_epoch, DIMX_ERR_STATE, "debug_table_read: table %d is not built", which);
+    DIMX_REQUIRE(bytes == size[which], DIMX_ERR_ARG, "debug_table_read: table %d has %zu bytes, not %zu", which, size[which], bytes);
+    DIMX_HIP(hipDeviceSynchronize());
+    DIMX_HIP(hipMemcpy(dst, src[which], bytes, hipMemcpyDeviceToHost));
+    return DIMX_OK;
+}
 
 int dimx_debug_chain_fault(dimx_handle h, int n_calls) {
     DIMX_REQUIRE(h && n_calls >= 0, DIMX_ERR_ARG, "debug_chain_fault: bad argument");
diff --git a/dyadic-interaction-modeling_amd/csrc/model.hip b/dyadic-interaction-modeling_amd/csrc/model.hip
--- a/dyadic-interaction-modeling_amd/csrc/model.hip
+++ b/dyadic-interaction-modeling_amd/csrc/model.hip
@@ -868,6 +868,7 @@
     c->multi_tr = getenv("DIMX_NO_MULTI_TR") ? 0 : 1;
     c->use_qkv0_table = getenv("DIMX_NO_QKV0_TABLE") ? 0 : 1;
     c->use_kv0_table = getenv("DIMX_NO_KV0_TABLE") ? 0 : 1;
+    c->use_s0_table = getenv("DIMX_NO_S0_TABLE") ? 0 : 1;
     if (getenv("DIMX_LAYER_PROF")) {
         void* p = nullptr;
         if (hipMalloc(&p, (size_t)8 * 256 * 16 * 8) == hipSuccess) {
@@ -911,6 +912,8 @@
     if (h->layer_prof_dev) (void)hipFree(h->layer_prof_dev);
     if (h->qkv0_table) (void)hipFree(h->qkv0_table);
     if (h->kv0_image) (void)hipFree(h->kv0_image);
+    if (h->s0_table) (void)hipFree(h->s0_table);
+    if (h->s0new_table) (void)hipFree(h->s0new_table);
     if (h->chain_err_host) (void)hipHostFree(h->chain_err_host);
     free_packed(h);
     stream_forget(h);
diff --git a/dyadic-interaction-modeling_amd/csrc/model.hpp b/dyadic-interaction-modeling_amd/csrc/model.hpp
--- a/dyadic-interaction-modeling_amd/csrc/model.hpp
+++ b/dyadic-interaction-modeling_amd/csrc/model.hpp
@@ -118,6 +118,8 @@
     int lookahead = 0;
     const float* qkv0 = nullptr;
     const void* kv0 = nullptr;
+    const float* s0 = nullptr;
+    const float* s0new = nullptr;
     const BeamCall* beam = nullptr;
     bool fault_inject = false;
     int G = 1, S = 1;
@@ -130,7 +132,7 @@
     int G, S;
     bool chain, defer, logits_chain, multi_tr, fault_inject;
     unsigned layer_kernel;
-    const void *qkv0, *kv0;
+    const void *qkv0, *kv0, *s0;
     const void* prompt_len;
     int ld_prompt, Pmax;
     int filter_kind;
@@ -140,7 +142,7 @@
         return ws == o.ws && B == o.B && T == o.T && top_k == o.top_k && noise == o.noise && start == o.start && mask == o.mask &&
                tokens == o.tokens && logits_out == o.logits_out && G == o.G && S == o.S && chain == o.chain && defer == o.defer &&
                logits_chain == o.logits_chain && multi_tr == o.multi_tr && fault_inject == o.fault_inject &&
-               layer_kernel == o.layer_kernel && qkv0 == o.qkv0 && kv0 == o.kv0 && prompt_len == o.prompt_len &&
+               layer_kernel == o.layer_kernel && qkv0 == o.qkv0 && kv0 == o.kv0 && s0 == o.s0 && prompt_len == o.prompt_len &&
                ld_prompt == o.ld_prompt && Pmax == o.Pmax && filter_kind == o.filter_kind && beam == o.beam && xwin_on == o.xwin_on &&
                xwin_lookahead == o.xwin_lookahead;
     }
@@ -212,6 +214,10 @@
     int use_kv0_table = 1;
     void* kv0_image = nullptr;
     int kv0_generations = 0;
+    int use_s0_table = 1;
+    float* s0_table = nullptr;
+    float* s0new_table = nullptr;
+    int s0_builds = 0;
     int shard_row_off = 0, shard_rows_total = 0;
     int filter_kind = 0;
     float filter_a = 0.f, filter_b = 0.f;
diff --git a/dyadic-interaction-modeling_amd/engine.py b/dyadic-interaction-modeling_amd/engine.py
--- a/dyadic-interaction-modeling_amd/engine.py
+++ b/dyadic-interaction-modeling_amd/engine.py
@@ -364,6 +364,20 @@
     def kv0_table_generations(self):
         return int(self.lib.dimx_kv0_table_generations(self.h))
 
+    def s0_table_builds(self):
+        return int(self.lib.dimx_s0_table_builds(self.h))
+
+    def debug_table(self, which):
+        dg = self.dims
+        V, H = int(dg.num_tokens), int(dg.heads)
+        inner = H * int(dg.dim_head)
+        shape, dt = {"qkv0": ((V, 3 * inner), torch.float32), "kv0": ((V, 2 * inner), torch.bfloat16),
+                     "s0": ((H, V, 512), torch.float32), "s0new": ((H, V), torch.float32)}[which]
+        out = torch.empty(shape, dtype=dt)
+        L.check(self.lib.dimx_debug_table_read(self.h, ("qkv0", "kv0", "s0", "s0new").index(which), out.data_ptr(),
+                                               out.numel() * out.element_size()), "dimx_debug_table_read")
+        return out
+
     def debug_chain_fault(self, n_calls=1):
         L.check(self.lib.dimx_debug_chain_fault(self.h, int(n_calls)), "dimx_debug_chain_fault")
 
diff --git a/dyadic-interaction-modeling_amd/lib.py b/dyadic-interaction-modeling_amd/lib.py
--- a/dyadic-interaction-modeling_amd/lib.py
+++ b/dyadic-interaction-modeling_amd/lib.py
@@ -138,6 +138,8 @@
     "dimx_chain_faults": (c_int, [c_void_p]),
     "dimx_qkv0_table_builds": (c_int, [c_void_p]),
     "dimx_kv0_table_generations": (c_int, [c_void_p]),
+    "dimx_s0_table_builds": (c_int, [c_void_p]),
+    "dimx_debug_table_read": (c_int, [c_void_p, c_int, c_void_p, c_size_t]),
     "dimx_lstm_faults": (c_int, [c_void_p]),
     "dimx_mesh_head": (c_int, [c_void_p, c_void_p, c_void_p, c_int, c_int, c_void_p, c_int, c_void_p, c_size_t, c_void_p]),
     "dimx_op_lstm_layer": (c_int, [c_int, c_void_p, c_int, c_int, c_int, c_int, POINTER(c_void_p), POINTER(c_void_p),
diff --git a/include/dimx.h b/include/dimx.h
--- a/include/dimx.h
+++ b/include/dimx.h
@@ -139,6 +139,8 @@
 int dimx_stream_set_events(dimx_handle h, void* ev_start, void* ev_encoded, void* ev_appended, void* ev_stepped);
 int dimx_qkv0_table_builds(dimx_handle h);
 int dimx_kv0_table_generations(dimx_handle h);
+int dimx_s0_table_builds(dimx_handle h);
+int dimx_debug_table_read(dimx_handle h, int which, void* dst, size_t bytes);
 int dimx_debug_chain_fault(dimx_handle h, int n_calls);
 
 int dimx_mesh_head(dimx_handle h, const float* motion, const float* templ, int B, int L, float* mesh_out, int flags, void* ws,
```

Result: no change. 1738 clips/s, median of 6 (+0.6%).
